# CityU-AIM-Group/HTD

Measured on AMD Instinct MI355X. Metric: images/sec (1333x800) HTD-R50 train step, higher is better.
Workload: dtype f32; 1 GPU; HTD ResNet-50 FPN fp32 train step fwd+bwd+SGD, batch 4/GPU @ 1333x800 (padded 1344x800), random-init weights, 2000 RPN proposals/img, 512 RoIs/img/stage; global_batch=4, parallelism=dp1, stage2_positives=169, proposals=random-init RPN (few positives: the regression branch is nearly idle)

## Files before the change

### htd_amd/csrc/common.h

```cpp
#pragma once
#include <hip/hip_runtime.h>
#include <stdint.h>
#include <stdio.h>
#include <string.h>

#include "../../include/htd_amd.h"

namespace htd {

void set_error(const char *fmt, ...);
int conv_math();

inline int check_launch(const char *what)
{
    hipError_t e = hipGetLastError();
    if (e != hipSuccess) {
        set_error("%s: launch failed: %s", what, hipGetErrorString(e));
        return HTD_ERR_LAUNCH;
    }
    return HTD_OK;
}

#define HTD_REQUIRE(cond, ...)               \
    do {                                     \
        if (!(cond)) {                       \
            htd::set_error(__VA_ARGS__);     \
            return HTD_ERR_ARG;              \
        }                                    \
    } while (0)

constexpr int kWave = 64;

__device__ __forceinline__ float wave_sum(float v)
{
#pragma unroll
    for (int o = 32; o > 0; o >>= 1) v += __shfl_xor(v, o, 64);
    return v;
}
__device__ __forceinline__ float wave_max(float v)
{
#pragma unroll
    for (int o = 32; o > 0; o >>= 1) v = fmaxf(v, __shfl_xor(v, o, 64));
    return v;
}

__device__ __forceinline__ unsigned mag_bits(float v) { return (v != v) ? 0x7fc00000u : (__float_as_uint(v) & 0x7fffffffu); }
__device__ __forceinline__ unsigned mag_bits4(unsigned mx, float4 v)
{
    return max(max(mx, max(mag_bits(v.x), mag_bits(v.y))), max(mag_bits(v.z), mag_bits(v.w)));
}
__device__ __forceinline__ void wave_mag_out(unsigned bits, float *out)
{
#pragma unroll
    for (int o = 32; o > 0; o >>= 1) bits = max(bits, (unsigned)__shfl_xor((int)bits, o, 64));
    if ((threadIdx.x & 63) == 0 && bits > *reinterpret_cast<volatile unsigned *>(out))
        __hip_atomic_fetch_max(reinterpret_cast<unsigned *>(out), bits, __ATOMIC_RELAXED, __HIP_MEMORY_SCOPE_AGENT);
}

inline int64_t ceil_div(int64_t a, int64_t b) { return (a + b - 1) / b; }

}
```

### htd_amd/csrc/conv_fwd.hip

```cpp
#include <algorithm>
#include <mutex>
#include <unordered_map>

#include <stdlib.h>

#include "common.h"

namespace {

using f32x16 = __attribute__((ext_vector_type(16))) float;
using bf16x8 = __attribute__((ext_vector_type(8))) __bf16;

using bf16x2 = __attribute__((ext_vector_type(2))) __bf16;
using f32x2 = __attribute__((ext_vector_type(2))) float;

__device__ __forceinline__ void split3x2(float a, float b, unsigned &h, unsigned &m, unsigned &l)
{
    union { bf16x2 v; unsigned u; } c;
    c.v = __builtin_convertvector(f32x2{a, b}, bf16x2);
    h = c.u;
    const float ra = a - __uint_as_float(h << 16), rb = b - __uint_as_float(h & 0xffff0000u);
    c.v = __builtin_convertvector(f32x2{ra, rb}, bf16x2);
    m = c.u;
    c.v = __builtin_convertvector(f32x2{ra - __uint_as_float(m << 16), rb - __uint_as_float(m & 0xffff0000u)}, bf16x2);
    l = c.u;
}

__device__ __forceinline__ float4 keep4(bool ok, float4 v)
{
    return make_float4(ok ? v.x : 0.f, ok ? v.y : 0.f, ok ? v.z : 0.f, ok ? v.w : 0.f);
}

__device__ __forceinline__ void mfma_x3(f32x16 &acc, const bf16x8 &a, const bf16x8 &b)
{
    asm("v_mfma_f32_32x32x16_bf16 %0, %1, %2, %0" : "+a"(acc) : "v"(a), "v"(b));
}

struct ConvParams {
    const float *x, *w, *bias, *residual, *mask_src;
    float *y;
    int B, H, W, Ci, Co, kh, kw, stride, pad, dil, Ho, Wo;
    int Hx, Wx;
    int ntaps;
    int tap_dy[16], tap_dx[16], tap_w[16];
    int o_h0, o_w0, o_step, oH, oW;
    int relu;
    int res_H, res_W;
    float res_sh, res_sw;
    int64_t w_bstride;
    const int64_t *group_count;
    int lim;
    int64_t M;
    int mt, nt;
    int splits;
    int slices_per_split;
    float *partial;
    int tail_first, tail_splits, tail_sps;
    int cmajor;
    float *amax_out;
};

template <int BK, int WGM, int WGN, int TM, int TN, bool X3 = false>
struct Tile {
    static constexpr int BM = WGM * TM * 32, BN = WGN * TN * 32;
    static constexpr int LDS_STRIDE = BK + 4;
    static constexpr int ROW_HALFS = 3 * BK + 8;
    static constexpr int VEC_PER_ROW = BK / 4;
    static constexpr int ROWS_PER_PASS = 256 / VEC_PER_ROW;
    static constexpr int PASSES_A = (BM + ROWS_PER_PASS - 1) / ROWS_PER_PASS;
    static constexpr int PASSES_B = (BN + ROWS_PER_PASS - 1) / ROWS_PER_PASS;
    static constexpr int MAIN_FLOATS = X3 ? (BM + BN) * ROW_HALFS / 2 : (BM + BN) * LDS_STRIDE;
    static constexpr int EPI_STRIDE = BN + 4;
    static constexpr int EPI_ROWS = WGM * 32;
    static constexpr int EPI_FLOATS = EPI_ROWS * EPI_STRIDE;
    static constexpr int LDS_FLOATS = MAIN_FLOATS > EPI_FLOATS ? MAIN_FLOATS : EPI_FLOATS;
};

template <int BK, int WGM, int WGN, int TM, int TN, bool TAPS, bool X3 = false>
__global__ __launch_bounds__(256, (TM * TN >= 4 ? 3 : 4)) void conv_igemm_kernel(ConvParams p)
{
    static_assert(!X3 || BK % 16 == 0, "the bf16 MFMA takes 16 k per instruction");
    using T = Tile<BK, WGM, WGN, TM, TN, X3>;
    __shared__ __attribute__((aligned(16))) float lds[T::LDS_FLOATS];

    const int nblk = p.mt * p.nt;
    int bid = blockIdx.x, tail_split = -1;
    if (p.tail_splits > 0) {
        const int xcd = bid % 8, idx = bid / 8, dp = p.tail_first / 8;
        if (idx < dp) {
            bid = xcd * dp + idx;
        } else {
            const int units = (nblk - p.tail_first) * p.tail_splits, q = units / 8, r = units % 8;
            const int w = (xcd < r ? xcd * (q + 1) : r * (q + 1) + (xcd - r) * q) + (idx - dp);
            bid = p.tail_first + w / p.tail_splits;
            tail_split = w % p.tail_splits;
        }
    } else {
        const int q = nblk / 8, r = nblk % 8, xcd = bid % 8, idx = bid / 8;
        bid = (xcd < r ? xcd * (q + 1) : r * (q + 1) + (xcd - r) * q) + idx;
    }
    const int tile_m = bid / p.nt, tile_n = bid % p.nt;
    const int64_t m0 = (int64_t)tile_m * T::BM;
    const int n0 = tile_n * T::BN;

    const int tid = threadIdx.x, lane = tid & 63, wave = tid >> 6;
    const int wm = wave / WGN, wn = wave % WGN;

    int k_limit = 0x7fffffff;
    if (p.group_count) {
        const int rows_per_group = p.Ho * p.Wo;
        const int g = (int)(m0 / rows_per_group);
        const int cnt = (int)p.group_count[g];
        const bool dead = ((p.lim & 1) && (int)(m0 - (int64_t)g * rows_per_group) >= cnt) || ((p.lim & 2) && n0 >= cnt);
        if (dead) {
            for (int e = tid; e < T::BM * (T::BN / 4); e += 256) {
                const int64_t m = m0 + e / (T::BN / 4);
                const int n = n0 + (e % (T::BN / 4)) * 4;
                if (m < p.M && n + 3 < p.Co) *reinterpret_cast<float4 *>(p.y + m * p.Co + n) = make_float4(0.f, 0.f, 0.f, 0.f);
                else if (m < p.M)
                    for (int q = 0; q < 4; ++q)
                        if (n + q < p.Co) p.y[m * p.Co + n + q] = 0.f;
            }
            return;
        }
        if (p.lim & 4) k_limit = cnt;
    }

    const int vcol = tid % T::VEC_PER_ROW;
    const int vrow = tid / T::VEC_PER_ROW;
    int a_hi0[T::PASSES_A], a_wi0[T::PASSES_A];
    unsigned a_img[T::PASSES_A];
    bool a_ok[T::PASSES_A];
#pragma unroll
    for (int i = 0; i < T::PASSES_A; ++i) {
        const int r = vrow + i * T::ROWS_PER_PASS;
        const int64_t m = m0 + r;
        a_ok[i] = r < T::BM && m < p.M;
        const unsigned mm = a_ok[i] ? (unsigned)m : 0u;
        const unsigned wo = mm % (unsigned)p.Wo;
        const unsigned t = mm / (unsigned)p.Wo;
        const unsigned ho = t % (unsigned)p.Ho;
        const unsigned b = t / (unsigned)p.Ho;
        a_hi0[i] = TAPS ? (int)ho : (int)ho * p.stride - p.pad;
        a_wi0[i] = TAPS ? (int)wo : (int)wo * p.stride - p.pad;
        a_img[i] = b * (unsigned)(p.Hx * p.Wx);
    }
    const unsigned wrow_stride = (unsigned)(p.kh * p.kw * p.Ci);
    const float *wbase = p.w + (p.w_bstride > 0 ? (m0 / ((int64_t)p.Ho * p.Wo)) * p.w_bstride : 0);
    bool b_ok[T::PASSES_B];
    unsigned b_off[T::PASSES_B];
#pragma unroll
    for (int i = 0; i < T::PASSES_B; ++i) {
        const int r = vrow + i * T::ROWS_PER_PASS;
        const int n = n0 + r;
        b_ok[i] = r < T::BN && n < p.Co;
        b_off[i] = (unsigned)(b_ok[i] ? n : 0) * wrow_stride + vcol * 4;
    }

    const int slices_per_tap = p.Ci / BK;
    const int total_slices = (TAPS ? p.ntaps : p.kh * p.kw) * slices_per_tap;
    const int s_begin = tail_split >= 0 ? tail_split * p.tail_sps : blockIdx.y * p.slices_per_split;
    int num_slices = min(total_slices, s_begin + (tail_split >= 0 ? p.tail_sps : p.slices_per_split));
    if (k_limit != 0x7fffffff) num_slices = min(num_slices, (k_limit + BK - 1) / BK);

    int ld_ci0, ld_ky, ld_kx;
    unsigned ld_woff;
    const bool cmajor = !TAPS && p.cmajor;
    if (cmajor) {
        const int ntap = p.kh * p.kw, cs = s_begin / ntap, tap = s_begin - cs * ntap;
        ld_ci0 = cs * BK;
        ld_ky = tap / p.kw;
        ld_kx = tap - ld_ky * p.kw;
        ld_woff = (unsigned)(tap * p.Ci + ld_ci0);
    } else {
        const int tap = s_begin / slices_per_tap;
        ld_ci0 = (s_begin - tap * slices_per_tap) * BK;
        ld_ky = TAPS ? tap : tap / p.kw;
        ld_kx = TAPS ? 0 : tap - ld_ky * p.kw;
        ld_woff = (unsigned)s_begin * BK;
    }

    float4 ra[T::PASSES_A], rb[T::PASSES_B];
    unsigned ra_ok = 0u;
    unsigned a_base[T::PASSES_A];
#pragma unroll
    for (int i = 0; i < T::PASSES_A; ++i)
        a_base[i] = (a_img[i] + (unsigned)(a_hi0[i] * p.Wx + a_wi0[i])) * (unsigned)p.Ci + vcol * 4;
    auto load_slice = [&]() {
        const int dy = TAPS ? p.tap_dy[ld_ky] : ld_ky * p.dil;
        const int dx = TAPS ? p.tap_dx[ld_ky] : ld_kx * p.dil;
        const unsigned koff = (unsigned)((dy * p.Wx + dx) * p.Ci + ld_ci0);
#pragma unroll
        for (int i = 0; i < T::PASSES_A; ++i) {
            const bool ok = a_ok[i] & ((unsigned)(a_hi0[i] + dy) < (unsigned)p.H) & ((unsigned)(a_wi0[i] + dx) < (unsigned)p.W);
            const unsigned off = (a_base[i] + koff) & (0u - (unsigned)ok);
            ra[i] = *reinterpret_cast<const float4 *>(p.x + off);
            ra_ok = ok ? (ra_ok | (1u << i)) : (ra_ok & ~(1u << i));
        }
        const unsigned woff = TAPS ? (unsigned)(p.tap_w[ld_ky] * p.Ci + ld_ci0) : ld_woff;
#pragma unroll
        for (int i = 0; i < T::PASSES_B; ++i) rb[i] = *reinterpret_cast<const float4 *>(wbase + b_off[i] + woff);
        if (cmajor) {
            ld_woff += (unsigned)p.Ci;
            if (++ld_kx == p.kw) {
                ld_kx = 0;
                if (++ld_ky == p.kh) {
                    ld_ky = 0;
                    ld_ci0 += BK;
                    ld_woff = (unsigned)ld_ci0;
                }
            }
        } else {
            ld_woff += BK;
            ld_ci0 += BK;
            if (ld_ci0 == p.Ci) {
                ld_ci0 = 0;
                if (TAPS) ++ld_ky;
                else if (++ld_kx == p.kw) { ld_kx = 0; ++ld_ky; }
            }
        }
    };
    auto store_slice = [&](int buf) {
        if constexpr (X3) {
            unsigned short *la = reinterpret_cast<unsigned short *>(lds);
            unsigned short *lb = la + T::BM * T::ROW_HALFS;
            auto put = [&](unsigned short *row, float4 v) {
                unsigned h0, m0_, l0, h1, m1, l1;
                split3x2(v.x, v.y, h0, m0_, l0);
                split3x2(v.z, v.w, h1, m1, l1);
                *reinterpret_cast<uint2 *>(row + vcol * 4) = make_uint2(h0, h1);
                *reinterpret_cast<uint2 *>(row + BK + vcol * 4) = make_uint2(m0_, m1);
                *reinterpret_cast<uint2 *>(row + 2 * BK + vcol * 4) = make_uint2(l0, l1);
            };
#pragma unroll
            for (int i = 0; i < T::PASSES_A; ++i) {
                const int r = vrow + i * T::ROWS_PER_PASS;
                if (T::BM % T::ROWS_PER_PASS == 0 || r < T::BM) put(la + r * T::ROW_HALFS, keep4((ra_ok >> i) & 1u, ra[i]));
            }
#pragma unroll
            for (int i = 0; i < T::PASSES_B; ++i) {
                const int r = vrow + i * T::ROWS_PER_PASS;
                if (T::BN % T::ROWS_PER_PASS == 0 || r < T::BN) put(lb + r * T::ROW_HALFS, keep4(b_ok[i], rb[i]));
            }
            return;
        }
        float *la = lds;
        float *lb = lds + T::BM * T::LDS_STRIDE;
#pragma unroll
        for (int i = 0; i < T::PASSES_A; ++i) {
            const int r = vrow + i * T::ROWS_PER_PASS;
            if (T::BM % T::ROWS_PER_PASS == 0 || r < T::BM)
                *reinterpret_cast<float4 *>(la + r * T::LDS_STRIDE + vcol * 4) = keep4((ra_ok >> i) & 1u, ra[i]);
        }
#pragma unroll
        for (int i = 0; i < T::PASSES_B; ++i) {
            const int r = vrow + i * T::ROWS_PER_PASS;
            if (T::BN % T::ROWS_PER_PASS == 0 || r < T::BN)
                *reinterpret_cast<float4 *>(lb + r * T::LDS_STRIDE + vcol * 4) = keep4(b_ok[i], rb[i]);
        }
// ... 78 lines not shown
            for (int j = 0; j < TN; ++j) asm volatile("s_nop 15" : "+a"(acc[i][j]));
    }

    const bool vec_ok = (p.Co & 3) == 0;
    unsigned omx = 0u;
    constexpr int V = T::BN / 4;
    constexpr int RPP = 256 / V;
#pragma unroll
    for (int i = 0; i < TM; ++i) {
#pragma unroll
        for (int j = 0; j < TN; ++j)
#pragma unroll
            for (int r = 0; r < 16; ++r) {
                const int row = wm * 32 + (r & 3) + 8 * (r >> 2) + 4 * fhalf;
                lds[row * T::EPI_STRIDE + (wn * TN + j) * 32 + frow] = acc[i][j][r];
            }
        __syncthreads();
        const int c4 = tid % V;
        const int n = n0 + c4 * 4;
        constexpr int NPASS = T::EPI_ROWS / RPP;
        if (vec_ok && tail_split < 0 && p.splits <= 1 && p.res_H == 0) {
            const bool col_ok = n < p.Co;
            float4 bv = make_float4(0.f, 0.f, 0.f, 0.f);
            if (p.bias != nullptr && col_ok) bv = *reinterpret_cast<const float4 *>(p.bias + n);
            constexpr int UB = NPASS < 4 ? NPASS : 4;
#pragma unroll
            for (int pass0 = 0; pass0 < NPASS; pass0 += UB) {
                float4 v[UB], rv[UB], mv[UB];
                int64_t o[UB];
                bool ok[UB];
#pragma unroll
                for (int u = 0; u < UB; ++u) {
                    const int row = tid / V + (pass0 + u) * RPP;
                    const int64_t m = m0 + ((row >> 5) * TM + i) * 32 + (row & 31);
                    ok[u] = m < p.M && col_ok;
                    int64_t oo;
                    if constexpr (TAPS) {
                        const unsigned mm = ok[u] ? (unsigned)m : 0u, wo = mm % (unsigned)p.Wo, t = mm / (unsigned)p.Wo;
                        const unsigned ho = t % (unsigned)p.Ho, b = t / (unsigned)p.Ho;
                        oo = (((int64_t)b * p.oH + p.o_h0 + p.o_step * (int)ho) * p.oW + p.o_w0 + p.o_step * (int)wo) * p.Co + n;
                    } else
                        oo = m * p.Co + n;
                    o[u] = oo & -(int64_t)ok[u];
                    v[u] = *reinterpret_cast<const float4 *>(lds + row * T::EPI_STRIDE + c4 * 4);
                }
                if (p.residual != nullptr) {
#pragma unroll
                    for (int u = 0; u < UB; ++u) rv[u] = *reinterpret_cast<const float4 *>(p.residual + o[u]);
                }
                if (p.mask_src != nullptr) {
#pragma unroll
                    for (int u = 0; u < UB; ++u) mv[u] = *reinterpret_cast<const float4 *>(p.mask_src + o[u]);
                }
#pragma unroll
                for (int u = 0; u < UB; ++u) { v[u].x += bv.x; v[u].y += bv.y; v[u].z += bv.z; v[u].w += bv.w; }
                if (p.residual != nullptr) {
#pragma unroll
                    for (int u = 0; u < UB; ++u) { v[u].x += rv[u].x; v[u].y += rv[u].y; v[u].z += rv[u].z; v[u].w += rv[u].w; }
                }
                if (p.relu) {
#pragma unroll
                    for (int u = 0; u < UB; ++u) {
                        v[u].x = fmaxf(v[u].x, 0.f); v[u].y = fmaxf(v[u].y, 0.f); v[u].z = fmaxf(v[u].z, 0.f); v[u].w = fmaxf(v[u].w, 0.f);
                    }
                }
                if (p.mask_src != nullptr) {
#pragma unroll
                    for (int u = 0; u < UB; ++u) {
                        v[u].x = mv[u].x > 0.f ? v[u].x : 0.f; v[u].y = mv[u].y > 0.f ? v[u].y : 0.f;
                        v[u].z = mv[u].z > 0.f ? v[u].z : 0.f; v[u].w = mv[u].w > 0.f ? v[u].w : 0.f;
                    }
                }
#pragma unroll
                for (int u = 0; u < UB; ++u)
                    if (ok[u]) {
                        *reinterpret_cast<float4 *>(p.y + o[u]) = v[u];
                        omx = htd::mag_bits4(omx, v[u]);
                    }
            }
            if (i + 1 < TM) __syncthreads();
            continue;
        }
#pragma unroll
        for (int pass = 0; pass < NPASS; ++pass) {
            const int row = tid / V + pass * RPP;
            const int64_t m = m0 + ((row >> 5) * TM + i) * 32 + (row & 31);
            if (m >= p.M || n >= p.Co) continue;
            float4 v = *reinterpret_cast<const float4 *>(lds + row * T::EPI_STRIDE + c4 * 4);
            int64_t o;
            if constexpr (TAPS) {
                const unsigned mm = (unsigned)m, wo = mm % (unsigned)p.Wo, t = mm / (unsigned)p.Wo;
                const unsigned ho = t % (unsigned)p.Ho, b = t / (unsigned)p.Ho;
                o = (((int64_t)b * p.oH + p.o_h0 + p.o_step * (int)ho) * p.oW + p.o_w0 + p.o_step * (int)wo) * p.Co + n;
            } else
                o = m * p.Co + n;
            if (tail_split >= 0) {
                const int lrow = ((row >> 5) * TM + i) * 32 + (row & 31);
                float *dst = p.partial + ((int64_t)(bid - p.tail_first) * p.tail_splits + tail_split) * (T::BM * T::BN) +
                             lrow * T::BN + c4 * 4;
                *reinterpret_cast<float4 *>(dst) = v;
                continue;
            }
            if (p.splits > 1) {
                float *dst = p.partial + (int64_t)blockIdx.y * p.M * p.Co + o;
                if (vec_ok) *reinterpret_cast<float4 *>(dst) = v;
                else {
                    dst[0] = v.x;
                    if (n + 1 < p.Co) dst[1] = v.y;
                    if (n + 2 < p.Co) dst[2] = v.z;
                    if (n + 3 < p.Co) dst[3] = v.w;
                }
                continue;
            }
            if (vec_ok) {
                if (p.bias) {
                    const float4 bv = *reinterpret_cast<const float4 *>(p.bias + n);
                    v.x += bv.x; v.y += bv.y; v.z += bv.z; v.w += bv.w;
                }
                if (p.residual) {
                    int64_t ro = o;
                    if (p.res_H > 0) {
                        const unsigned mm = (unsigned)m, wo = mm % (unsigned)p.Wo, t = mm / (unsigned)p.Wo;
                        const unsigned ho = t % (unsigned)p.Ho, b = t / (unsigned)p.Ho;
                        const int rh = min((int)floorf(ho * p.res_sh), p.res_H - 1);
                        const int rw = min((int)floorf(wo * p.res_sw), p.res_W - 1);
                        ro = (((int64_t)b * p.res_H + rh) * p.res_W + rw) * p.Co + n;
                    }
                    const float4 rv = *reinterpret_cast<const float4 *>(p.residual + ro);
                    v.x += rv.x; v.y += rv.y; v.z += rv.z; v.w += rv.w;
                }
                if (p.relu) { v.x = fmaxf(v.x, 0.f); v.y = fmaxf(v.y, 0.f); v.z = fmaxf(v.z, 0.f); v.w = fmaxf(v.w, 0.f); }
                if (p.mask_src) {
                    const float4 mv = *reinterpret_cast<const float4 *>(p.mask_src + o);
                    v.x = mv.x > 0.f ? v.x : 0.f; v.y = mv.y > 0.f ? v.y : 0.f;
                    v.z = mv.z > 0.f ? v.z : 0.f; v.w = mv.w > 0.f ? v.w : 0.f;
                }
                *reinterpret_cast<float4 *>(p.y + o) = v;
                omx = htd::mag_bits4(omx, v);
            } else {
                auto put = [&](int e, float t) {
                    if (n + e >= p.Co) return;
                    t += p.bias ? p.bias[n + e] : 0.f;
                    if (p.residual) t += p.residual[o + e];
                    if (p.relu) t = fmaxf(t, 0.f);
                    if (p.mask_src) t = p.mask_src[o + e] > 0.f ? t : 0.f;
                    p.y[o + e] = t;
                    omx = max(omx, htd::mag_bits(t));
                };
                put(0, v.x); put(1, v.y); put(2, v.z); put(3, v.w);
            }
        }
        if (i + 1 < TM) __syncthreads();
    }
    if (p.amax_out != nullptr && tail_split < 0 && p.splits <= 1) htd::wave_mag_out(omx, p.amax_out);
}

__global__ __launch_bounds__(256) void conv_splitk_epilogue_kernel(ConvParams p)
{
    const int64_t total = p.M * p.Co;
    unsigned omx = 0u;
    for (int64_t o = (int64_t)blockIdx.x * blockDim.x + threadIdx.x; o < total; o += (int64_t)gridDim.x * blockDim.x) {
        float v = 0.f;
        for (int k = 0; k < p.splits; ++k) v += p.partial[(int64_t)k * total + o];
        const int n = (int)(o % p.Co);
        if (p.bias) v += p.bias[n];
        if (p.residual) {
            int64_t ro = o;
            if (p.res_H > 0) {
                const int64_t m = o / p.Co;
                const unsigned mm = (unsigned)m, wo = mm % (unsigned)p.Wo, t = mm / (unsigned)p.Wo;
                const unsigned ho = t % (unsigned)p.Ho, b = t / (unsigned)p.Ho;
                const int rh = min((int)floorf(ho * p.res_sh), p.res_H - 1);
                const int rw = min((int)floorf(wo * p.res_sw), p.res_W - 1);
                ro = (((int64_t)b * p.res_H + rh) * p.res_W + rw) * p.Co + n;
            }
            v += p.residual[ro];
        }
        if (p.relu) v = fmaxf(v, 0.f);
        if (p.mask_src) v = p.mask_src[o] > 0.f ? v : 0.f;
        p.y[o] = v;
        omx = max(omx, htd::mag_bits(v));
    }
    if (p.amax_out != nullptr) htd::wave_mag_out(omx, p.amax_out);
}

__global__ __launch_bounds__(256) void conv_tail_epilogue_kernel(ConvParams p, int BM, int BN)
{
    const int64_t per_tile = (int64_t)BM * BN, total = (int64_t)(p.mt * p.nt - p.tail_first) * per_tile;
    unsigned omx = 0u;
    for (int64_t e = (int64_t)blockIdx.x * blockDim.x + threadIdx.x; e < total; e += (int64_t)gridDim.x * blockDim.x) {
        const int t = (int)(e / per_tile), within = (int)(e - (int64_t)t * per_tile);
        const int tile = p.tail_first + t, tile_m = tile / p.nt, tile_n = tile % p.nt;
        const int64_t m = (int64_t)tile_m * BM + within / BN;
        const int n = tile_n * BN + within % BN;
        if (m >= p.M || n >= p.Co) continue;
        const float *src = p.partial + (int64_t)t * p.tail_splits * per_tile + within;
        float v = 0.f;
        for (int k = 0; k < p.tail_splits; ++k) v += src[(int64_t)k * per_tile];
        const int64_t o = m * p.Co + n;
        if (p.bias) v += p.bias[n];
        if (p.residual) {
            int64_t ro = o;
            if (p.res_H > 0) {
                const unsigned mm = (unsigned)m, wo = mm % (unsigned)p.Wo, tt = mm / (unsigned)p.Wo;
                const unsigned ho = tt % (unsigned)p.Ho, b = tt / (unsigned)p.Ho;
                const int rh = min((int)floorf(ho * p.res_sh), p.res_H - 1);
                const int rw = min((int)floorf(wo * p.res_sw), p.res_W - 1);
                ro = (((int64_t)b * p.res_H + rh) * p.res_W + rw) * p.Co + n;
            }
            v += p.residual[ro];
        }
        if (p.relu) v = fmaxf(v, 0.f);
        if (p.mask_src) v = p.mask_src[o] > 0.f ? v : 0.f;
        p.y[o] = v;
        omx = max(omx, htd::mag_bits(v));
    }
    if (p.amax_out != nullptr) htd::wave_mag_out(omx, p.amax_out);
}

int g_conv_math = getenv("HTD_CONV_MATH") ? atoi(getenv("HTD_CONV_MATH")) : 1;

template <int WGM, int WGN, int TM, int TN>
void launch_cfg(const ConvParams &p, unsigned blocks, hipStream_t s)
{
    const dim3 grid(blocks, p.splits);
    const bool x3 = g_conv_math == 1;
    if (p.ntaps > 0) {
        if (p.Ci % 16 == 0) {
            if (x3) hipLaunchKernelGGL((conv_igemm_kernel<16, WGM, WGN, TM, TN, true, true>), grid, dim3(256), 0, s, p);
            else hipLaunchKernelGGL((conv_igemm_kernel<16, WGM, WGN, TM, TN, true>), grid, dim3(256), 0, s, p);
        } else
            hipLaunchKernelGGL((conv_igemm_kernel<8, WGM, WGN, TM, TN, true>), grid, dim3(256), 0, s, p);
    } else if (p.Ci % 32 == 0) {
        if (x3) hipLaunchKernelGGL((conv_igemm_kernel<32, WGM, WGN, TM, TN, false, true>), grid, dim3(256), 0, s, p);
        else hipLaunchKernelGGL((conv_igemm_kernel<32, WGM, WGN, TM, TN, false>), grid, dim3(256), 0, s, p);
    } else if (p.Ci % 16 == 0) {
        if (x3) hipLaunchKernelGGL((conv_igemm_kernel<16, WGM, WGN, TM, TN, false, true>), grid, dim3(256), 0, s, p);
        else hipLaunchKernelGGL((conv_igemm_kernel<16, WGM, WGN, TM, TN, false>), grid, dim3(256), 0, s, p);
    } else
        hipLaunchKernelGGL((conv_igemm_kernel<8, WGM, WGN, TM, TN, false>), grid, dim3(256), 0, s, p);
}

int plan_splits(int64_t M, int Co, int Ci, int taps)
{
    const int bk = Ci % 32 == 0 ? 32 : (Ci % 16 == 0 ? 16 : 8);
    const int total_slices = taps * (Ci / bk);
    const int64_t tiles = htd::ceil_div(M, 128) * htd::ceil_div(Co, 64);
    if (tiles <= 0 || tiles >= 384 || total_slices < 16) return 1;
    int64_t want = htd::ceil_div(768, tiles);
    want = std::min<int64_t>(want, total_slices / 8);
    return (int)std::max<int64_t>(1, std::min<int64_t>(want, 16));
}

struct TileCfg { int bm, bn; };
constexpr TileCfg kTileCfg[] = {{64, 64}, {128, 32}, {128, 64}, {128, 128}, {128, 64}, {64, 128}};
constexpr int kNumTileCfg = 6;

static const bool g_tune = getenv("HTD_CONV_TUNE") != nullptr;
int forced_tile()
{
    if (!g_tune) return -1;
    const char *e = getenv("HTD_CONV_FORCE_TILE");
    const int v = e ? atoi(e) : -1;
    return (v >= 0 && v < kNumTileCfg) ? v : -1;
}

static float tile_score(int cfg, int64_t M, int Co, int K, int splits)
{
    const int bm = kTileCfg[cfg].bm, bn = kTileCfg[cfg].bn;
    const int64_t tiles = htd::ceil_div(M, bm) * htd::ceil_div(Co, bn);
    const bool long_k = K >= 1024;
    float base;
    if (g_conv_math == 1) {
        switch (cfg) {
        case 3: base = 1.00f; break;
        case 4: base = long_k ? 0.86f : 0.90f; break;
        case 5: base = long_k ? 0.88f : 0.94f; break;
        default: base = long_k ? 0.72f : 0.82f; break;
        }
    } else {
        switch (cfg) {
        case 3: base = long_k ? 1.00f : 0.90f; break;
        case 4: base = long_k ? 0.98f : 0.97f; break;
        case 5: base = long_k ? 0.98f : 0.98f; break;
        default: base = long_k ? 0.86f : (K >= 512 ? 0.90f : 0.95f); break;
        }
    }
    const float w = (float)(tiles * splits) / 256.f;
    float quant;
    if (w >= 7.f) quant = w / ceilf(w);
    else if (w >= 3.f) quant = 0.97f;
    else quant = w / ceilf(w);
    const float useful = (float)((double)M * Co / ((double)tiles * bm * bn));
    return base * quant * useful;
}

struct TileKey {
    int64_t M;
    int Co, Ci, taps, epi;
    bool operator==(const TileKey &o) const { return M == o.M && Co == o.Co && Ci == o.Ci && taps == o.taps && epi == o.epi; }
};
struct TileKeyHash {
    size_t operator()(const TileKey &k) const
    {
        uint64_t h = (uint64_t)k.M * 0x9E3779B97F4A7C15ull;
        h ^= ((uint64_t)k.Co << 40) ^ ((uint64_t)k.Ci << 20) ^ ((uint64_t)k.taps << 4) ^ (uint64_t)k.epi;
        h *= 0xBF58476D1CE4E5B9ull;
        return (size_t)(h ^ (h >> 29));
    }
};
std::mutex g_tile_mutex;
std::unordered_map<TileKey, int, TileKeyHash> g_tile_table;

int table_tile(int64_t M, int Co, int Ci, int taps, int epi)
{
    std::lock_guard<std::mutex> lock(g_tile_mutex);
    if (g_tile_table.empty()) return -1;
    const auto it = g_tile_table.find(TileKey{M, Co, Ci, taps, epi});
    return it == g_tile_table.end() ? -1 : it->second;
}

int choose_tile(int64_t M, int Co, int Ci, int taps, int epi, int splits, int &bm, int &bn)
{
    const int K = taps * Ci;
    int cfg = forced_tile();
    if (cfg < 0 && epi >= 0) cfg = table_tile(M, Co, Ci, taps, epi);
    if (cfg >= 0 && Co <= 64 && kTileCfg[cfg].bn > 64) cfg = -1;
    if (cfg < 0) {
        if (Co <= 32) cfg = 1;
        else if (Co <= 64) cfg = (htd::ceil_div(M, 128) * htd::ceil_div(Co, 64) < 4400 && M >= 2048) ? 0 : 2;
        else {
            static const int cand[4] = {3, 4, 5, 0};
            float best = -1.f;
            for (int c : cand) {
                const float sc = tile_score(c, M, Co, K, splits);
                if (sc > best * 1.005f) { best = sc; cfg = c; }
            }
        }
    }
    bm = kTileCfg[cfg].bm;
    bn = kTileCfg[cfg].bn;
    return cfg;
}

static const bool g_no_tail = getenv("HTD_CONV_NO_TAIL") != nullptr;
int plan_tail(int64_t M, int Co, int Ci, int taps, int bm, int bn, int &tail_splits, int &tail_sps)
{
    tail_splits = tail_sps = 0;
    if (g_no_tail || (Co & 3)) return 0;
    const int bk = Ci % 32 == 0 ? 32 : (Ci % 16 == 0 ? 16 : 8);
    const int total_slices = taps * (Ci / bk);
    const int64_t tiles = htd::ceil_div(M, bm) * htd::ceil_div(Co, bn);
    const int64_t rem = tiles % 256, whole = tiles - rem;
    if (tiles < 256 * 3 || tiles >= 256 * 7 || rem == 0 || rem > 128 || total_slices < 8) return 0;
    int want = (int)std::min<int64_t>(16, std::max<int64_t>(2, (256 + rem / 2) / rem));
    want = std::min(want, total_slices / 4);
    if (want < 2) return 0;
    tail_sps = (int)htd::ceil_div(total_slices, want);
    tail_splits = (int)htd::ceil_div(total_slices, tail_sps);
    return (int)whole;
}

int launch_conv(ConvParams p, hipStream_t s, void *workspace)
{
    const int bk = (p.Ci % 32 == 0 && p.ntaps == 0) ? 32 : (p.Ci % 16 == 0 ? 16 : 8);
    const int total_slices = (p.ntaps > 0 ? p.ntaps : p.kh * p.kw) * (p.Ci / bk);
    p.splits = (workspace && p.ntaps == 0) ? plan_splits(p.M, p.Co, p.Ci, p.kh * p.kw) : 1;
    p.slices_per_split = (int)htd::ceil_div(total_slices, p.splits);
    p.splits = (int)htd::ceil_div(total_slices, p.slices_per_split);
    int bm, bn;
// ... 309 lines not shown
```

### htd_amd/csrc/conv_wgrad.hip

```cpp
#include <algorithm>

#include "common.h"

namespace {

using f32x16 = __attribute__((ext_vector_type(16))) float;

__device__ __forceinline__ float4 keep4(bool ok, float4 v)
{
    return make_float4(ok ? v.x : 0.f, ok ? v.y : 0.f, ok ? v.z : 0.f, ok ? v.w : 0.f);
}

struct WgradParams {
    const float *x, *gy;
    float *out;
    float *bias_out;
    int B, H, W, Ci, Co, kh, kw, stride, pad, dil, Ho, Wo;
    int64_t K;
    int Ntot;
    int mt, nt, splits;
    int64_t slices_per_split;
    const float *amax_x, *amax_g;
};

// ... 1104 lines not shown
            if ((c & 1) == 0) {
                if constexpr (H2) split2w(v.x * sc, v.y * sc, h[0], l[0]);
                else split3x2w(v.x, v.y, h[0], m[0], l[0]);
            } else {
                if constexpr (H2) split2w(v.z * sc, v.w * sc, h[1], l[1]);
                else split3x2w(v.z, v.w, h[1], m[1], l[1]);
                unsigned short *d = wr + (u >= PA ? b_lds0 : u == 0 ? a_lds0 : a_lds1);
                const int plane = u < PA ? XHD_PLANE_A : XHD_PLANE_B;
                *reinterpret_cast<uint2 *>(d) = make_uint2(h[0], h[1]);
                if constexpr (H2) {
                    *reinterpret_cast<uint2 *>(d + plane) = make_uint2(l[0], l[1]);
                } else {
                    *reinterpret_cast<uint2 *>(d + plane) = make_uint2(m[0], m[1]);
                    *reinterpret_cast<uint2 *>(d + 2 * plane) = make_uint2(l[0], l[1]);
                }
                if (u < PA) { bsum.x += v.x; bsum.y += v.y; bsum.z += v.z; bsum.w += v.w; }
            }
#pragma unroll
            for (int e = c * NM / NC; e < (c + 1) * NM / NC; ++e) {
                const int q = e / (3 * TM), t = (e % (3 * TM)) / TM, i = e % TM;
                acc[t][i] = mfma_x3w<H2>(fa[i][QA[q]], fb[t][QB[q]], acc[t][i]);
            }
            __builtin_amdgcn_sched_barrier(0);
        }
        if (__builtin_amdgcn_readfirstlane(wave) == 0) {
            if (ragged) put(wr + b_lds1, XHD_PLANE_B, qb[1], sx);
        }
        load_slice(qa, qb);
        __syncthreads();
    };
    auto store_slice = [&](unsigned short *wr, const float4 (&qa)[PA], const float4 (&qb)[2]) {
        put(wr + a_lds0, XHD_PLANE_A, qa[0], sg);
        if constexpr (PA > 1) put(wr + a_lds1, XHD_PLANE_A, qa[PA - 1], sg);
#pragma unroll
        for (int i = 0; i < PA; ++i) { bsum.x += qa[i].x; bsum.y += qa[i].y; bsum.z += qa[i].z; bsum.w += qa[i].w; }
        put(wr + b_lds0, XHD_PLANE_B, qb[0], sx);
        if (ragged) put(wr + b_lds1, XHD_PLANE_B, qb[1], sx);
    };

    unsigned short *buf0 = lds, *buf1 = lds + XHD_BUF;
    load_slice(ra[0], rb[0]);
    load_slice(ra[1], rb[1]);
    store_slice(buf0, ra[0], rb[0]);
    load_slice(ra[0], rb[0]);
    __syncthreads();
    for (int s = 0; s < n_slices; s += 2) {
        half(buf0, buf1, ra[1], rb[1]);
        half(buf1, buf0, ra[0], rb[0]);
    }

    if (do_bias) {
        float4 *red = reinterpret_cast<float4 *>(lds);
        __syncthreads();
        red[tid] = bsum;
        __syncthreads();
        if (tid < VA) {
            float4 t = red[tid];
            for (int r = 1; r < RA; ++r) {
                const float4 v = red[r * VA + tid];
                t.x += v.x; t.y += v.y; t.z += v.z; t.w += v.w;
            }
            float *dst = p.bias_out + (int64_t)split * p.Co;
            const int m = m0 + tid * 4;
            if (m < p.Co) dst[m] = t.x;
            if (m + 1 < p.Co) dst[m + 1] = t.y;
            if (m + 2 < p.Co) dst[m + 2] = t.z;
            if (m + 3 < p.Co) dst[m + 3] = t.w;
        }
    }
    float *out = p.out + (int64_t)split * p.Co * p.Ntot;
    const int fcol = lane & 31, fhalf = lane >> 5;
    const int ci = ci0 + wn * 32 + fcol;
    if (ci < p.Ci) {
#pragma unroll
        for (int t = 0; t < 3; ++t) {
            const int n = (ky * 3 + t) * p.Ci + ci;
#pragma unroll
            for (int i = 0; i < TM; ++i)
#pragma unroll
                for (int r = 0; r < 16; ++r) {
                    const int m = m0 + wm * TM * 32 + i * 32 + (r & 3) + 8 * (r >> 2) + 4 * fhalf;
                    if (m < p.Co) out[(int64_t)m * p.Ntot + n] = H2 ? acc[t][i][r] * sg_inv * sx_inv : acc[t][i][r];
                }
        }
    }
}

__global__ __launch_bounds__(256) void splitk_reduce_kernel(const float *__restrict__ ws, float *__restrict__ out,
                                                            int64_t n, int splits, const float *__restrict__ ws2 = nullptr,
                                                            float *__restrict__ out2 = nullptr, int n2 = 0, int acc = 0)
{
    const int extra = out2 ? (n2 + 255) / 256 : 0;
    if ((int)blockIdx.x >= (int)gridDim.x - extra) {
        const int i = ((int)blockIdx.x - ((int)gridDim.x - extra)) * 256 + threadIdx.x;
        if (i < n2) {
            float s = acc ? out2[i] : 0.f;
            int k = 0;
            for (; k + 3 < splits; k += 4) {
                const float a = ws2[(int64_t)k * n2 + i], b = ws2[(int64_t)(k + 1) * n2 + i];
                const float c = ws2[(int64_t)(k + 2) * n2 + i], d = ws2[(int64_t)(k + 3) * n2 + i];
                s += a; s += b; s += c; s += d;
            }
            for (; k < splits; ++k) s += ws2[(int64_t)k * n2 + i];
            out2[i] = s;
        }
        return;
    }
    const unsigned main_blocks = gridDim.x - extra;
    const int64_t n4 = (n & 3) == 0 ? (n >> 2) : 0;
    for (int64_t i = (int64_t)blockIdx.x * blockDim.x + threadIdx.x; i < n4; i += (int64_t)main_blocks * blockDim.x) {
        float4 s = acc ? *reinterpret_cast<const float4 *>(out + i * 4) : make_float4(0.f, 0.f, 0.f, 0.f);
        int k = 0;
        for (; k + 3 < splits; k += 4) {
            float4 v[4];
#pragma unroll
            for (int u = 0; u < 4; ++u) v[u] = *reinterpret_cast<const float4 *>(ws + (int64_t)(k + u) * n + i * 4);
#pragma unroll
            for (int u = 0; u < 4; ++u) { s.x += v[u].x; s.y += v[u].y; s.z += v[u].z; s.w += v[u].w; }
        }
        for (; k < splits; ++k) {
            const float4 v = *reinterpret_cast<const float4 *>(ws + (int64_t)k * n + i * 4);
            s.x += v.x; s.y += v.y; s.z += v.z; s.w += v.w;
        }
        *reinterpret_cast<float4 *>(out + i * 4) = s;
    }
    if (blockIdx.x == 0)
        for (int64_t i = n4 * 4 + threadIdx.x; i < n; i += blockDim.x) {
            float s = acc ? out[i] : 0.f;
            for (int k = 0; k < splits; ++k) s += ws[(int64_t)k * n + i];
            out[i] = s;
        }
}

__global__ __launch_bounds__(256) void reduce_rows_kernel(const float *__restrict__ ws, float *__restrict__ out, int n,
                                                          int rows)
{
    __shared__ float red[16][17];
    const int col = threadIdx.x & 15, grp = threadIdx.x >> 4;
    const int c = blockIdx.x * 16 + col;
    float s = 0.f;
    if (c < n)
        for (int k = grp; k < rows; k += 16) s += ws[(int64_t)k * n + c];
    red[grp][col] = s;
    __syncthreads();
    if (grp == 0 && c < n) {
        float t = red[0][col];
#pragma unroll
        for (int g = 1; g < 16; ++g) t += red[g][col];
        out[c] = t;
    }
}

using htd::mag_bits;
using htd::wave_mag_out;

__global__ __launch_bounds__(256) void colsum_mask_kernel(const float *__restrict__ g, const float *__restrict__ y,
                                                          float *__restrict__ gm, float *__restrict__ partial,
                                                          int64_t rows, int C, int64_t rows_per_block, float *__restrict__ amax_out)
{
    const int c = blockIdx.y * 256 + threadIdx.x;
    const int64_t r0 = (int64_t)blockIdx.x * rows_per_block, r1 = min(rows, r0 + rows_per_block);
    float s = 0.f;
    unsigned mx = 0u;
    if (c < C)
        for (int64_t r = r0; r < r1; ++r) {
            float v = g[r * C + c];
            if (y) {
                v = y[r * C + c] > 0.f ? v : 0.f;
                gm[r * C + c] = v;
            }
            mx = max(mx, mag_bits(v));
            s += v;
        }
    if (amax_out) wave_mag_out(mx, amax_out);
    if (partial && c < C) partial[(int64_t)blockIdx.x * C + c] = s;
}

__global__ __launch_bounds__(256) void colsum_mask_vec_kernel(const float *__restrict__ g, const float *__restrict__ y,
                                                              float *__restrict__ gm, float *__restrict__ partial,
                                                              int64_t rows, int C, int64_t rows_per_block,
                                                              float *__restrict__ amax_out)
{
    __shared__ float4 red[256];
    unsigned mx = 0u;
    const int C4 = C >> 2;
    const int cbase = blockIdx.y * 256;
    const int cw = min(256, C4 - cbase);
    const int R = 256 / cw;
    const int c4 = threadIdx.x % cw, rsub = threadIdx.x / cw;
    const int64_t r0 = (int64_t)blockIdx.x * rows_per_block, r1 = min(rows, r0 + rows_per_block);
    float4 s = make_float4(0.f, 0.f, 0.f, 0.f);
    if (rsub < R) {
        int64_t r = r0 + rsub;
        for (; r + 3 * (int64_t)R < r1; r += 4 * (int64_t)R) {
            float4 v[4], yv[4];
#pragma unroll
            for (int u = 0; u < 4; ++u) {
                const int64_t o = (r + u * (int64_t)R) * C + (int64_t)(cbase + c4) * 4;
                v[u] = *reinterpret_cast<const float4 *>(g + o);
                if (y) yv[u] = *reinterpret_cast<const float4 *>(y + o);
            }
#pragma unroll
            for (int u = 0; u < 4; ++u) {
                if (y) {
                    const int64_t o = (r + u * (int64_t)R) * C + (int64_t)(cbase + c4) * 4;
                    v[u].x = yv[u].x > 0.f ? v[u].x : 0.f; v[u].y = yv[u].y > 0.f ? v[u].y : 0.f;
                    v[u].z = yv[u].z > 0.f ? v[u].z : 0.f; v[u].w = yv[u].w > 0.f ? v[u].w : 0.f;
                    *reinterpret_cast<float4 *>(gm + o) = v[u];
                }
                mx = htd::mag_bits4(mx, v[u]);
                s.x += v[u].x; s.y += v[u].y; s.z += v[u].z; s.w += v[u].w;
            }
        }
        for (; r < r1; r += R) {
            const int64_t o = r * C + (int64_t)(cbase + c4) * 4;
            float4 v = *reinterpret_cast<const float4 *>(g + o);
            if (y) {
                const float4 yv = *reinterpret_cast<const float4 *>(y + o);
                v.x = yv.x > 0.f ? v.x : 0.f; v.y = yv.y > 0.f ? v.y : 0.f;
                v.z = yv.z > 0.f ? v.z : 0.f; v.w = yv.w > 0.f ? v.w : 0.f;
                *reinterpret_cast<float4 *>(gm + o) = v;
            }
            mx = htd::mag_bits4(mx, v);
            s.x += v.x; s.y += v.y; s.z += v.z; s.w += v.w;
        }
    }
    if (amax_out) wave_mag_out(mx, amax_out);
    if (!partial) return;
    red[threadIdx.x] = s;
    __syncthreads();
    if (rsub == 0) {
        for (int k = 1; k < R; ++k) {
            const float4 t = red[k * cw + c4];
            s.x += t.x; s.y += t.y; s.z += t.z; s.w += t.w;
        }
        *reinterpret_cast<float4 *>(partial + (int64_t)blockIdx.x * C + (int64_t)(cbase + c4) * 4) = s;
    }
}

struct Cfg { int splits; int mt, nt; int bm, bn; };

template <int WGM, int WGN, int TM, int TN>
void launch_wgrad(int pix, bool covec, dim3 grid, hipStream_t s, const WgradParams &p)
{
#define HTD_WGRAD_CASE(PIX, CV)                                                                                   \
    if (pix == PIX && covec == CV) {                                                                               \
        hipLaunchKernelGGL((conv_wgrad_kernel<WGM, WGN, TM, TN, PIX, CV>), grid, dim3(256), 0, s, p);             \
        return;                                                                                                    \
    }
    HTD_WGRAD_CASE(PIX_POINTWISE, true) HTD_WGRAD_CASE(PIX_WIDE, true) HTD_WGRAD_CASE(PIX_GENERAL, true)
    HTD_WGRAD_CASE(PIX_POINTWISE, false) HTD_WGRAD_CASE(PIX_WIDE, false) HTD_WGRAD_CASE(PIX_GENERAL, false)
#undef HTD_WGRAD_CASE
}

Cfg choose(int Co, int Ntot, int64_t K)
{
    Cfg c;
    c.bm = Co <= 32 ? 32 : 128;
    c.bn = 128;
    c.mt = (int)htd::ceil_div(Co, c.bm);
    c.nt = (int)htd::ceil_div(Ntot, c.bn);
    const int64_t slices = htd::ceil_div(K, BKW);
    static const int units = getenv("HTD_WGRAD_UNITS") ? atoi(getenv("HTD_WGRAD_UNITS")) : 1536;
    int64_t want = htd::ceil_div(units, (int64_t)c.mt * c.nt);
    const int64_t tiles = (int64_t)c.mt * c.nt;
    int64_t cap = std::max<int64_t>(1, slices / 20);
    if (tiles * cap < 256)
        cap = std::max(cap, std::min<int64_t>(htd::ceil_div(256, tiles), std::max<int64_t>(1, slices / 5)));
    want = std::min<int64_t>(want, cap);
    c.splits = (int)std::max<int64_t>(1, std::min<int64_t>(want, 192));
    if (c.splits >= 6) c.splits = (c.splits + 7) / 8 * 8;
    static const int forced = getenv("HTD_WGRAD_SPLITS") ? atoi(getenv("HTD_WGRAD_SPLITS")) : 0;
    if (forced > 0) c.splits = (int)std::min<int64_t>(forced, slices);
    return c;
}

static const bool g_wgrad_x3h_off = getenv("HTD_WGRAD_X3H") != nullptr && atoi(getenv("HTD_WGRAD_X3H")) == 0;
bool x3h_takes(int Ci, int Co, int kh, int kw, int stride, int pad, int dil)
{
    return !g_wgrad_x3h_off && kh == 3 && kw == 3 && stride == 1 && pad == 1 && dil == 1 && Co >= 64 && (Co & 3) == 0 &&
           Ci >= 32 && (Ci & 3) == 0;
}
int x3h_splits(int B, int H, int W, int Ci, int Co)
{
    const int64_t tiles = htd::ceil_div(Co, 128) * htd::ceil_div(Ci, 64) * 3;
    const int64_t slices = htd::ceil_div((int64_t)B * H * (W + 1), XH_KS);
    static const int target = getenv("HTD_WGRAD_X3H_UNITS") ? atoi(getenv("HTD_WGRAD_X3H_UNITS")) : 768;
    int64_t want = htd::ceil_div(target, tiles);
    int64_t cap = std::max<int64_t>(1, slices / 8);
    if (tiles * cap < 256) cap = std::max(cap, std::min<int64_t>(htd::ceil_div(256, tiles), std::max<int64_t>(1, slices / 4)));
    want = std::min<int64_t>(want, cap);
    int splits = (int)std::max<int64_t>(1, std::min<int64_t>(want, 128));
    if (splits >= 6) splits = (splits + 7) / 8 * 8;
    static const int forced = getenv("HTD_WGRAD_X3H_SPLITS") ? atoi(getenv("HTD_WGRAD_X3H_SPLITS")) : 0;
    if (forced > 0) splits = (int)std::min<int64_t>(forced, std::max<int64_t>(1, slices / 2));
    return splits;
}

}

int g_wgrad_math = -1;

extern "C" int64_t htd_conv2d_wgrad_workspace_bytes(int B, int H, int W, int Ci, int Co, int kh, int kw, int stride,
                                                    int pad, int dil)
{
    const int Ho = (H + 2 * pad - (dil * (kh - 1) + 1)) / stride + 1;
    const int Wo = (W + 2 * pad - (dil * (kw - 1) + 1)) / stride + 1;
    const Cfg c = choose(Co, kh * kw * Ci, (int64_t)B * Ho * Wo);
    int splits = c.splits;
    if (x3h_takes(Ci, Co, kh, kw, stride, pad, dil)) splits = std::max(splits, x3h_splits(B, H, W, Ci, Co));
    return (int64_t)splits * Co * (kh * kw * Ci + 1) * 4 + 256;
}

static int bwd_weight_impl(const float *x, const float *gy, float *gw, float *gbias, int B, int H, int W, int Ci, int Co, int kh,
                           int kw, int stride, int pad, int dil, void *workspace, void *stream, int accumulate,
                           const float *amax_x = nullptr, const float *amax_g = nullptr)
{
    HTD_REQUIRE(B > 0 && H > 0 && W > 0 && Ci > 0 && Co > 0 && kh > 0 && kw > 0 && stride > 0 && dil > 0 && pad >= 0,
                "conv2d_bwd_weight: bad sizes");
    HTD_REQUIRE(Ci % 4 == 0, "conv2d_bwd_weight: Ci=%d must be a multiple of 4", Ci);
    HTD_REQUIRE(x && gy && gw && workspace, "conv2d_bwd_weight: null pointer");
    WgradParams p{};
    p.x = x; p.gy = gy;
    p.amax_x = amax_x; p.amax_g = amax_g;
    const bool h2 = amax_x != nullptr && amax_g != nullptr;
    p.B = B; p.H = H; p.W = W; p.Ci = Ci; p.Co = Co; p.kh = kh; p.kw = kw; p.stride = stride; p.pad = pad; p.dil = dil;
    p.Ho = (H + 2 * pad - (dil * (kh - 1) + 1)) / stride + 1;
    p.Wo = (W + 2 * pad - (dil * (kw - 1) + 1)) / stride + 1;
    HTD_REQUIRE(p.Ho > 0 && p.Wo > 0, "conv2d_bwd_weight: empty output");
    p.K = (int64_t)B * p.Ho * p.Wo;
    HTD_REQUIRE((int64_t)B * H * W * Ci < (1ll << 31) && p.K * Co < (1ll << 31),
                "conv2d_bwd_weight: operand larger than 2^31 elements (32-bit element offsets)");
    p.Ntot = kh * kw * Ci;
    static const int math_env0 = getenv("HTD_CONV_MATH") ? atoi(getenv("HTD_CONV_MATH")) : 1;
    if ((g_wgrad_math < 0 ? math_env0 : g_wgrad_math) == 1 && x3h_takes(Ci, Co, kh, kw, stride, pad, dil)) {
        p.mt = (int)htd::ceil_div(Co, 128);
        p.nt = (int)htd::ceil_div(Ci, 64);
        p.splits = x3h_splits(B, H, W, Ci, Co);
        const int64_t slices = htd::ceil_div((int64_t)B * H * (W + 1), XH_KS);
        p.slices_per_split = htd::ceil_div(slices, p.splits);
        p.splits = (int)htd::ceil_div(slices, p.slices_per_split);
        const bool direct = p.splits == 1 && !accumulate;
        p.out = direct ? gw : (float *)workspace;
        float *bias_part = (float *)workspace + (int64_t)p.splits * Co * p.Ntot;
        p.bias_out = !gbias ? nullptr : (direct ? gbias : bias_part);
        hipStream_t s = (hipStream_t)stream;
        const dim3 grid((unsigned)(p.mt * p.nt * 3 * p.splits));
        static const bool x3hd_on = !(getenv("HTD_WGRAD_X3D") && atoi(getenv("HTD_WGRAD_X3D")) == 0);
        if (x3hd_on && XHD_KS / (W + 1) + 1 <= H && (int64_t)B * H * W * Ci * 4 < (1ll << 31) &&
            (int64_t)B * H * W * Co * 4 < (1ll << 31))
        {
            static const bool tile64 = !(getenv("HTD_WGRAD_TILE64") && atoi(getenv("HTD_WGRAD_TILE64")) == 0);
            if (tile64 && Co <= 64) {
                p.mt = (int)htd::ceil_div(Co, 64);
                const dim3 g64((unsigned)(p.mt * p.nt * 3 * p.splits));
                if (h2) hipLaunchKernelGGL((conv_wgrad_x3hd_kernel<1, true>), g64, dim3(256), 0, s, p);
                else hipLaunchKernelGGL((conv_wgrad_x3hd_kernel<1, false>), g64, dim3(256), 0, s, p);
            } else if (h2) {
                hipLaunchKernelGGL((conv_wgrad_x3hd_kernel<2, true>), grid, dim3(256), 0, s, p);
            } else {
                hipLaunchKernelGGL((conv_wgrad_x3hd_kernel<2, false>), grid, dim3(256), 0, s, p);
            }
        }
        else {
            HTD_REQUIRE(!h2, "conv2d_bwd_weight_h2: this 3x3 layer is not taken by the H2 kernels (htd_conv2d_bwd_weight_h2_supported)");
            if (W + 1 >= XH_KS) hipLaunchKernelGGL(conv_wgrad_x3h_kernel<true>, grid, dim3(256), 0, s, p);
            else hipLaunchKernelGGL(conv_wgrad_x3h_kernel<false>, grid, dim3(256), 0, s, p);
        }
        if (!direct) {
            const int64_t n = (int64_t)Co * p.Ntot;
            const unsigned blocks = (unsigned)std::min<int64_t>(htd::ceil_div(n, 256), 2048);
            const unsigned extra = gbias ? (unsigned)htd::ceil_div(Co, 256) : 0u;
            hipLaunchKernelGGL(splitk_reduce_kernel, dim3(blocks + extra), dim3(256), 0, s, (const float *)workspace, gw, n,
                               p.splits, (const float *)(gbias ? bias_part : nullptr), gbias, Co, accumulate);
        }
        return htd::check_launch("conv2d_bwd_weight");
    }
    const Cfg c = choose(Co, p.Ntot, p.K);
    p.mt = c.mt; p.nt = c.nt; p.splits = c.splits;
    p.slices_per_split = htd::ceil_div(htd::ceil_div(p.K, BKW), c.splits);
// ... 130 lines not shown
```

### htd_amd/csrc/roi_align.hip

```cpp
#include <algorithm>

#include "common.h"

namespace {

struct RoiGeom {
    float start_h, start_w, bin_h, bin_w;
    int grid_h, grid_w, batch;
    float inv_count;
};

__device__ __forceinline__ RoiGeom roi_geometry(const float *roi, float scale, int ph, int pw,
                                                int sampling_ratio, int aligned)
{
    RoiGeom g;
    const float off = aligned ? 0.5f : 0.f;
    g.batch = (int)roi[0];
    g.start_w = roi[1] * scale - off;
    g.start_h = roi[2] * scale - off;
    const float end_w = roi[3] * scale - off, end_h = roi[4] * scale - off;
    float rw = end_w - g.start_w, rh = end_h - g.start_h;
    if (!aligned) { rw = fmaxf(rw, 1.f); rh = fmaxf(rh, 1.f); }
    g.bin_h = rh / (float)ph;
    g.bin_w = rw / (float)pw;
    g.grid_h = sampling_ratio > 0 ? sampling_ratio : (int)ceilf(rh / (float)ph);
    g.grid_w = sampling_ratio > 0 ? sampling_ratio : (int)ceilf(rw / (float)pw);
    const int cnt = g.grid_h * g.grid_w;
    g.inv_count = 1.f / (float)(cnt > 1 ? cnt : 1);
    return g;
}

__device__ __forceinline__ float axis_weight(float start, float bin, int bin_idx, int grid, int p,
                                             int extent)
{
    float w = 0.f;
    const float step = bin / (float)grid;
    const float base = start + (float)bin_idx * bin;
    for (int s = 0; s < grid; ++s) {
        const float v = base + ((float)s + .5f) * step;
        if (v < -1.0f || v > (float)extent) continue;
        const float vc = fminf(fmaxf(v, 0.f), (float)(extent - 1));
        w += fmaxf(0.f, 1.f - fabsf(vc - (float)p));
    }
    return w;
}

__device__ __forceinline__ void axis_span(float start, float bin, int bin_idx, int grid, int extent,
                                          int &lo, int &hi)
{
    if (grid <= 0) { lo = 0; hi = -1; return; }
    const float step = bin / (float)grid;
    const float base = start + (float)bin_idx * bin;
    const float v0 = base + .5f * step, v1 = base + ((float)(grid - 1) + .5f) * step;
    const float c0 = fminf(fmaxf(fminf(v0, v1), 0.f), (float)(extent - 1));
    const float c1 = fminf(fmaxf(fmaxf(v0, v1), 0.f), (float)(extent - 1));
    lo = (int)c0;
    hi = min((int)c1 + 1, extent - 1);
}

__device__ __forceinline__ float lane_bcast(float v, int src)
{
    return __int_as_float(__builtin_amdgcn_readlane(__float_as_int(v), src));
}

template <bool BACKWARD>
__global__ __launch_bounds__(256) void roi_align_kernel(const float *__restrict__ feat_or_gout,
                                                        const float *__restrict__ rois,
                                                        const int64_t *__restrict__ roi_level, int level,
                                                        float *__restrict__ out_or_gfeat, int64_t n,
                                                        int B, int C, int H, int W, int ph, int pw,
                                                        float scale, int sampling_ratio, int aligned,
                                                        int chunks, int64_t tasks)
{
    const int lane = threadIdx.x & 63;
    const int64_t task = (int64_t)blockIdx.x * (blockDim.x >> 6) + (threadIdx.x >> 6);
    if (task >= tasks) return;
    const int chunk = (int)(task % chunks);
    const int64_t t2 = task / chunks;
    const int bin = (int)(t2 % (ph * pw));
    const int64_t ri = t2 / (ph * pw);
    const int64_t roi_row = ri;
    if (roi_level && roi_level[ri] != (int64_t)level) return;
    const int bi = bin / pw, bj = bin % pw;
    const RoiGeom g = roi_geometry(rois + 5 * roi_row, scale, ph, pw, sampling_ratio, aligned);

    int r0, r1, c0, c1;
    axis_span(g.start_h, g.bin_h, bi, g.grid_h, H, r0, r1);
    axis_span(g.start_w, g.bin_w, bj, g.grid_w, W, c0, c1);
    if (g.batch < 0 || g.batch >= B) { r0 = 0; r1 = -1; }

    const size_t img_base = (size_t)g.batch * H * W * C;
    const size_t bin_off = ((size_t)roi_row * ph * pw + bin) * C;

    if (!BACKWARD) {
        const int ch = chunk * 256 + lane * 4;
        const bool act = ch < C;
        float4 acc = make_float4(0.f, 0.f, 0.f, 0.f);
        for (int rb = r0; rb <= r1; rb += 64) {
            const float wy_l = (rb + lane <= r1) ? axis_weight(g.start_h, g.bin_h, bi, g.grid_h, rb + lane, H) : 0.f;
            for (int cb = c0; cb <= c1; cb += 64) {
                const float wx_l = (cb + lane <= c1) ? axis_weight(g.start_w, g.bin_w, bj, g.grid_w, cb + lane, W) : 0.f;
                const int rn = min(64, r1 - rb + 1), cn = min(64, c1 - cb + 1);
                for (int r = 0; r < rn; ++r) {
                    const float wy = lane_bcast(wy_l, r);
                    const float *row = feat_or_gout + img_base + ((size_t)(rb + r) * W + cb) * C + ch;
#pragma unroll 4
                    for (int c = 0; c < cn; ++c) {
                        const float w = wy * lane_bcast(wx_l, c);
                        if (act) {
                            const float4 v = *reinterpret_cast<const float4 *>(row + (size_t)c * C);
                            acc.x += w * v.x; acc.y += w * v.y; acc.z += w * v.z; acc.w += w * v.w;
                        }
                    }
                }
            }
        }
        if (act) {
            acc.x *= g.inv_count; acc.y *= g.inv_count; acc.z *= g.inv_count; acc.w *= g.inv_count;
            *reinterpret_cast<float4 *>(out_or_gfeat + bin_off + ch) = acc;
        }
    } else {
        float go[4];
#pragma unroll
        for (int k = 0; k < 4; ++k) {
            const int ch = chunk * 256 + lane + 64 * k;
            go[k] = ch < C ? feat_or_gout[bin_off + ch] * g.inv_count : 0.f;
        }
        for (int rb = r0; rb <= r1; rb += 64) {
            const float wy_l = (rb + lane <= r1) ? axis_weight(g.start_h, g.bin_h, bi, g.grid_h, rb + lane, H) : 0.f;
            for (int cb = c0; cb <= c1; cb += 64) {
                const float wx_l = (cb + lane <= c1) ? axis_weight(g.start_w, g.bin_w, bj, g.grid_w, cb + lane, W) : 0.f;
                const int rn = min(64, r1 - rb + 1), cn = min(64, c1 - cb + 1);
                for (int r = 0; r < rn; ++r) {
                    const float wy = lane_bcast(wy_l, r);
                    if (wy == 0.f) continue;
                    float *row = out_or_gfeat + img_base + ((size_t)(rb + r) * W + cb) * C + chunk * 256 + lane;
                    for (int c = 0; c < cn; ++c) {
                        const float w = wy * lane_bcast(wx_l, c);
                        if (w == 0.f) continue;
#pragma unroll
                        for (int k = 0; k < 4; ++k)
                            if (chunk * 256 + lane + 64 * k < C)
                                atomicAdd(row + (size_t)c * C + 64 * k, w * go[k]);
                    }
                }
            }
        }
    }
}

template <int WAVES>
__global__ __launch_bounds__(64 * WAVES) void roi_align_fwd_split_kernel(const float *__restrict__ feat, const float *__restrict__ rois,
                                                                  const int64_t *__restrict__ roi_level, int level,
                                                                  float *__restrict__ out, int B, int C, int H, int W, int ph,
                                                                  int pw, float scale, int sampling_ratio, int aligned,
                                                                  int chunks)
{
    __shared__ float4 part[WAVES][64];
    const int lane = threadIdx.x & 63, wave = threadIdx.x >> 6;
    const int64_t task = blockIdx.x;
    const int chunk = (int)(task % chunks);
    const int64_t t2 = task / chunks;
    const int bin = (int)(t2 % (ph * pw));
    const int64_t ri = t2 / (ph * pw);
    if (roi_level && roi_level[ri] != (int64_t)level) return;
    const int bi = bin / pw, bj = bin % pw;
    const RoiGeom g = roi_geometry(rois + 5 * ri, scale, ph, pw, sampling_ratio, aligned);
    int r0, r1, c0, c1;
    axis_span(g.start_h, g.bin_h, bi, g.grid_h, H, r0, r1);
    axis_span(g.start_w, g.bin_w, bj, g.grid_w, W, c0, c1);
    if (g.batch < 0 || g.batch >= B) { r0 = 0; r1 = -1; }
    const size_t img_base = (size_t)g.batch * H * W * C;
    const int ch = chunk * 256 + lane * 4;
    const bool act = ch < C;
    float4 acc = make_float4(0.f, 0.f, 0.f, 0.f);
    for (int rb = r0; rb <= r1; rb += 64) {
        const float wy_l = (rb + lane <= r1) ? axis_weight(g.start_h, g.bin_h, bi, g.grid_h, rb + lane, H) : 0.f;
        const int rn = min(64, r1 - rb + 1);
        for (int cb = c0; cb <= c1; cb += 64) {
            const float wx_l = (cb + lane <= c1) ? axis_weight(g.start_w, g.bin_w, bj, g.grid_w, cb + lane, W) : 0.f;
            const int cn = min(64, c1 - cb + 1);
            for (int r = wave; r < rn; r += WAVES) {
                const float wy = lane_bcast(wy_l, r);
                const float *row = feat + img_base + ((size_t)(rb + r) * W + cb) * C + ch;
#pragma unroll 4
                for (int c = 0; c < cn; ++c) {
                    const float w = wy * lane_bcast(wx_l, c);
                    if (act) {
                        const float4 v = *reinterpret_cast<const float4 *>(row + (size_t)c * C);
                        acc.x += w * v.x; acc.y += w * v.y; acc.z += w * v.z; acc.w += w * v.w;
                    }
                }
            }
        }
    }
    part[wave][lane] = acc;
    __syncthreads();
    if (wave == 0 && act) {
        float4 t = part[0][lane];
#pragma unroll
        for (int w = 1; w < WAVES; ++w) {
            const float4 v = part[w][lane];
            t.x += v.x; t.y += v.y; t.z += v.z; t.w += v.w;
        }
        t.x *= g.inv_count; t.y *= g.inv_count; t.z *= g.inv_count; t.w *= g.inv_count;
        *reinterpret_cast<float4 *>(out + ((size_t)ri * ph * pw + bin) * C + ch) = t;
    }
}

struct LevelTable {
    const float *feat[8];
    int H[8], W[8];
    float scale[8];
};

__global__ __launch_bounds__(256) void roi_align_levels_fwd_kernel(LevelTable tab, const float *__restrict__ rois,
                                                                   const int64_t *__restrict__ roi_level, float *__restrict__ out,
                                                                   int64_t n, int B, int C, int L, int ph, int pw,
                                                                   int sampling_ratio, int aligned, int chunks, int64_t tasks,
                                                                   float *__restrict__ amax_out)
{
    const int lane = threadIdx.x & 63;
    const int64_t task = (int64_t)blockIdx.x * (blockDim.x >> 6) + (threadIdx.x >> 6);
    if (task >= tasks) return;
    const unsigned seen = amax_out ? *reinterpret_cast<const volatile unsigned *>(amax_out) : 0u;
    const int chunk = (int)(task % chunks);
    const int64_t t2 = task / chunks;
    const int bin = (int)(t2 % (ph * pw));
    const int64_t ri = t2 / (ph * pw);
    const int lv = (int)roi_level[ri];
    const int ch = chunk * 256 + lane * 4;
    const bool act = ch < C;
    const size_t bin_off = ((size_t)ri * ph * pw + bin) * C;
    float4 acc = make_float4(0.f, 0.f, 0.f, 0.f);
    RoiGeom g{};
    g.inv_count = 0.f;
    if (lv >= 0 && lv < L) {
        const int H = tab.H[lv], W = tab.W[lv];
        const float *feat = tab.feat[lv];
        const int bi = bin / pw, bj = bin % pw;
        g = roi_geometry(rois + 5 * ri, tab.scale[lv], ph, pw, sampling_ratio, aligned);
        int r0, r1, c0, c1;
        axis_span(g.start_h, g.bin_h, bi, g.grid_h, H, r0, r1);
        axis_span(g.start_w, g.bin_w, bj, g.grid_w, W, c0, c1);
        if (g.batch < 0 || g.batch >= B) { r0 = 0; r1 = -1; }
        const size_t img_base = (size_t)g.batch * H * W * C;
        for (int rb = r0; rb <= r1; rb += 64) {
            const float wy_l = (rb + lane <= r1) ? axis_weight(g.start_h, g.bin_h, bi, g.grid_h, rb + lane, H) : 0.f;
            for (int cb = c0; cb <= c1; cb += 64) {
                const float wx_l = (cb + lane <= c1) ? axis_weight(g.start_w, g.bin_w, bj, g.grid_w, cb + lane, W) : 0.f;
                const int rn = min(64, r1 - rb + 1), cn = min(64, c1 - cb + 1);
                for (int r = 0; r < rn; ++r) {
                    const float wy = lane_bcast(wy_l, r);
                    const float *row = feat + img_base + ((size_t)(rb + r) * W + cb) * C + ch;
#pragma unroll 4
                    for (int c = 0; c < cn; ++c) {
                        const float w = wy * lane_bcast(wx_l, c);
                        if (act) {
                            const float4 v = *reinterpret_cast<const float4 *>(row + (size_t)c * C);
                            acc.x += w * v.x; acc.y += w * v.y; acc.z += w * v.z; acc.w += w * v.w;
                        }
                    }
                }
            }
        }
    }
    if (act) {
        acc.x *= g.inv_count; acc.y *= g.inv_count; acc.z *= g.inv_count; acc.w *= g.inv_count;
        *reinterpret_cast<float4 *>(out + bin_off + ch) = acc;
    }
    if (amax_out) {
        const bool nan = act && ((acc.x != acc.x) | (acc.y != acc.y) | (acc.z != acc.z) | (acc.w != acc.w));
        const float m = act ? fmaxf(fmaxf(fabsf(acc.x), fabsf(acc.y)), fmaxf(fabsf(acc.z), fabsf(acc.w))) : 0.f;
        unsigned bits = nan ? 0x7fc00000u : __float_as_uint(m);
        for (int o = 32; o > 0; o >>= 1) bits = max(bits, (unsigned)__shfl_xor((int)bits, o));
        if (lane == 0 && bits > seen)
            __hip_atomic_fetch_max(reinterpret_cast<unsigned *>(amax_out), bits, __ATOMIC_RELAXED, __HIP_MEMORY_SCOPE_AGENT);
    }
}

struct AllLevelsOut {
    float *out[8];
};

template <int WAVES>
__global__ __launch_bounds__(WAVES == 1 ? 256 : 64 * WAVES) void roi_align_all_levels_fwd_kernel(
    LevelTable tab, AllLevelsOut outs, const float *__restrict__ rois, int64_t n, int B, int C, int L, int ph, int pw,
    int sampling_ratio, int aligned, int chunks, int64_t tasks)
{
    __shared__ float4 part[WAVES == 1 ? 1 : WAVES][64];
    const int lane = threadIdx.x & 63, wave = threadIdx.x >> 6;
    const int64_t task = WAVES == 1 ? (int64_t)blockIdx.x * 4 + wave : (int64_t)blockIdx.x;
    if (WAVES == 1 && task >= tasks) return;
    const int chunk = (int)(task % chunks);
    int64_t t2 = task / chunks;
    const int bin = (int)(t2 % (ph * pw));
    t2 /= ph * pw;
    const int64_t ri = t2 % n;
    const int lv = (int)(t2 / n);
    const int H = tab.H[lv], W = tab.W[lv];
    const float *feat = tab.feat[lv];
    const int bi = bin / pw, bj = bin % pw;
    const RoiGeom g = roi_geometry(rois + 5 * ri, tab.scale[lv], ph, pw, sampling_ratio, aligned);
    int r0, r1, c0, c1;
    axis_span(g.start_h, g.bin_h, bi, g.grid_h, H, r0, r1);
    axis_span(g.start_w, g.bin_w, bj, g.grid_w, W, c0, c1);
    if (g.batch < 0 || g.batch >= B) { r0 = 0; r1 = -1; }
    const size_t img_base = (size_t)g.batch * H * W * C;
    const int ch = chunk * 256 + lane * 4;
    const bool act = ch < C;
    float4 acc = make_float4(0.f, 0.f, 0.f, 0.f);
    for (int rb = r0; rb <= r1; rb += 64) {
        const float wy_l = (rb + lane <= r1) ? axis_weight(g.start_h, g.bin_h, bi, g.grid_h, rb + lane, H) : 0.f;
        const int rn = min(64, r1 - rb + 1);
        for (int cb = c0; cb <= c1; cb += 64) {
            const float wx_l = (cb + lane <= c1) ? axis_weight(g.start_w, g.bin_w, bj, g.grid_w, cb + lane, W) : 0.f;
            const int cn = min(64, c1 - cb + 1);
            for (int r = (WAVES == 1 ? 0 : wave); r < rn; r += WAVES) {
                const float wy = lane_bcast(wy_l, r);
                const float *row = feat + img_base + ((size_t)(rb + r) * W + cb) * C + ch;
#pragma unroll 4
                for (int c = 0; c < cn; ++c) {
                    const float w = wy * lane_bcast(wx_l, c);
                    if (act) {
                        const float4 v = *reinterpret_cast<const float4 *>(row + (size_t)c * C);
                        acc.x += w * v.x; acc.y += w * v.y; acc.z += w * v.z; acc.w += w * v.w;
                    }
                }
            }
        }
    }
    float *dst = outs.out[lv] + ((size_t)ri * ph * pw + bin) * C + ch;
    if constexpr (WAVES == 1) {
        if (act) {
            acc.x *= g.inv_count; acc.y *= g.inv_count; acc.z *= g.inv_count; acc.w *= g.inv_count;
            *reinterpret_cast<float4 *>(dst) = acc;
        }
    } else {
        part[wave][lane] = acc;
        __syncthreads();
        if (wave == 0 && act) {
            float4 t = part[0][lane];
#pragma unroll
            for (int w = 1; w < WAVES; ++w) {
                const float4 v = part[w][lane];
                t.x += v.x; t.y += v.y; t.z += v.z; t.w += v.w;
            }
            t.x *= g.inv_count; t.y *= g.inv_count; t.z *= g.inv_count; t.w *= g.inv_count;
            *reinterpret_cast<float4 *>(dst) = t;
        }
    }
}

constexpr int MAXP = 8;

__global__ __launch_bounds__(256) void roi_align_bwd_rows_kernel(const float *__restrict__ gout,
                                                                 const float *__restrict__ rois,
                                                                 const int64_t *__restrict__ roi_level, int level,
                                                                 float *__restrict__ gfeat, int64_t n, int B, int C,
                                                                 int H, int W, int ph, int pw, float scale,
                                                                 int sampling_ratio, int aligned, int chunks,
                                                                 int row_slots, int64_t tasks)
{
    const int lane = threadIdx.x & 63;
    const int64_t task = (int64_t)blockIdx.x * (blockDim.x >> 6) + (threadIdx.x >> 6);
    if (task >= tasks) return;
    const int chunk = (int)(task % chunks);
    const int64_t t2 = task / chunks;
    const int slot = (int)(t2 % row_slots);
    const int64_t ri = t2 / row_slots;
    if (roi_level && roi_level[ri] != (int64_t)level) return;
    const RoiGeom g = roi_geometry(rois + 5 * ri, scale, ph, pw, sampling_ratio, aligned);
    if (g.batch < 0 || g.batch >= B) return;
    int r_lo, r_hi, c_lo, c_hi, t0, t1;
    axis_span(g.start_h, g.bin_h, 0, g.grid_h, H, r_lo, t0);
    axis_span(g.start_h, g.bin_h, ph - 1, g.grid_h, H, t1, r_hi);
    if (t0 < r_lo || r_hi < t1) return;
    axis_span(g.start_w, g.bin_w, 0, g.grid_w, W, c_lo, t0);
    axis_span(g.start_w, g.bin_w, pw - 1, g.grid_w, W, t1, c_hi);
    if (t0 < c_lo || c_hi < t1) return;
    const size_t img_base = (size_t)g.batch * H * W * C;
    const float *go = gout + (size_t)ri * ph * pw * C + chunk * 256 + lane;
    bool chk[4];
#pragma unroll
    for (int k = 0; k < 4; ++k) chk[k] = chunk * 256 + lane + 64 * k < C;

    for (int r = r_lo + slot; r <= r_hi; r += row_slots) {
        const float wy_l = lane < ph ? axis_weight(g.start_h, g.bin_h, lane, g.grid_h, r, H) : 0.f;
        float T[MAXP][4];
#pragma unroll
        for (int q = 0; q < MAXP; ++q)
#pragma unroll
            for (int k = 0; k < 4; ++k) T[q][k] = 0.f;
        bool any_row = false;
        for (int p = 0; p < ph; ++p) {
            const float wy = lane_bcast(wy_l, p) * g.inv_count;
            if (wy == 0.f) continue;
            any_row = true;
#pragma unroll
            for (int q = 0; q < MAXP; ++q)
                if (q < pw) {
#pragma unroll
                    for (int k = 0; k < 4; ++k)
                        if (chk[k]) T[q][k] += wy * go[((size_t)p * pw + q) * C + 64 * k];
                }
        }
        if (!any_row) continue;
        for (int cb = c_lo; cb <= c_hi; cb += 64) {
            float wx_l[MAXP];
#pragma unroll
            for (int q = 0; q < MAXP; ++q)
                wx_l[q] = (q < pw && cb + lane <= c_hi) ? axis_weight(g.start_w, g.bin_w, q, g.grid_w, cb + lane, W) : 0.f;
            const int cn = min(64, c_hi - cb + 1);
            float *row = gfeat + img_base + ((size_t)r * W + cb) * C + chunk * 256 + lane;
            for (int c = 0; c < cn; ++c) {
                float v[4] = {0.f, 0.f, 0.f, 0.f};
                bool any = false;
#pragma unroll
                for (int q = 0; q < MAXP; ++q) {
                    const float w = lane_bcast(wx_l[q], c);
                    if (w != 0.f) {
                        any = true;
#pragma unroll
                        for (int k = 0; k < 4; ++k) v[k] += w * T[q][k];
                    }
                }
                if (!any) continue;
#pragma unroll
                for (int k = 0; k < 4; ++k)
                    if (chk[k]) atomicAdd(row + (size_t)c * C + 64 * k, v[k]);
            }
        }
    }
}

constexpr int GW_TILE = 8;

struct RoiBox { short b, r_lo, r_hi, c_lo, c_hi, pad0, pad1, pad2; };

__global__ __launch_bounds__(256) void roi_bbox_kernel(const float *__restrict__ rois, const int64_t *__restrict__ roi_level,
                                                       int level, RoiBox *__restrict__ box, int64_t n, int B, int H, int W,
                                                       int ph, int pw, float scale, int sampling_ratio, int aligned)
{
    const int64_t ri = (int64_t)blockIdx.x * 256 + threadIdx.x;
    if (ri >= n) return;
    RoiBox o{};
    o.b = -1;
    if (!roi_level || roi_level[ri] == (int64_t)level) {
        const RoiGeom g = roi_geometry(rois + 5 * ri, scale, ph, pw, sampling_ratio, aligned);
        int r_lo, r_hi, c_lo, c_hi, t0, t1;
        axis_span(g.start_h, g.bin_h, 0, g.grid_h, H, r_lo, t0);
        axis_span(g.start_h, g.bin_h, ph - 1, g.grid_h, H, t1, r_hi);
        bool ok = g.batch >= 0 && g.batch < B && !(t0 < r_lo || r_hi < t1);
        axis_span(g.start_w, g.bin_w, 0, g.grid_w, W, c_lo, t0);
        axis_span(g.start_w, g.bin_w, pw - 1, g.grid_w, W, t1, c_hi);
        ok = ok && !(t0 < c_lo || c_hi < t1);
        if (ok) { o.b = (short)g.batch; o.r_lo = (short)r_lo; o.r_hi = (short)r_hi; o.c_lo = (short)c_lo; o.c_hi = (short)c_hi; }
    }
    box[ri] = o;
}

template <int CPL, int ROWS, int RS, bool FOLD>
__device__ __forceinline__ void gather_tile(const float *__restrict__ gout, const float *__restrict__ rois,
                                            const RoiBox *__restrict__ box, float *__restrict__ gfeat, int64_t n, int B, int C,
                                            int H, int W, int ph, int pw, float scale, int sampling_ratio, int aligned,
                                            int accumulate, int chunks, int segs, int hts, int64_t task, bool active,
                                            const float *__restrict__ tbuf)
{
    static_assert(!FOLD || ROWS == 1, "folded rows: one-row tiles");
    static_assert(ROWS * MAXP <= 64, "one lane per (row, bin) weight");
    static_assert(RS == 1 || ROWS == 1, "the RoI split keeps one-row tiles");
    const int lane = threadIdx.x & 63;
    const int wave = threadIdx.x >> 6, part = wave % RS;
    constexpr unsigned long long kEvery = RS == 4 ? 0x1111111111111111ull : (RS == 2 ? 0x5555555555555555ull : ~0ull);
    const unsigned long long mine = kEvery << part;
    const int chunk = (int)(task % chunks);
    int64_t t2 = task / chunks;
    const int seg = (int)(t2 % segs);
    t2 /= segs;
    const int ht = (int)(t2 % hts), b = (int)(t2 / hts);
    const int y0 = ht * ROWS, y1 = min(H, y0 + ROWS) - 1;
    const int x0 = seg * GW_TILE, x1 = min(W, x0 + GW_TILE) - 1;
    const int ch = chunk * 64 * CPL + lane * CPL;
    const bool act = ch < C;

    float acc[ROWS][GW_TILE][CPL];
#pragma unroll
    for (int r = 0; r < ROWS; ++r)
#pragma unroll
        for (int i = 0; i < GW_TILE; ++i)
#pragma unroll
            for (int k = 0; k < CPL; ++k) acc[r][i][k] = 0.f;
    bool touched = false;

    for (int64_t base = 0; base < (active ? n : 0); base += 64) {
        bool hit = false;
        if (base + lane < n) {
            const RoiBox o = box[base + lane];
            hit = o.b == b && o.r_lo <= y1 && y0 <= o.r_hi && o.c_lo <= x1 && o.c_hi >= x0;
        }
        unsigned long long mask = __ballot(hit) & mine;
        while (mask) {
            const int src = __builtin_ctzll(mask);
            mask &= mask - 1;
            const int64_t ri = base + src;
            touched = true;
            const RoiGeom g = roi_geometry(rois + 5 * ri, scale, ph, pw, sampling_ratio, aligned);
            if constexpr (FOLD) {
                static_assert(GW_TILE * MAXP == 64, "one lane per (bin, pixel) weight");
                const int xi_f = lane % GW_TILE, q_f = lane / GW_TILE;
                const float wx_f = (x0 + xi_f <= x1 && q_f < pw) ? axis_weight(g.start_w, g.bin_w, q_f, g.grid_w, x0 + xi_f, W) : 0.f;
                const float *tp = tbuf + (((size_t)ri * H + y0) * pw) * C + ch;
#pragma unroll
                for (int q = 0; q < MAXP; ++q) {
                    if (q >= pw) continue;
                    if (__ballot(q_f == q && wx_f != 0.f) == 0ull) continue;
                    float v[CPL];
#pragma unroll
                    for (int k = 0; k < CPL; ++k) v[k] = 0.f;
                    if (act) {
                        if constexpr (CPL == 4) {
                            const float4 t4 = *reinterpret_cast<const float4 *>(tp + (size_t)q * C);
                            v[0] = t4.x; v[1] = t4.y; v[2] = t4.z; v[3] = t4.w;
                        } else {
#pragma unroll
                            for (int k = 0; k < CPL; ++k) v[k] = tp[(size_t)q * C + k];
                        }
                    }
#pragma unroll
                    for (int xi = 0; xi < GW_TILE; ++xi) {
                        const float w = lane_bcast(wx_f, q * GW_TILE + xi);
                        if (w != 0.f) {
#pragma unroll
                            for (int k = 0; k < CPL; ++k) acc[0][xi][k] += w * v[k];
                        }
                    }
                }
                continue;
            }
            const int r_l = lane / MAXP, p_l = lane % MAXP;
            const float wy_l = (r_l < ROWS && p_l < ph && y0 + r_l <= y1)
                                   ? axis_weight(g.start_h, g.bin_h, p_l, g.grid_h, y0 + r_l, H) * g.inv_count : 0.f;
            float T[ROWS][MAXP][CPL];
#pragma unroll
            for (int r = 0; r < ROWS; ++r)
#pragma unroll
                for (int q = 0; q < MAXP; ++q)
#pragma unroll
                    for (int k = 0; k < CPL; ++k) T[r][q][k] = 0.f;
            const float *go = gout + (size_t)ri * ph * pw * C + ch;
            for (int p = 0; p < ph; ++p) {
                float wy[ROWS];
                bool any = false;
#pragma unroll
                for (int r = 0; r < ROWS; ++r) {
                    wy[r] = lane_bcast(wy_l, r * MAXP + p);
                    any = any || wy[r] != 0.f;
                }
                if (!any) continue;
#pragma unroll
                for (int q = 0; q < MAXP; ++q)
                    if (q < pw && act) {
                        float v[CPL];
                        if constexpr (CPL == 4) {
                            const float4 t = *reinterpret_cast<const float4 *>(go + ((size_t)p * pw + q) * C);
                            v[0] = t.x; v[1] = t.y; v[2] = t.z; v[3] = t.w;
                        } else if constexpr (CPL == 2) {
                            const float2 t = *reinterpret_cast<const float2 *>(go + ((size_t)p * pw + q) * C);
                            v[0] = t.x; v[1] = t.y;
                        } else {
                            v[0] = go[((size_t)p * pw + q) * C];
                        }
#pragma unroll
                        for (int r = 0; r < ROWS; ++r)
#pragma unroll
                            for (int k = 0; k < CPL; ++k) T[r][q][k] += wy[r] * v[k];
                    }
            }
            static_assert(GW_TILE * MAXP == 64, "one lane per (bin, pixel) weight");
            const int xi_l = lane % GW_TILE, q_l = lane / GW_TILE;
            const float wx_l = (x0 + xi_l <= x1 && q_l < pw) ? axis_weight(g.start_w, g.bin_w, q_l, g.grid_w, x0 + xi_l, W) : 0.f;
#pragma unroll
            for (int xi = 0; xi < GW_TILE; ++xi) {
#pragma unroll
                for (int q = 0; q < MAXP; ++q) {
                    if (q >= pw) continue;
                    const float w = lane_bcast(wx_l, q * GW_TILE + xi);
                    if (w != 0.f) {
#pragma unroll
                        for (int r = 0; r < ROWS; ++r)
#pragma unroll
                            for (int k = 0; k < CPL; ++k) acc[r][xi][k] += w * T[r][q][k];
                    }
                }
            }
        }
    }
    if constexpr (RS > 1) {
        __shared__ float lsum[4][GW_TILE * CPL][64];
        __shared__ int ltouched[4];
        if (part > 0) {
#pragma unroll
            for (int i = 0; i < GW_TILE; ++i)
#pragma unroll
                for (int k = 0; k < CPL; ++k) lsum[wave][i * CPL + k][lane] = acc[0][i][k];
            if (lane == 0) ltouched[wave] = touched ? 1 : 0;
        }
        __syncthreads();
        if (part > 0) return;
#pragma unroll
        for (int w = 1; w < RS; ++w) {
#pragma unroll
            for (int i = 0; i < GW_TILE; ++i)
#pragma unroll
                for (int k = 0; k < CPL; ++k) acc[0][i][k] += lsum[wave + w][i * CPL + k][lane];
            touched = touched || ltouched[wave + w] != 0;
        }
    }
    if (!active || !act || (accumulate && !touched)) return;
#pragma unroll
    for (int r = 0; r < ROWS; ++r) {
        if (y0 + r > y1) continue;
        float *row = gfeat + (((size_t)b * H + y0 + r) * W + x0) * C + ch;
#pragma unroll
        for (int xi = 0; xi < GW_TILE; ++xi) {
            if (x0 + xi > x1) continue;
            float *dst = row + (size_t)xi * C;
#pragma unroll
            for (int k = 0; k < CPL; ++k) dst[k] = accumulate ? dst[k] + acc[r][xi][k] : acc[r][xi][k];
        }
    }
}

template <int CPL, int ROWS, int RS>
__global__ __launch_bounds__(256, (RS > 1 ? 4 : 1)) void roi_align_bwd_gather_kernel(const float *__restrict__ gout, const float *__restrict__ rois,
                                                                   const RoiBox *__restrict__ box, float *__restrict__ gfeat,
                                                                   int64_t n, int B, int C, int H, int W, int ph, int pw,
                                                                   float scale, int sampling_ratio, int aligned, int accumulate,
                                                                   int chunks, int segs, int hts, int64_t tasks)
{
    const int64_t task = (int64_t)blockIdx.x * (4 / RS) + (threadIdx.x >> 6) / RS;
    if (RS == 1 && task >= tasks) return;
    gather_tile<CPL, ROWS, RS, false>(gout, rois, box, gfeat, n, B, C, H, W, ph, pw, scale, sampling_ratio, aligned, accumulate,
                                      chunks, segs, hts, task < tasks ? task : 0, task < tasks, nullptr);
}

constexpr int GL_MAX = 6;
struct GatherLevels {
    float *gfeat[GL_MAX];
    const float *gout[GL_MAX];
    float *tbuf[GL_MAX];
    int64_t ftask0[GL_MAX + 1];
    const RoiBox *box[GL_MAX];
    int H[GL_MAX], W[GL_MAX], segs[GL_MAX], hts[GL_MAX], accumulate[GL_MAX], level[GL_MAX];
    float scale[GL_MAX];
    int64_t task0[GL_MAX + 1];
    int slots;
};

__global__ __launch_bounds__(256) void roi_fold_kernel(const float *__restrict__ gout, const float *__restrict__ rois, GatherLevels t,
                                                       int64_t n, int C, int ph, int pw, int sampling_ratio, int aligned, int chunks)
{
    const int lane = threadIdx.x & 63;
    const int64_t task = (int64_t)blockIdx.x * 4 + (threadIdx.x >> 6);
    if (task >= t.ftask0[t.slots]) return;
    int k = 0;
#pragma unroll
    for (int i = 1; i < GL_MAX; ++i)
        if (i < t.slots && task >= t.ftask0[i]) k = i;
    int64_t r = task - t.ftask0[k];
    const int chunk = (int)(r % chunks);
    r /= chunks;
    const int H = t.H[k];
    const int y = (int)(r % H);
    const int64_t ri = r / H;
    const RoiBox o = t.box[k][ri];
    if (o.b < 0 || y < o.r_lo || y > o.r_hi) return;
    const RoiGeom g = roi_geometry(rois + 5 * ri, t.scale[k], ph, pw, sampling_ratio, aligned);
    const float wy_l = lane < ph ? axis_weight(g.start_h, g.bin_h, lane, g.grid_h, y, H) * g.inv_count : 0.f;
    const int ch = chunk * 256 + lane * 4;
    if (ch >= C) return;
    float T[MAXP][4];
#pragma unroll
    for (int q = 0; q < MAXP; ++q)
#pragma unroll
        for (int c = 0; c < 4; ++c) T[q][c] = 0.f;
    const float *go = (t.gout[k] ? t.gout[k] : gout) + (size_t)ri * ph * pw * C + ch;
    for (int p = 0; p < ph; ++p) {
        const float wy = lane_bcast(wy_l, p);
        if (wy == 0.f) continue;
#pragma unroll
        for (int q = 0; q < MAXP; ++q)
            if (q < pw) {
                const float4 v = *reinterpret_cast<const float4 *>(go + ((size_t)p * pw + q) * C);
                T[q][0] += wy * v.x; T[q][1] += wy * v.y; T[q][2] += wy * v.z; T[q][3] += wy * v.w;
            }
    }
    float *dst = t.tbuf[k] + (((size_t)ri * H + y) * pw) * C + ch;
#pragma unroll
    for (int q = 0; q < MAXP; ++q)
        if (q < pw) *reinterpret_cast<float4 *>(dst + (size_t)q * C) = make_float4(T[q][0], T[q][1], T[q][2], T[q][3]);
}

template <int CPL, int ROWS, int RS, bool FOLD>
__global__ __launch_bounds__(256, (RS > 1 ? 4 : 1)) void roi_align_bwd_gather_levels_kernel(const float *__restrict__ gout,
                                                                          const float *__restrict__ rois, GatherLevels t, int64_t n,
                                                                          int B, int C, int ph, int pw, int sampling_ratio,
                                                                          int aligned, int chunks)
{
    int64_t task = (int64_t)blockIdx.x * (4 / RS) + (threadIdx.x >> 6) / RS;
    const bool active = task < t.task0[t.slots];
    if (RS == 1 && !active) return;
    if (!active) task = 0;
    int k = 0;
#pragma unroll
    for (int i = 1; i < GL_MAX; ++i)
        if (i < t.slots && task >= t.task0[i]) k = i;
    gather_tile<CPL, ROWS, RS, FOLD>(t.gout[k] ? t.gout[k] : gout, rois, t.box[k], t.gfeat[k], n, B, C, t.H[k], t.W[k], ph, pw,
                                     t.scale[k], sampling_ratio, aligned, t.accumulate[k], chunks, t.segs[k], t.hts[k],
                                     task - t.task0[k], active, t.tbuf[k]);
}

__global__ __launch_bounds__(256) void roi_bbox_levels_kernel(const float *__restrict__ rois, const int64_t *__restrict__ roi_level,
                                                              GatherLevels t, int64_t n, int B, int ph, int pw, int sampling_ratio,
                                                              int aligned)
{
    const int64_t ri = (int64_t)blockIdx.x * 256 + threadIdx.x;
    if (ri >= n) return;
    const int k = blockIdx.y;
    const int H = t.H[k], W = t.W[k];
    RoiBox o{};
    o.b = -1;
    if (!roi_level || roi_level[ri] == (int64_t)t.level[k]) {
        const RoiGeom g = roi_geometry(rois + 5 * ri, t.scale[k], ph, pw, sampling_ratio, aligned);
        int r_lo, r_hi, c_lo, c_hi, t0, t1;
        axis_span(g.start_h, g.bin_h, 0, g.grid_h, H, r_lo, t0);
        axis_span(g.start_h, g.bin_h, ph - 1, g.grid_h, H, t1, r_hi);
        bool ok = g.batch >= 0 && g.batch < B && !(t0 < r_lo || r_hi < t1);
        axis_span(g.start_w, g.bin_w, 0, g.grid_w, W, c_lo, t0);
        axis_span(g.start_w, g.bin_w, pw - 1, g.grid_w, W, t1, c_hi);
        ok = ok && !(t0 < c_lo || c_hi < t1);
        if (ok) { o.b = (short)g.batch; o.r_lo = (short)r_lo; o.r_hi = (short)r_hi; o.c_lo = (short)c_lo; o.c_hi = (short)c_hi; }
    }
    const_cast<RoiBox *>(t.box[k])[ri] = o;
}

int gather_split(int64_t n, int64_t tiles_min, bool every_level)
{
    static const int forced = getenv("HTD_ROI_BWD_SPLIT") ? atoi(getenv("HTD_ROI_BWD_SPLIT")) : 0;
    if (forced == 1 || forced == 2 || forced == 4) return forced;
    (void)n; (void)tiles_min;
    return every_level ? 2 : 1;
}

int launch(bool backward, const float *in, const float *rois, const int64_t *roi_level, int level, float *out,
           int64_t n, int B, int C, int H, int W, int ph, int pw, float scale, int sr, int aligned,
           void *stream)
{
    HTD_REQUIRE(n >= 0 && B > 0 && C > 0 && H > 0 && W > 0 && ph > 0 && pw > 0,
                "roi_align: bad sizes n=%lld B=%d C=%d H=%d W=%d", (long long)n, B, C, H, W);
    HTD_REQUIRE(C % 4 == 0, "roi_align: C=%d must be a multiple of 4 (float4 channel vectors)", C);
    if (n == 0) return HTD_OK;
    HTD_REQUIRE(in && rois && out, "roi_align: null pointer");
    const int chunks = (C + 255) / 256;
    const int waves_per_block = 4;
    hipStream_t s = (hipStream_t)stream;
    if (backward && ph <= MAXP && pw <= MAXP && n * chunks >= 256) {
        const int row_slots = (int)std::min<int64_t>(H, std::max<int64_t>(8, htd::ceil_div(16384, n * chunks)));
        const int64_t tasks = n * row_slots * chunks;
        const int64_t blocks = htd::ceil_div(tasks, waves_per_block);
        HTD_REQUIRE(blocks < (1ll << 31), "roi_align: too many tasks");
        hipLaunchKernelGGL(roi_align_bwd_rows_kernel, dim3((unsigned)blocks), dim3(256), 0, s, in, rois, roi_level,
                           level, out, n, B, C, H, W, ph, pw, scale, sr, aligned, chunks, row_slots, tasks);
        return htd::check_launch("roi_align");
    }
    const int64_t tasks = n * ph * pw * chunks;
    if (!backward && tasks < 8192) {
        hipLaunchKernelGGL(roi_align_fwd_split_kernel<8>, dim3((unsigned)tasks), dim3(512), 0, s, in, rois, roi_level, level, out, B,
                           C, H, W, ph, pw, scale, sr, aligned, chunks);
        return htd::check_launch("roi_align");
    }
    const int64_t blocks = htd::ceil_div(tasks, waves_per_block);
    HTD_REQUIRE(blocks < (1ll << 31), "roi_align: too many tasks");
    if (backward)
        hipLaunchKernelGGL(roi_align_kernel<true>, dim3((unsigned)blocks), dim3(256), 0, s, in, rois, roi_level, level,
                           out, n, B, C, H, W, ph, pw, scale, sr, aligned, chunks, tasks);
    else
        hipLaunchKernelGGL(roi_align_kernel<false>, dim3((unsigned)blocks), dim3(256), 0, s, in, rois, roi_level, level,
                           out, n, B, C, H, W, ph, pw, scale, sr, aligned, chunks, tasks);
    return htd::check_launch("roi_align");
}

}

extern "C" int htd_roi_align_fwd(const float *feat, const float *rois, const int64_t *roi_level, int level,
                                 float *out, int64_t n, int B, int C, int H, int W, int ph, int pw, float spatial_scale,
                                 int sampling_ratio, int aligned, void *stream)
{
    return launch(false, feat, rois, roi_level, level, out, n, B, C, H, W, ph, pw, spatial_scale, sampling_ratio,
                  aligned, stream);
}

static int roi_align_levels_fwd_impl(const float *const *feats, const int *H, const int *W, const float *scales, int L,
                                     const float *rois, const int64_t *roi_level, float *out, int64_t n, int B, int C, int ph,
                                     int pw, int sampling_ratio, int aligned, float *amax_out, void *stream)
{
    HTD_REQUIRE(L > 0 && L <= 8 && n >= 0 && B > 0 && C > 0 && ph > 0 && pw > 0, "roi_align_levels: bad sizes");
    HTD_REQUIRE(C % 4 == 0, "roi_align_levels: C=%d must be a multiple of 4", C);
    if (n == 0) return HTD_OK;
    HTD_REQUIRE(feats && H && W && scales && rois && roi_level && out, "roi_align_levels: null pointer");
    LevelTable tab{};
    for (int l = 0; l < L; ++l) {
        HTD_REQUIRE(feats[l] && H[l] > 0 && W[l] > 0, "roi_align_levels: bad level %d", l);
        tab.feat[l] = feats[l]; tab.H[l] = H[l]; tab.W[l] = W[l]; tab.scale[l] = scales[l];
    }
    const int chunks = (C + 255) / 256;
    const int64_t tasks = n * ph * pw * chunks;
    const int64_t blocks = htd::ceil_div(tasks, 4);
    HTD_REQUIRE(blocks < (1ll << 31), "roi_align_levels: too many tasks");
    hipLaunchKernelGGL(roi_align_levels_fwd_kernel, dim3((unsigned)blocks), dim3(256), 0, (hipStream_t)stream, tab, rois, roi_level, out,
                       n, B, C, L, ph, pw, sampling_ratio, aligned, chunks, tasks, amax_out);
    return htd::check_launch("roi_align_levels");
}

extern "C" int htd_roi_align_levels_fwd(const float *const *feats, const int *H, const int *W, const float *scales, int L,
                                        const float *rois, const int64_t *roi_level, float *out, int64_t n, int B, int C, int ph,
                                        int pw, int sampling_ratio, int aligned, void *stream)
{
    return roi_align_levels_fwd_impl(feats, H, W, scales, L, rois, roi_level, out, n, B, C, ph, pw, sampling_ratio, aligned, nullptr,
                                     stream);
}

extern "C" int htd_roi_align_levels_fwd_amax(const float *const *feats, const int *H, const int *W, const float *scales, int L,
                                             const float *rois, const int64_t *roi_level, float *out, int64_t n, int B, int C,
                                             int ph, int pw, int sampling_ratio, int aligned, float *amax_out, void *stream)
{
    HTD_REQUIRE(amax_out, "roi_align_levels: null maximum");
    return roi_align_levels_fwd_impl(feats, H, W, scales, L, rois, roi_level, out, n, B, C, ph, pw, sampling_ratio, aligned, amax_out,
                                     stream);
}

extern "C" int htd_roi_align_all_levels_fwd(const float *const *feats, const int *H, const int *W, const float *scales, int L,
                                            const float *rois, float *const *outs, int64_t n, int B, int C, int ph, int pw,
                                            int sampling_ratio, int aligned, void *stream)
{
    HTD_REQUIRE(L > 0 && L <= 8 && n >= 0 && B > 0 && C > 0 && ph > 0 && pw > 0, "roi_align_all_levels: bad sizes");
    HTD_REQUIRE(C % 4 == 0, "roi_align_all_levels: C=%d must be a multiple of 4", C);
    if (n == 0) return HTD_OK;
    HTD_REQUIRE(feats && H && W && scales && rois && outs, "roi_align_all_levels: null pointer");
    LevelTable tab{};
    AllLevelsOut o{};
    for (int l = 0; l < L; ++l) {
        HTD_REQUIRE(feats[l] && outs[l] && H[l] > 0 && W[l] > 0, "roi_align_all_levels: bad level %d", l);
        tab.feat[l] = feats[l]; tab.H[l] = H[l]; tab.W[l] = W[l]; tab.scale[l] = scales[l];
        o.out[l] = outs[l];
    }
    const int chunks = (C + 255) / 256;
    const int64_t tasks = (int64_t)L * n * ph * pw * chunks;
    HTD_REQUIRE(tasks < (1ll << 31), "roi_align_all_levels: too many tasks");
    hipStream_t s = (hipStream_t)stream;
    if (tasks < 4 * 8192)
        hipLaunchKernelGGL(roi_align_all_levels_fwd_kernel<8>, dim3((unsigned)tasks), dim3(512), 0, s, tab, o, rois, n, B, C, L, ph, pw,
                           sampling_ratio, aligned, chunks, tasks);
    else
        hipLaunchKernelGGL(roi_align_all_levels_fwd_kernel<1>, dim3((unsigned)htd::ceil_div(tasks, 4)), dim3(256), 0, s, tab, o, rois, n,
                           B, C, L, ph, pw, sampling_ratio, aligned, chunks, tasks);
    return htd::check_launch("roi_align_all_levels");
}

extern "C" int64_t htd_roi_align_bwd_gather_workspace_bytes(int64_t n) { return (n > 0 ? n : 1) * (int64_t)sizeof(RoiBox); }

extern "C" int htd_roi_align_bwd_gather(const float *grad_out, const float *rois, const int64_t *roi_level, int level,
                                        float *grad_feat, int64_t n, int B, int C, int H, int W, int ph, int pw,
                                        float spatial_scale, int sampling_ratio, int aligned, int accumulate, void *workspace,
                                        void *stream)
{
    HTD_REQUIRE(n >= 0 && B > 0 && C > 0 && H > 0 && W > 0 && ph > 0 && pw > 0 && ph <= MAXP && pw <= MAXP,
                "roi_align_bwd_gather: bad sizes n=%lld B=%d C=%d H=%d W=%d out=%dx%d", (long long)n, B, C, H, W, ph, pw);
    HTD_REQUIRE(C % 4 == 0 && H < 32768 && W < 32768 && B < 32768, "roi_align_bwd_gather: C=%d must be a multiple of 4", C);
    HTD_REQUIRE(grad_feat && (n == 0 || (grad_out && rois && workspace)), "roi_align_bwd_gather: null pointer");
    hipStream_t s = (hipStream_t)stream;
    if (n == 0) {
        if (!accumulate && hipMemsetAsync(grad_feat, 0, (size_t)B * H * W * C * 4, s) != hipSuccess) {
            htd::set_error("roi_align_bwd_gather: memset failed");
            return HTD_ERR_LAUNCH;
        }
        return HTD_OK;
    }
    RoiBox *box = (RoiBox *)workspace;
    hipLaunchKernelGGL(roi_bbox_kernel, dim3((unsigned)htd::ceil_div(n, 256)), dim3(256), 0, s, rois, roi_level, level, box, n, B,
                       H, W, ph, pw, spatial_scale, sampling_ratio, aligned);
    const int segs = (W + GW_TILE - 1) / GW_TILE;
    constexpr int rows = 1;
    const int chunks = (C + 255) / 256;
    const int hts = (H + rows - 1) / rows;
    const int64_t tasks = (int64_t)B * hts * segs * chunks;
    const int64_t blocks = htd::ceil_div(tasks, 4);
    HTD_REQUIRE(blocks < (1ll << 31), "roi_align_bwd_gather: too many tiles");
    const int rs = gather_split(n, tasks, roi_level == nullptr);
    if (rs == 4)
        hipLaunchKernelGGL((roi_align_bwd_gather_kernel<4, rows, 4>), dim3((unsigned)tasks), dim3(256), 0, s, grad_out, rois, box,
                           grad_feat, n, B, C, H, W, ph, pw, spatial_scale, sampling_ratio, aligned, accumulate, chunks, segs, hts, tasks);
    else if (rs == 2)
        hipLaunchKernelGGL((roi_align_bwd_gather_kernel<4, rows, 2>), dim3((unsigned)htd::ceil_div(tasks, 2)), dim3(256), 0, s, grad_out,
                           rois, box, grad_feat, n, B, C, H, W, ph, pw, spatial_scale, sampling_ratio, aligned, accumulate, chunks, segs,
                           hts, tasks);
    else
        hipLaunchKernelGGL((roi_align_bwd_gather_kernel<4, rows, 1>), dim3((unsigned)blocks), dim3(256), 0, s, grad_out, rois, box,
                           grad_feat, n, B, C, H, W, ph, pw, spatial_scale, sampling_ratio, aligned, accumulate, chunks, segs, hts, tasks);
    return htd::check_launch("roi_align_bwd_gather");
}

namespace {
int levels_bwd_gather(const float *grad_out, const float *const *grad_outs, const float *rois, const int64_t *roi_level,
                      float *const *grad_feats, const int *H, const int *W, const float *scales, const int *accumulate, int L,
                      int64_t n, int B, int C, int ph, int pw, int sampling_ratio, int aligned, void *workspace, void *stream,
                      const char *what, void *fold_ws = nullptr)
{
    HTD_REQUIRE(L > 0 && L <= GL_MAX && n >= 0 && B > 0 && C > 0 && ph > 0 && pw > 0 && ph <= MAXP && pw <= MAXP,
                "%s: bad sizes L=%d n=%lld B=%d C=%d out=%dx%d", what, L, (long long)n, B, C, ph, pw);
    HTD_REQUIRE(C % 4 == 0 && B < 32768 && grad_feats && H && W && scales && accumulate,
                "%s: C=%d must be a multiple of 4, tables non-null", what, C);
    HTD_REQUIRE(n == 0 || ((grad_out || grad_outs) && rois && workspace), "%s: null pointer", what);
    hipStream_t s = (hipStream_t)stream;
    GatherLevels t{};
    const int chunks = (C + 255) / 256;
    int64_t tasks = 0, tiles_min = 1ll << 62;
    for (int l = L - 1; l >= 0; --l) {
        if (!grad_feats[l]) continue;
        HTD_REQUIRE(H[l] > 0 && W[l] > 0 && H[l] < 32768 && W[l] < 32768, "%s: bad map size", what);
        if (n == 0) {
            if (!accumulate[l] && hipMemsetAsync(grad_feats[l], 0, (size_t)B * H[l] * W[l] * C * 4, s) != hipSuccess) {
                htd::set_error("%s: memset failed", what);
                return HTD_ERR_LAUNCH;
            }
            continue;
        }
        const int k = t.slots++;
        t.gfeat[k] = grad_feats[l];
        t.gout[k] = grad_outs ? grad_outs[l] : nullptr;
        HTD_REQUIRE(!grad_outs || grad_outs[l], "%s: level %d has a gradient map but no grad_out", what, l);
        t.box[k] = (const RoiBox *)workspace + (int64_t)l * n;
        t.H[k] = H[l]; t.W[k] = W[l]; t.scale[k] = scales[l]; t.accumulate[k] = accumulate[l]; t.level[k] = l;
        t.segs[k] = (W[l] + GW_TILE - 1) / GW_TILE;
        t.hts[k] = H[l];
        t.task0[k] = tasks;
        const int64_t tiles = (int64_t)B * t.hts[k] * t.segs[k] * chunks;
        tiles_min = std::min(tiles_min, tiles);
        tasks += tiles;
    }
    if (t.slots == 0) return HTD_OK;
    t.task0[t.slots] = tasks;
    int64_t ftasks = 0, foff = 0;
    for (int k = 0; k < t.slots; ++k) {
        t.tbuf[k] = fold_ws ? (float *)fold_ws + foff : nullptr;
        foff += n * (int64_t)t.H[k] * pw * C;
        t.ftask0[k] = ftasks;
        ftasks += n * (int64_t)t.H[k] * chunks;
    }
    t.ftask0[t.slots] = ftasks;
    hipLaunchKernelGGL(roi_bbox_levels_kernel, dim3((unsigned)htd::ceil_div(n, 256), (unsigned)t.slots), dim3(256), 0, s, rois,
                       roi_level, t, n, B, ph, pw, sampling_ratio, aligned);
    HTD_REQUIRE(tasks < (1ll << 31), "%s: too many tiles", what);
    const int rs = gather_split(n, tiles_min, roi_level == nullptr);
    if (fold_ws) {
        HTD_REQUIRE(ftasks < (1ll << 33), "%s: too many fold tasks", what);
        hipLaunchKernelGGL(roi_fold_kernel, dim3((unsigned)htd::ceil_div(ftasks, 4)), dim3(256), 0, s, grad_out, rois, t, n, C, ph, pw,
                           sampling_ratio, aligned, chunks);
        if (rs == 4)
            hipLaunchKernelGGL((roi_align_bwd_gather_levels_kernel<4, 1, 4, true>), dim3((unsigned)tasks), dim3(256), 0, s, grad_out, rois,
                               t, n, B, C, ph, pw, sampling_ratio, aligned, chunks);
        else if (rs == 2)
            hipLaunchKernelGGL((roi_align_bwd_gather_levels_kernel<4, 1, 2, true>), dim3((unsigned)htd::ceil_div(tasks, 2)), dim3(256), 0,
                               s, grad_out, rois, t, n, B, C, ph, pw, sampling_ratio, aligned, chunks);
        else
            hipLaunchKernelGGL((roi_align_bwd_gather_levels_kernel<4, 1, 1, true>), dim3((unsigned)htd::ceil_div(tasks, 4)), dim3(256), 0,
                               s, grad_out, rois, t, n, B, C, ph, pw, sampling_ratio, aligned, chunks);
        return htd::check_launch(what);
    }
    if (rs == 4)
        hipLaunchKernelGGL((roi_align_bwd_gather_levels_kernel<4, 1, 4, false>), dim3((unsigned)tasks), dim3(256), 0, s, grad_out, rois, t,
                           n, B, C, ph, pw, sampling_ratio, aligned, chunks);
    else if (rs == 2)
        hipLaunchKernelGGL((roi_align_bwd_gather_levels_kernel<4, 1, 2, false>), dim3((unsigned)htd::ceil_div(tasks, 2)), dim3(256), 0, s,
                           grad_out, rois, t, n, B, C, ph, pw, sampling_ratio, aligned, chunks);
    else
        hipLaunchKernelGGL((roi_align_bwd_gather_levels_kernel<4, 1, 1, false>), dim3((unsigned)htd::ceil_div(tasks, 4)), dim3(256), 0, s,
                           grad_out, rois, t, n, B, C, ph, pw, sampling_ratio, aligned, chunks);
    return htd::check_launch(what);
}
}

extern "C" int htd_roi_align_levels_bwd_gather(const float *grad_out, const float *rois, const int64_t *roi_level,
                                               float *const *grad_feats, const int *H, const int *W, const float *scales,
                                               const int *accumulate, int L, int64_t n, int B, int C, int ph, int pw,
                                               int sampling_ratio, int aligned, void *workspace, void *stream)
{
    HTD_REQUIRE(n == 0 || (grad_out && roi_level), "roi_align_levels_bwd_gather: null pointer");
    return levels_bwd_gather(grad_out, nullptr, rois, roi_level, grad_feats, H, W, scales, accumulate, L, n, B, C, ph, pw,
                             sampling_ratio, aligned, workspace, stream, "roi_align_levels_bwd_gather");
}

extern "C" int htd_roi_align_all_levels_bwd_gather(const float *const *grad_outs, const float *rois, float *const *grad_feats,
                                                   const int *H, const int *W, const float *scales, const int *accumulate, int L,
                                                   int64_t n, int B, int C, int ph, int pw, int sampling_ratio, int aligned,
                                                   void *workspace, void *stream)
{
    HTD_REQUIRE(n == 0 || grad_outs, "roi_align_all_levels_bwd_gather: null pointer");
    return levels_bwd_gather(nullptr, grad_outs, rois, nullptr, grad_feats, H, W, scales, accumulate, L, n, B, C, ph, pw,
                             sampling_ratio, aligned, workspace, stream, "roi_align_all_levels_bwd_gather");
}

extern "C" int64_t htd_roi_align_fold_workspace_bytes(int64_t n, const int *H, int L, int pw, int C)
{
    int64_t rows = 0;
    for (int l = 0; l < L; ++l) rows += H[l];
    return (n > 0 ? n : 1) * rows * pw * C * 4;
}

extern "C" int htd_roi_align_levels_bwd_gather_folded(const float *grad_out, const float *rois, const int64_t *roi_level,
                                                      float *const *grad_feats, const int *H, const int *W, const float *scales,
                                                      const int *accumulate, int L, int64_t n, int B, int C, int ph, int pw,
                                                      int sampling_ratio, int aligned, void *workspace, void *fold_ws, void *stream)
{
    HTD_REQUIRE(n == 0 || (grad_out && roi_level && fold_ws), "roi_align_levels_bwd_gather_folded: null pointer");
    return levels_bwd_gather(grad_out, nullptr, rois, roi_level, grad_feats, H, W, scales, accumulate, L, n, B, C, ph, pw,
                             sampling_ratio, aligned, workspace, stream, "roi_align_levels_bwd_gather_folded", fold_ws);
}

extern "C" int htd_roi_align_all_levels_bwd_gather_folded(const float *const *grad_outs, const float *rois, float *const *grad_feats,
                                                          const int *H, const int *W, const float *scales, const int *accumulate,
                                                          int L, int64_t n, int B, int C, int ph, int pw, int sampling_ratio,
                                                          int aligned, void *workspace, void *fold_ws, void *stream)
{
    HTD_REQUIRE(n == 0 || (grad_outs && fold_ws), "roi_align_all_levels_bwd_gather_folded: null pointer");
    return levels_bwd_gather(nullptr, grad_outs, rois, nullptr, grad_feats, H, W, scales, accumulate, L, n, B, C, ph, pw,
                             sampling_ratio, aligned, workspace, stream, "roi_align_all_levels_bwd_gather_folded", fold_ws);
}

extern "C" int htd_roi_align_bwd(const float *grad_out, const float *rois, const int64_t *roi_level, int level,
                                 float *grad_feat, int64_t n, int B, int C, int H, int W, int ph, int pw,
                                 float spatial_scale, int sampling_ratio, int aligned, void *stream)
{
    return launch(true, grad_out, rois, roi_level, level, grad_feat, n, B, C, H, W, ph, pw, spatial_scale,
                  sampling_ratio, aligned, stream);
}
```

### htd_amd/csrc/roi_ops.hip

```cpp
#include <algorithm>

#include "common.h"

namespace {

__device__ __forceinline__ float4 ld4(const float *p) { return *reinterpret_cast<const float4 *>(p); }
__device__ __forceinline__ void st4(float *p, float4 v) { *reinterpret_cast<float4 *>(p) = v; }

__global__ __launch_bounds__(256) void fuse_global_fwd_kernel(const float *__restrict__ x,
                                                              const float *__restrict__ rois,
                                                              const float *__restrict__ g,
                                                              const float *__restrict__ extra, float alpha,
                                                              float *__restrict__ out, int64_t total4, int P,
                                                              int C4, int B, float *__restrict__ amax_out)
{
    unsigned mx = 0u;
    for (int64_t idx = (int64_t)blockIdx.x * blockDim.x + threadIdx.x; idx < total4;
         idx += (int64_t)gridDim.x * blockDim.x) {
        const int c4 = (int)(idx % C4);
        const int64_t i = idx / ((int64_t)P * C4);
        int b = (int)rois[5 * i];
        b = b < 0 ? 0 : (b >= B ? B - 1 : b);
        float4 v = ld4(x + idx * 4);
        const float4 gv = ld4(g + ((int64_t)b * C4 + c4) * 4);
        v.x += gv.x; v.y += gv.y; v.z += gv.z; v.w += gv.w;
        if (extra) {
            const float4 e = ld4(extra + idx * 4);
            v.x += alpha * e.x; v.y += alpha * e.y; v.z += alpha * e.z; v.w += alpha * e.w;
        }
        st4(out + idx * 4, v);
        mx = htd::mag_bits4(mx, v);
    }
    if (amax_out) htd::wave_mag_out(mx, amax_out);
}

__global__ __launch_bounds__(256) void plain_and_fused_kernel(const float *__restrict__ x, const float *__restrict__ rois,
                                                              const float *__restrict__ g, float *__restrict__ both,
                                                              int64_t total4, int P, int C4, int B, float *__restrict__ amax_out)
{
    unsigned mx = 0u;
    for (int64_t idx = (int64_t)blockIdx.x * blockDim.x + threadIdx.x; idx < total4; idx += (int64_t)gridDim.x * blockDim.x) {
        const int c4 = (int)(idx % C4);
        const int64_t i = idx / ((int64_t)P * C4);
        int b = (int)rois[5 * i];
        b = b < 0 ? 0 : (b >= B ? B - 1 : b);
        float4 v = ld4(x + idx * 4);
        st4(both + idx * 4, v);
        mx = htd::mag_bits4(mx, v);
        const float4 gv = ld4(g + ((int64_t)b * C4 + c4) * 4);
        v.x += gv.x; v.y += gv.y; v.z += gv.z; v.w += gv.w;
        st4(both + (total4 + idx) * 4, v);
        mx = htd::mag_bits4(mx, v);
    }
    if (amax_out) htd::wave_mag_out(mx, amax_out);
}

constexpr int ROIS_PER_BLOCK = 16;
__global__ __launch_bounds__(256) void fuse_global_bwd_kernel(const float *__restrict__ grad,
                                                              const float *__restrict__ rois,
                                                              float *__restrict__ gg, int64_t n, int P, int C,
                                                              int B)
{
    const int c = blockIdx.y * 256 + threadIdx.x;
    if (c >= C) return;
    const int64_t i0 = (int64_t)blockIdx.x * ROIS_PER_BLOCK;
    const int64_t i1 = min(n, i0 + ROIS_PER_BLOCK);
    float acc = 0.f;
    int cur = -1;
    for (int64_t i = i0; i < i1; ++i) {
        int b = (int)rois[5 * i];
        b = b < 0 ? 0 : (b >= B ? B - 1 : b);
        if (b != cur) {
            if (cur >= 0) atomicAdd(gg + (int64_t)cur * C + c, acc);
            acc = 0.f;
            cur = b;
        }
        const float *p = grad + (i * P) * C + c;
        for (int q = 0; q < P; ++q) acc += p[(int64_t)q * C];
    }
    if (cur >= 0) atomicAdd(gg + (int64_t)cur * C + c, acc);
}

constexpr int VROIS = 4;
__global__ __launch_bounds__(256) void fuse_global_bwd_vec_kernel(const float *__restrict__ grad,
                                                                  const float *__restrict__ rois,
                                                                  float *__restrict__ gg, int64_t n, int P, int C4,
                                                                  int B)
{
    __shared__ float4 red[4][64];
    const int lane = threadIdx.x & 63, wave = threadIdx.x >> 6;
    const int64_t i0 = (int64_t)blockIdx.x * VROIS, i1 = min(n, i0 + VROIS);
    for (int c4 = blockIdx.y * 64 + lane; c4 - lane < C4; c4 += gridDim.y * 64) {
        const bool live = c4 < C4;
        float4 acc = make_float4(0.f, 0.f, 0.f, 0.f);
        int cur = -1;
        for (int64_t i = i0; i <= i1; ++i) {
            int b = -1;
            if (i < i1) {
                b = (int)rois[5 * i];
                b = b < 0 ? 0 : (b >= B ? B - 1 : b);
            }
            if (b != cur) {
                if (cur >= 0) {
                    red[wave][lane] = acc;
                    __syncthreads();
                    if (wave == 0 && live) {
                        float4 t = red[0][lane];
                        for (int w = 1; w < 4; ++w) { t.x += red[w][lane].x; t.y += red[w][lane].y; t.z += red[w][lane].z; t.w += red[w][lane].w; }
                        float *dst = gg + ((int64_t)cur * C4 + c4) * 4;
                        atomicAdd(dst, t.x); atomicAdd(dst + 1, t.y); atomicAdd(dst + 2, t.z); atomicAdd(dst + 3, t.w);
                    }
                    __syncthreads();
                }
                acc = make_float4(0.f, 0.f, 0.f, 0.f);
                cur = b;
            }
            if (i < i1 && live) {
                const float4 *p = reinterpret_cast<const float4 *>(grad) + (i * P) * C4 + c4;
                for (int q = wave; q < P; q += 4) {
                    const float4 v = p[(int64_t)q * C4];
                    acc.x += v.x; acc.y += v.y; acc.z += v.z; acc.w += v.w;
                }
            }
        }
    }
}

struct Ptr4 { const float *p[4]; };
struct MPtr4 { float *p[4]; };

__device__ __forceinline__ void softmax4(const float *att, int L, int64_t n, int64_t i, float *w)
{
    float m = -INFINITY;
    for (int l = 0; l < L; ++l) m = fmaxf(m, att[l * n + i]);
    float s = 0.f;
    for (int l = 0; l < L; ++l) { w[l] = __expf(att[l * n + i] - m); s += w[l]; }
    const float inv = 1.f / s;
    for (int l = 0; l < L; ++l) w[l] *= inv;
}

__device__ __forceinline__ bool on_ring(int p, int ph, int pw, int edge)
{
    const int y = p / pw, x = p % pw;
    return edge == 0 || y < edge || y >= ph - edge || x < edge || x >= pw - edge;
}

__global__ __launch_bounds__(256) void ba_fuse_fwd_kernel(Ptr4 lvl, int L, const float *__restrict__ border,
                                                          const float *__restrict__ att, float *__restrict__ out,
                                                          int64_t n, int ph, int pw, int C4, int edge)
{
    const int64_t i = blockIdx.x;
    float w[4];
    softmax4(att, L, n, i, w);
    const int P = ph * pw;
    const int64_t base = i * P * C4;
    for (int e = threadIdx.x; e < P * C4; e += blockDim.x) {
        const int p = e / C4;
        float4 acc = make_float4(0.f, 0.f, 0.f, 0.f);
        for (int l = 0; l < L; ++l) {
            const float4 v = ld4(lvl.p[l] + (base + e) * 4);
            acc.x += w[l] * v.x; acc.y += w[l] * v.y; acc.z += w[l] * v.z; acc.w += w[l] * v.w;
        }
        if (on_ring(p, ph, pw, edge)) {
            const float4 v = ld4(border + (base + e) * 4);
            acc.x += v.x; acc.y += v.y; acc.z += v.z; acc.w += v.w;
        }
        st4(out + (base + e) * 4, acc);
    }
}

__global__ __launch_bounds__(256) void ba_fuse_bwd_kernel(Ptr4 lvl, int L, const float *__restrict__ att,
                                                          const float *__restrict__ go, MPtr4 glvl,
                                                          float *__restrict__ gborder, float *__restrict__ gatt,
                                                          int64_t n, int ph, int pw, int C4, int edge)
{
    const int64_t i = blockIdx.x;
    float w[4];
    softmax4(att, L, n, i, w);
    const int P = ph * pw;
    const int64_t base = i * P * C4;
    float d[4] = {0.f, 0.f, 0.f, 0.f};
    for (int e = threadIdx.x; e < P * C4; e += blockDim.x) {
        const int p = e / C4;
        const float4 g = ld4(go + (base + e) * 4);
        const bool ring = on_ring(p, ph, pw, edge);
        for (int l = 0; l < L; ++l) {
            const float4 v = ld4(lvl.p[l] + (base + e) * 4);
            d[l] += g.x * v.x + g.y * v.y + g.z * v.z + g.w * v.w;
            float4 o = make_float4(w[l] * g.x, w[l] * g.y, w[l] * g.z, w[l] * g.w);
            if (l == 0 && gborder == nullptr && ring) {
                o.x += g.x; o.y += g.y; o.z += g.z; o.w += g.w;
            }
            st4(glvl.p[l] + (base + e) * 4, o);
        }
        if (gborder != nullptr) st4(gborder + (base + e) * 4, ring ? g : make_float4(0.f, 0.f, 0.f, 0.f));
    }
    __shared__ float red[4][4];
    const int lane = threadIdx.x & 63, wv = threadIdx.x >> 6;
    for (int l = 0; l < 4; ++l) {
        const float s = htd::wave_sum(d[l]);
        if (lane == 0) red[wv][l] = s;
    }
    __syncthreads();
    if (threadIdx.x == 0) {
        float dl[4], dot = 0.f;
        for (int l = 0; l < L; ++l) {
            dl[l] = red[0][l] + red[1][l] + red[2][l] + red[3][l];
// ... 404 lines not shown
}

__global__ __launch_bounds__(256) void bn_fold_fwd_kernel(const float *__restrict__ w, const float *__restrict__ gamma,
                                                          const float *__restrict__ beta, const float *__restrict__ mean,
                                                          const float *__restrict__ var, float eps,
                                                          float *__restrict__ wf, float *__restrict__ bf, int K)
{
    const int co = blockIdx.x;
    const float s = gamma[co] * rsqrtf(var[co] + eps);
    if (threadIdx.x == 0) bf[co] = beta[co] - mean[co] * s;
    const float *wr = w + (int64_t)co * K;
    float *wo = wf + (int64_t)co * K;
    for (int k = threadIdx.x * 4; k < K; k += 1024) {
        const float4 v = ld4(wr + k);
        st4(wo + k, make_float4(v.x * s, v.y * s, v.z * s, v.w * s));
    }
}

__global__ __launch_bounds__(256) void bn_fold_bwd_kernel(const float *__restrict__ w, const float *__restrict__ gamma,
                                                          const float *__restrict__ mean, const float *__restrict__ var,
                                                          float eps, const float *__restrict__ gwf,
                                                          const float *__restrict__ gbf, float *__restrict__ gw,
                                                          float *__restrict__ ggamma, float *__restrict__ gbeta, int K)
{
    const int co = blockIdx.x;
    const float rs = rsqrtf(var[co] + eps);
    const float s = gamma[co] * rs;
    const float *wr = w + (int64_t)co * K, *gr = gwf + (int64_t)co * K;
    float *go = gw + (int64_t)co * K;
    float dot = 0.f;
    for (int k = threadIdx.x * 4; k < K; k += 1024) {
        const float4 v = ld4(wr + k), g = ld4(gr + k);
        dot += v.x * g.x + v.y * g.y + v.z * g.z + v.w * g.w;
        st4(go + k, make_float4(g.x * s, g.y * s, g.z * s, g.w * s));
    }
    __shared__ float red[4];
    dot = htd::wave_sum(dot);
    if ((threadIdx.x & 63) == 0) red[threadIdx.x >> 6] = dot;
    __syncthreads();
    if (threadIdx.x == 0) {
        const float tot = red[0] + red[1] + red[2] + red[3];
        const float gb = gbf[co];
        gbeta[co] = gb;
        ggamma[co] = (tot - mean[co] * gb) * rs;
    }
}

struct FoldDesc {
    const float *w, *gamma, *beta, *mean, *var;
    float *wf, *bf, *wT;
    int Co, Ci, taps, tile0;
};
struct FoldBwdDesc {
    const float *w, *gamma, *mean, *var, *gwf, *gbf;
    float *gw, *ggamma, *gbeta;
    int Co, K, row0, pad;
};

template <typename D, typename F>
__device__ __forceinline__ int find_layer(const D *d, int n, int idx, F first)
{
    int lo = 0, hi = n - 1;
    while (lo < hi) {
        const int mid = (lo + hi + 1) >> 1;
        if (first(d[mid]) <= idx) lo = mid; else hi = mid - 1;
    }
    return lo;
}

__global__ __launch_bounds__(256) void bn_fold_many_fwd_kernel(const FoldDesc *__restrict__ descs, int n, float eps)
{
    __shared__ float tile[32][33];
    const int l = find_layer(descs, n, (int)blockIdx.x, [](const FoldDesc &x) { return x.tile0; });
    const FoldDesc d = descs[l];
    const int nco = (d.Co + 31) / 32, nci = (d.Ci + 31) / 32;
    int idx = (int)blockIdx.x - d.tile0;
    const int ci_t = idx % nci;
    idx /= nci;
    const int co_t = idx % nco, t = idx / nco;
    const int co0 = co_t * 32, ci0 = ci_t * 32;
    const int tx = threadIdx.x & 31, ty = threadIdx.x >> 5;
    for (int r = ty; r < 32; r += 8) {
        const int co = co0 + r, ci = ci0 + tx;
        float v = 0.f;
        if (co < d.Co && ci < d.Ci) {
            const int64_t i = ((int64_t)co * d.taps + t) * d.Ci + ci;
            if (d.gamma) {
                v = d.w[i] * (d.gamma[co] * rsqrtf(d.var[co] + eps));
                d.wf[i] = v;
            } else
                v = d.w[i];
        }
        tile[r][tx] = v;
    }
    if (d.gamma && t == 0 && ci_t == 0 && ty == 0 && co0 + tx < d.Co) {
        const int co = co0 + tx;
        const float s = d.gamma[co] * rsqrtf(d.var[co] + eps);
        d.bf[co] = d.beta[co] - d.mean[co] * s;
    }
    if (!d.wT) return;
    __syncthreads();
    for (int r = ty; r < 32; r += 8) {
        const int ci = ci0 + r, co = co0 + tx;
        if (ci < d.Ci && co < d.Co) d.wT[((int64_t)ci * d.taps + (d.taps - 1 - t)) * d.Co + co] = tile[tx][r];
    }
}

__global__ __launch_bounds__(256) void bn_fold_many_bwd_kernel(const FoldBwdDesc *__restrict__ descs, int n, float eps)
{
    const int l = find_layer(descs, n, (int)blockIdx.x, [](const FoldBwdDesc &x) { return x.row0; });
    const FoldBwdDesc d = descs[l];
    const int co = (int)blockIdx.x - d.row0, K = d.K;
    const float rs = rsqrtf(d.var[co] + eps);
    const float s = d.gamma[co] * rs;
    const float *wr = d.w + (int64_t)co * K, *gr = d.gwf + (int64_t)co * K;
    float *go = d.gw + (int64_t)co * K;
    float dot = 0.f;
    for (int k = threadIdx.x * 4; k < K; k += 1024) {
        const float4 v = ld4(wr + k), g = ld4(gr + k);
        dot += v.x * g.x + v.y * g.y + v.z * g.z + v.w * g.w;
        st4(go + k, make_float4(g.x * s, g.y * s, g.z * s, g.w * s));
    }
    __shared__ float red[4];
    dot = htd::wave_sum(dot);
    if ((threadIdx.x & 63) == 0) red[threadIdx.x >> 6] = dot;
    __syncthreads();
    if (threadIdx.x == 0) {
        const float tot = red[0] + red[1] + red[2] + red[3];
        const float gb = d.gbf[co];
        d.gbeta[co] = gb;
        d.ggamma[co] = (tot - d.mean[co] * gb) * rs;
    }
}

__global__ __launch_bounds__(256) void rows_gather_kernel(const float4 *__restrict__ x, const int64_t *__restrict__ rows,
                                                          float4 *__restrict__ out, int64_t total, int F4)
{
    for (int64_t t = (int64_t)blockIdx.x * 256 + threadIdx.x; t < total; t += (int64_t)gridDim.x * 256) {
        const int64_t i = t / F4;
        out[t] = x[rows[i] * F4 + (t - i * F4)];
    }
}
__global__ __launch_bounds__(256) void rows_add_kernel(const float4 *__restrict__ g, const int64_t *__restrict__ rows,
                                                       float4 *__restrict__ gx, int64_t total, int F4)
{
    for (int64_t t = (int64_t)blockIdx.x * 256 + threadIdx.x; t < total; t += (int64_t)gridDim.x * 256) {
        const int64_t i = t / F4;
        const int64_t o = rows[i] * F4 + (t - i * F4);
        const float4 a = gx[o], b = g[t];
        gx[o] = make_float4(a.x + b.x, a.y + b.y, a.z + b.z, a.w + b.w);
    }
}

inline unsigned grid_for(int64_t work, int block = 256, int cap = 4096)
{
    int64_t b = htd::ceil_div(work, block);
    return (unsigned)(b < 1 ? 1 : (b > cap ? cap : b));
}

}

static int fuse_global_fwd_impl(const float *roi_feats, const float *rois, const float *global_feat, const float *extra, float alpha,
                                float *out, int64_t n, int P, int C, int B, float *amax_out, void *stream)
{
    HTD_REQUIRE(C % 4 == 0 && P > 0 && B > 0 && n >= 0, "fuse_global: bad sizes n=%lld P=%d C=%d B=%d",
                (long long)n, P, C, B);
    if (n == 0) return HTD_OK;
    HTD_REQUIRE(roi_feats && rois && global_feat && out, "fuse_global: null pointer");
    const int64_t total4 = n * P * (C / 4);
    hipLaunchKernelGGL(fuse_global_fwd_kernel, dim3(grid_for(total4)), dim3(256), 0, (hipStream_t)stream, roi_feats,
                       rois, global_feat, extra, alpha, out, total4, P, C / 4, B, amax_out);
    return htd::check_launch("fuse_global_fwd");
}

extern "C" int htd_fuse_global_fwd(const float *roi_feats, const float *rois, const float *global_feat,
                                   const float *extra, float alpha, float *out, int64_t n, int P, int C, int B,
                                   void *stream)
{
    return fuse_global_fwd_impl(roi_feats, rois, global_feat, extra, alpha, out, n, P, C, B, nullptr, stream);
}

extern "C" int htd_fuse_global_fwd_amax(const float *roi_feats, const float *rois, const float *global_feat, const float *extra,
                                        float alpha, float *out, int64_t n, int P, int C, int B, float *amax_out, void *stream)
{
    HTD_REQUIRE(amax_out, "fuse_global: null maximum");
    return fuse_global_fwd_impl(roi_feats, rois, global_feat, extra, alpha, out, n, P, C, B, amax_out, stream);
}

static int plain_and_fused_impl(const float *roi_feats, const float *rois, const float *global_feat, float *both, int64_t n, int P,
                                int C, int B, float *amax_out, void *stream)
{
    HTD_REQUIRE(C % 4 == 0 && P > 0 && B > 0 && n >= 0, "plain_and_fused: bad sizes n=%lld P=%d C=%d B=%d", (long long)n, P, C, B);
    if (n == 0) return HTD_OK;
    HTD_REQUIRE(roi_feats && rois && global_feat && both, "plain_and_fused: null pointer");
    const int64_t total4 = n * P * (C / 4);
    hipLaunchKernelGGL(plain_and_fused_kernel, dim3(grid_for(total4)), dim3(256), 0, (hipStream_t)stream, roi_feats, rois,
                       global_feat, both, total4, P, C / 4, B, amax_out);
    return htd::check_launch("plain_and_fused_fwd");
}

extern "C" int htd_plain_and_fused_fwd(const float *roi_feats, const float *rois, const float *global_feat, float *both,
                                       int64_t n, int P, int C, int B, void *stream)
{
    return plain_and_fused_impl(roi_feats, rois, global_feat, both, n, P, C, B, nullptr, stream);
}

extern "C" int htd_plain_and_fused_fwd_amax(const float *roi_feats, const float *rois, const float *global_feat, float *both,
                                            int64_t n, int P, int C, int B, float *amax_out, void *stream)
{
    HTD_REQUIRE(amax_out, "plain_and_fused: null maximum");
    return plain_and_fused_impl(roi_feats, rois, global_feat, both, n, P, C, B, amax_out, stream);
}

extern "C" int htd_fuse_global_bwd_global(const float *grad, const float *rois, float *grad_global, int64_t n, int P,
                                          int C, int B, void *stream)
{
    HTD_REQUIRE(P > 0 && C > 0 && B > 0 && n >= 0, "fuse_global_bwd: bad sizes");
    if (n == 0) return HTD_OK;
    HTD_REQUIRE(grad && rois && grad_global, "fuse_global_bwd: null pointer");
    if ((C & 3) == 0 && (((uintptr_t)grad | (uintptr_t)grad_global) & 15) == 0) {
        dim3 grid((unsigned)htd::ceil_div(n, VROIS), (unsigned)htd::ceil_div(C / 4, 64));
        hipLaunchKernelGGL(fuse_global_bwd_vec_kernel, grid, dim3(256), 0, (hipStream_t)stream, grad, rois,
                           grad_global, n, P, C / 4, B);
        return htd::check_launch("fuse_global_bwd");
    }
    dim3 grid((unsigned)htd::ceil_div(n, ROIS_PER_BLOCK), (unsigned)htd::ceil_div(C, 256));
    hipLaunchKernelGGL(fuse_global_bwd_kernel, grid, dim3(256), 0, (hipStream_t)stream, grad, rois, grad_global, n, P,
                       C, B);
    return htd::check_launch("fuse_global_bwd");
}

extern "C" int htd_fuse_global_bwd_global_ws(const float *grad, const float *rois, float *grad_global, int64_t n, int P,
                                             int C, int B, void *workspace, void *stream)
{
    HTD_REQUIRE(P > 0 && C > 0 && B > 0 && n >= 0 && (C & 3) == 0, "fuse_global_bwd_ws: bad sizes");
    HTD_REQUIRE(grad_global, "fuse_global_bwd_ws: null pointer");
    hipStream_t s = (hipStream_t)stream;
    if (n == 0) {
        hipMemsetAsync(grad_global, 0, (size_t)B * C * 4, s);
        return HTD_OK;
    }
    HTD_REQUIRE(grad && rois && workspace, "fuse_global_bwd_ws: null pointer");
    float *tile = (float *)workspace, *partial = tile + n * C;
    const int chunks = (int)htd::ceil_div(n, IMG_CHUNK);
    hipLaunchKernelGGL(roi_tile_sums_kernel, dim3((unsigned)n), dim3(256), 0, s, grad, tile, P, C / 4);
    hipLaunchKernelGGL(image_sums_kernel, dim3((unsigned)B, (unsigned)htd::ceil_div(C / 4, 64), (unsigned)chunks), dim3(64), 0, s,
                       (const float *)tile, rois, partial, n, C / 4, B);
    hipLaunchKernelGGL(chunk_sums_kernel, dim3((unsigned)htd::ceil_div((int64_t)B * C, 256)), dim3(256), 0, s,
                       (const float *)partial, grad_global, (int64_t)B * C, chunks);
    return htd::check_launch("fuse_global_bwd_ws");
}

extern "C" int htd_ba_fuse_fwd(const float *const *lvl, int L, const float *border, const float *att, float *out,
                               int64_t n, int ph, int pw, int C, int edge, void *stream)
{
    HTD_REQUIRE(L >= 1 && L <= 4, "ba_fuse: L=%d not in [1,4]", L);
    HTD_REQUIRE(C % 4 == 0 && ph > 0 && pw > 0 && edge >= 0, "ba_fuse: bad sizes");
    if (n == 0) return HTD_OK;
    HTD_REQUIRE(lvl && border && att && out, "ba_fuse: null pointer");
    Ptr4 p{};
    for (int l = 0; l < L; ++l) p.p[l] = lvl[l];
    hipLaunchKernelGGL(ba_fuse_fwd_kernel, dim3((unsigned)n), dim3(256), 0, (hipStream_t)stream, p, L, border, att,
                       out, n, ph, pw, C / 4, edge);
    return htd::check_launch("ba_fuse_fwd");
}

extern "C" int htd_ba_fuse_bwd(const float *const *lvl, int L, const float *att, const float *grad_out,
                               float *const *grad_lvl, float *grad_border, float *grad_att, int64_t n, int ph, int pw,
                               int C, int edge, void *stream)
{
    HTD_REQUIRE(L >= 1 && L <= 4, "ba_fuse: L=%d not in [1,4]", L);
    HTD_REQUIRE(C % 4 == 0 && ph > 0 && pw > 0 && edge >= 0, "ba_fuse: bad sizes");
    if (n == 0) return HTD_OK;
    HTD_REQUIRE(lvl && att && grad_out && grad_lvl && grad_att, "ba_fuse_bwd: null pointer");
    Ptr4 p{};
    MPtr4 g{};
    for (int l = 0; l < L; ++l) { p.p[l] = lvl[l]; g.p[l] = grad_lvl[l]; }
    hipLaunchKernelGGL(ba_fuse_bwd_kernel, dim3((unsigned)n), dim3(256), 0, (hipStream_t)stream, p, L, att, grad_out,
                       g, grad_border, grad_att, n, ph, pw, C / 4, edge);
    return htd::check_launch("ba_fuse_bwd");
}

extern "C" int htd_global_avg_pool_fwd(const float *x, float *out, int64_t B, int P, int C, void *stream)
{
    HTD_REQUIRE(P > 0 && C > 0 && B >= 0, "global_avg_pool: bad sizes");
    if (B == 0) return HTD_OK;
    HTD_REQUIRE(x && out, "global_avg_pool: null pointer");
    hipLaunchKernelGGL(gap_fwd_kernel, dim3((unsigned)B, (unsigned)htd::ceil_div(C, 256)), dim3(256), 0,
                       (hipStream_t)stream, x, out, P, C);
    return htd::check_launch("global_avg_pool_fwd");
}

extern "C" int htd_global_avg_pool_bwd(const float *g, float *gx, int64_t B, int P, int C, void *stream)
{
    HTD_REQUIRE(P > 0 && C > 0 && C % 4 == 0 && B >= 0, "global_avg_pool_bwd: bad sizes");
    if (B == 0) return HTD_OK;
    HTD_REQUIRE(g && gx, "global_avg_pool_bwd: null pointer");
    const int64_t total4 = B * P * (C / 4);
    hipLaunchKernelGGL(gap_bwd_kernel, dim3(grid_for(total4)), dim3(256), 0, (hipStream_t)stream, g, gx, total4, P,
                       C / 4, 0);
    return htd::check_launch("global_avg_pool_bwd");
}

extern "C" int htd_global_avg_pool_bwd_acc(const float *g, float *gx, int64_t B, int P, int C, void *stream)
{
    HTD_REQUIRE(B >= 0 && P > 0 && C > 0 && C % 4 == 0, "global_avg_pool_bwd_acc: bad sizes");
    if (B == 0) return HTD_OK;
    HTD_REQUIRE(g && gx, "global_avg_pool_bwd_acc: null pointer");
    const int64_t total4 = B * P * (C / 4);
    hipLaunchKernelGGL(gap_bwd_kernel, dim3(grid_for(total4)), dim3(256), 0, (hipStream_t)stream, g, gx, total4, P, C / 4, 1);
    return htd::check_launch("global_avg_pool_bwd_acc");
}

static int gn_fwd_impl(const float *x, const float *gamma, const float *beta, float *y, float *mean, float *rstd, int64_t n, int P,
                       int C, int G, float eps, int relu, float *amax_out, void *stream)
{
    HTD_REQUIRE(G > 0 && C % G == 0, "group_norm: C=%d not divisible by G=%d", C, G);
    const int cpg = C / G;
    HTD_REQUIRE(cpg <= 64 && (cpg & (cpg - 1)) == 0, "group_norm: channels/group=%d must be a power of two <= 64", cpg);
    HTD_REQUIRE(C <= 1024, "group_norm: C=%d > 1024", C);
    if (n == 0) return HTD_OK;
    HTD_REQUIRE(x && gamma && beta && y && mean && rstd, "group_norm: null pointer");
    const int threads = (int)htd::ceil_div(C, 64) * 64;
    if (P <= 49)
        hipLaunchKernelGGL(gn_fwd_kernel<49>, dim3((unsigned)n), dim3(threads), 0, (hipStream_t)stream, x, gamma, beta, y,
                           mean, rstd, P, C, G, eps, relu, amax_out);
    else
        hipLaunchKernelGGL(gn_fwd_kernel<0>, dim3((unsigned)n), dim3(threads), 0, (hipStream_t)stream, x, gamma, beta, y,
                           mean, rstd, P, C, G, eps, relu, amax_out);
    return htd::check_launch("group_norm_fwd");
}

extern "C" int htd_group_norm_relu_fwd(const float *x, const float *gamma, const float *beta, float *y, float *mean,
                                       float *rstd, int64_t n, int P, int C, int G, float eps, int relu, void *stream)
{
    return gn_fwd_impl(x, gamma, beta, y, mean, rstd, n, P, C, G, eps, relu, nullptr, stream);
}

extern "C" int htd_group_norm_relu_fwd_amax(const float *x, const float *gamma, const float *beta, float *y, float *mean,
                                            float *rstd, int64_t n, int P, int C, int G, float eps, int relu, float *amax_out,
                                            void *stream)
{
    return gn_fwd_impl(x, gamma, beta, y, mean, rstd, n, P, C, G, eps, relu, amax_out, stream);
}

extern "C" int htd_group_norm_relu_bwd(const float *x, const float *y, const float *gamma, const float *mean,
                                       const float *rstd, const float *gy, float *gx, float *ggamma, float *gbeta,
                                       int64_t n, int P, int C, int G, int relu, void *stream)
{
    HTD_REQUIRE(G > 0 && C % G == 0, "group_norm: C=%d not divisible by G=%d", C, G);
    const int cpg = C / G;
    HTD_REQUIRE(cpg <= 64 && (cpg & (cpg - 1)) == 0, "group_norm: channels/group=%d must be a power of two <= 64", cpg);
    HTD_REQUIRE(C <= 1024, "group_norm: C=%d > 1024", C);
    if (n == 0) return HTD_OK;
    HTD_REQUIRE(x && y && gamma && mean && rstd && gy && gx && ggamma && gbeta, "group_norm_bwd: null pointer");
    const int threads = (int)htd::ceil_div(C, 64) * 64;
    if (launch_gn_bwd_tile(x, y, gamma, mean, rstd, gy, gx, ggamma, gbeta, n, P, C, G, relu, nullptr, nullptr, (hipStream_t)stream))
        return htd::check_launch("group_norm_bwd");
    hipLaunchKernelGGL((P <= 49 ? gn_bwd_kernel<49> : gn_bwd_kernel<0>), dim3((unsigned)n), dim3(threads), 0, (hipStream_t)stream, x, y, gamma, mean,
                       rstd, gy, gx, ggamma, gbeta, P, C, G, relu, (float *)nullptr);
    return htd::check_launch("group_norm_bwd");
}

static int gn_bwd_ws_impl(const float *x, const float *y, const float *gamma, const float *mean, const float *rstd, const float *gy,
                          float *gx, float *ggamma, float *gbeta, int64_t n, int P, int C, int G, int relu, void *workspace,
                          float *amax_out, void *stream)
{
    HTD_REQUIRE(G > 0 && C % G == 0, "group_norm: C=%d not divisible by G=%d", C, G);
    const int cpg = C / G;
    HTD_REQUIRE(cpg <= 64 && (cpg & (cpg - 1)) == 0, "group_norm: channels/group=%d must be a power of two <= 64", cpg);
    HTD_REQUIRE(C <= 1024, "group_norm: C=%d > 1024", C);
    HTD_REQUIRE(ggamma && gbeta, "group_norm_bwd: null pointer");
    hipStream_t s = (hipStream_t)stream;
    if (n == 0) {
        hipMemsetAsync(ggamma, 0, (size_t)C * 4, s);
        hipMemsetAsync(gbeta, 0, (size_t)C * 4, s);
        return HTD_OK;
    }
    HTD_REQUIRE(x && y && gamma && mean && rstd && gy && gx && workspace, "group_norm_bwd: null pointer");
    const int threads = (int)htd::ceil_div(C, 64) * 64;
    float *ws = (float *)workspace;
    if (!launch_gn_bwd_tile(x, y, gamma, mean, rstd, gy, gx, ggamma, gbeta, n, P, C, G, relu, ws, amax_out, s)) {
        HTD_REQUIRE(amax_out == nullptr, "group_norm_bwd: this shape (C=%d, P=%d) runs on the kernel that leaves no maximum", C, P);
        hipLaunchKernelGGL((P <= 49 ? gn_bwd_kernel<49> : gn_bwd_kernel<0>), dim3((unsigned)n), dim3(threads), 0, s, x, y, gamma, mean, rstd, gy, gx,
                           ggamma, gbeta, P, C, G, relu, ws);
    }
    hipLaunchKernelGGL(colsum_rows_kernel, dim3((unsigned)htd::ceil_div(C, 16), 2), dim3(256), 0, s, (const float *)ws, ggamma,
                       gbeta, C, (int)n);
    return htd::check_launch("group_norm_bwd_ws");
}

extern "C" int htd_group_norm_relu_bwd_ws(const float *x, const float *y, const float *gamma, const float *mean,
                                          const float *rstd, const float *gy, float *gx, float *ggamma, float *gbeta,
                                          int64_t n, int P, int C, int G, int relu, void *workspace, void *stream)
{
    return gn_bwd_ws_impl(x, y, gamma, mean, rstd, gy, gx, ggamma, gbeta, n, P, C, G, relu, workspace, nullptr, stream);
}

extern "C" int htd_group_norm_bwd_amax_supported(int P, int C, int G)
{
    if (gn_tile_off() || G <= 0 || C % G != 0 || (C & 3) || ((C / G) & 3) || C / 4 > 256 || P < 1) return 0;
    const int V = C / 4, R = std::min(1024 / V, P);
    return htd::ceil_div(P, R) <= 8 ? 1 : 0;
}

extern "C" int htd_group_norm_relu_bwd_amax(const float *x, const float *y, const float *gamma, const float *mean,
                                            const float *rstd, const float *gy, float *gx, float *ggamma, float *gbeta,
                                            int64_t n, int P, int C, int G, int relu, void *workspace, float *amax_out, void *stream)
{
    return gn_bwd_ws_impl(x, y, gamma, mean, rstd, gy, gx, ggamma, gbeta, n, P, C, G, relu, workspace, amax_out, stream);
}

extern "C" int htd_sgd_momentum_step(float *param, const float *grad, float *momentum_buf, int64_t n,
                                     const float *lr_dev, float momentum, float weight_decay, float grad_scale,
                                     void *stream)
{
    if (n == 0) return HTD_OK;
    HTD_REQUIRE(param && grad && momentum_buf && lr_dev, "sgd: null pointer");
    HTD_REQUIRE((((uintptr_t)param | (uintptr_t)grad | (uintptr_t)momentum_buf) & 15) == 0,
                "sgd: buffers must be 16-byte aligned");
    hipLaunchKernelGGL(sgd_kernel, dim3(grid_for(n / 4 + 1)), dim3(256), 0, (hipStream_t)stream, param, grad,
                       momentum_buf, n, lr_dev, momentum, weight_decay, grad_scale);
    return htd::check_launch("sgd");
}

__global__ __launch_bounds__(64) void log_accumulate_kernel(const float *__restrict__ packed, int n, int loss_index,
                                                            float weight, int64_t iter, double *__restrict__ acc)
{
    const double w = (double)weight;
    for (int i = threadIdx.x; i < n; i += 64)
        acc[i] = __dadd_rn(acc[i], __dmul_rn(w, (double)packed[i]));
    if (threadIdx.x == 0) {
        acc[n] = __dadd_rn(acc[n], w);
        if (!isfinite(packed[loss_index]) && acc[n + 1] < 0.0) acc[n + 1] = (double)iter;
    }
}

extern "C" int htd_log_accumulate(const float *packed, int n, int loss_index, float weight, int64_t iter, double *acc,
                                  void *stream)
{
    HTD_REQUIRE(n > 0 && loss_index >= 0 && loss_index < n, "log_accumulate: n=%d loss_index=%d", n, loss_index);
    HTD_REQUIRE(iter >= 0, "log_accumulate: iter=%lld", (long long)iter);
    HTD_REQUIRE(packed && acc, "log_accumulate: null pointer");
    hipLaunchKernelGGL(log_accumulate_kernel, dim3(1), dim3(64), 0, (hipStream_t)stream, packed, n, loss_index, weight,
                       iter, acc);
    return htd::check_launch("log_accumulate");
}

extern "C" int htd_bn_fold_fwd(const float *w, const float *gamma, const float *beta, const float *mean,
                               const float *var, float eps, float *w_folded, float *b_folded, int Co, int K,
                               void *stream)
{
    HTD_REQUIRE(Co > 0 && K > 0 && K % 4 == 0, "bn_fold: bad sizes Co=%d K=%d", Co, K);
    HTD_REQUIRE(w && gamma && beta && mean && var && w_folded && b_folded, "bn_fold: null pointer");
    hipLaunchKernelGGL(bn_fold_fwd_kernel, dim3((unsigned)Co), dim3(256), 0, (hipStream_t)stream, w, gamma, beta, mean,
                       var, eps, w_folded, b_folded, K);
    return htd::check_launch("bn_fold_fwd");
}

extern "C" int htd_bn_fold_many_fwd(const void *desc, int n_layers, int total_tiles, float eps, void *stream)
{
    static_assert(sizeof(FoldDesc) == 80, "FoldDesc layout is part of the ABI");
    HTD_REQUIRE(desc && n_layers > 0 && total_tiles > 0, "bn_fold_many_fwd: bad arguments");
    hipLaunchKernelGGL(bn_fold_many_fwd_kernel, dim3((unsigned)total_tiles), dim3(256), 0, (hipStream_t)stream,
                       (const FoldDesc *)desc, n_layers, eps);
    return htd::check_launch("bn_fold_many_fwd");
}

extern "C" int htd_bn_fold_many_bwd(const void *desc, int n_layers, int total_rows, float eps, void *stream)
{
    static_assert(sizeof(FoldBwdDesc) == 88, "FoldBwdDesc layout is part of the ABI");
    HTD_REQUIRE(desc && n_layers > 0 && total_rows > 0, "bn_fold_many_bwd: bad arguments");
    hipLaunchKernelGGL(bn_fold_many_bwd_kernel, dim3((unsigned)total_rows), dim3(256), 0, (hipStream_t)stream,
                       (const FoldBwdDesc *)desc, n_layers, eps);
    return htd::check_launch("bn_fold_many_bwd");
}

extern "C" int htd_bn_fold_bwd(const float *w, const float *gamma, const float *mean, const float *var, float eps,
                               const float *gw_folded, const float *gb_folded, float *gw, float *ggamma, float *gbeta,
                               int Co, int K, void *stream)
{
    HTD_REQUIRE(Co > 0 && K > 0 && K % 4 == 0, "bn_fold: bad sizes Co=%d K=%d", Co, K);
    HTD_REQUIRE(w && gamma && mean && var && gw_folded && gb_folded && gw && ggamma && gbeta, "bn_fold_bwd: null pointer");
    hipLaunchKernelGGL(bn_fold_bwd_kernel, dim3((unsigned)Co), dim3(256), 0, (hipStream_t)stream, w, gamma, mean, var,
                       eps, gw_folded, gb_folded, gw, ggamma, gbeta, K);
    return htd::check_launch("bn_fold_bwd");
}

namespace {

__global__ __launch_bounds__(256) void max_pool_fwd_kernel(const float *__restrict__ x, float *__restrict__ y,
                                                           int *__restrict__ idx, int B, int H, int W, int C4, int Ho,
                                                           int Wo, int k, int s, int p, float *__restrict__ amax_out)
{
    const int64_t total = (int64_t)B * Ho * Wo * C4;
    unsigned mx = 0u;
    for (int64_t t = (int64_t)blockIdx.x * 256 + threadIdx.x; t < total; t += (int64_t)gridDim.x * 256) {
        const int c4 = (int)(t % C4);
        int64_t r = t / C4;
        const int wo = (int)(r % Wo);
        r /= Wo;
        const int ho = (int)(r % Ho), b = (int)(r / Ho);
        float4 m = make_float4(-INFINITY, -INFINITY, -INFINITY, -INFINITY);
        int4 am = make_int4(-1, -1, -1, -1);
        for (int i = 0; i < k; ++i) {
            const int hi = ho * s - p + i;
            if ((unsigned)hi >= (unsigned)H) continue;
            for (int j = 0; j < k; ++j) {
                const int wi = wo * s - p + j;
                if ((unsigned)wi >= (unsigned)W) continue;
                const float4 v = reinterpret_cast<const float4 *>(x)[(((int64_t)b * H + hi) * W + wi) * C4 + c4];
                const int pix = hi * W + wi;
                if (v.x > m.x || v.x != v.x) { m.x = v.x; am.x = pix; }
                if (v.y > m.y || v.y != v.y) { m.y = v.y; am.y = pix; }
                if (v.z > m.z || v.z != v.z) { m.z = v.z; am.z = pix; }
                if (v.w > m.w || v.w != v.w) { m.w = v.w; am.w = pix; }
            }
        }
        reinterpret_cast<float4 *>(y)[t] = m;
        if (idx) reinterpret_cast<int4 *>(idx)[t] = am;
        mx = htd::mag_bits4(mx, m);
    }
    if (amax_out) htd::wave_mag_out(mx, amax_out);
}

__global__ __launch_bounds__(256) void max_pool_bwd_kernel(const float *__restrict__ g, const int *__restrict__ idx,
                                                           float *__restrict__ gx, int B, int H, int W, int C4, int Ho,
                                                           int Wo, int k, int s, int p)
{
    const int64_t total = (int64_t)B * H * W * C4;
    for (int64_t t = (int64_t)blockIdx.x * 256 + threadIdx.x; t < total; t += (int64_t)gridDim.x * 256) {
        const int c4 = (int)(t % C4);
        int64_t r = t / C4;
        const int wi = (int)(r % W);
        r /= W;
        const int hi = (int)(r % H), b = (int)(r / H);
        const int pix = hi * W + wi;
        float4 acc = make_float4(0.f, 0.f, 0.f, 0.f);
        const int ho_lo = max(0, (hi + p - k + s) / s), ho_hi = min(Ho - 1, (hi + p) / s);
        const int wo_lo = max(0, (wi + p - k + s) / s), wo_hi = min(Wo - 1, (wi + p) / s);
        for (int ho = ho_lo; ho <= ho_hi; ++ho)
            for (int wo = wo_lo; wo <= wo_hi; ++wo) {
                const int64_t o = (((int64_t)b * Ho + ho) * Wo + wo) * C4 + c4;
                const int4 am = reinterpret_cast<const int4 *>(idx)[o];
                const float4 gv = reinterpret_cast<const float4 *>(g)[o];
                if (am.x == pix) acc.x += gv.x;
                if (am.y == pix) acc.y += gv.y;
                if (am.z == pix) acc.z += gv.z;
                if (am.w == pix) acc.w += gv.w;
            }
        reinterpret_cast<float4 *>(gx)[t] = acc;
    }
}

}

namespace {
__global__ __launch_bounds__(256) void upsample_nearest_bwd_kernel(const float4 *__restrict__ g, float4 *__restrict__ out, int B,
                                                                   int H, int W, int h, int w, int C4, float sh, float sw)
{
    const int64_t total = (int64_t)B * h * w * C4;
    for (int64_t e = (int64_t)blockIdx.x * 256 + threadIdx.x; e < total; e += (int64_t)gridDim.x * 256) {
        const int c = (int)(e % C4);
        int64_t t = e / C4;
        const int rw = (int)(t % w);
        t /= w;
        const int rh = (int)(t % h), b = (int)(t / h);
        const int ho0 = max(0, (int)floorf(rh / sh) - 1), ho1 = min(H - 1, (int)ceilf((rh + 1) / sh) + 1);
        const int wo0 = max(0, (int)floorf(rw / sw) - 1), wo1 = min(W - 1, (int)ceilf((rw + 1) / sw) + 1);
        float4 acc = make_float4(0.f, 0.f, 0.f, 0.f);
        for (int ho = ho0; ho <= ho1; ++ho) {
            if (min((int)floorf(ho * sh), h - 1) != rh) continue;
            for (int wo = wo0; wo <= wo1; ++wo) {
                if (min((int)floorf(wo * sw), w - 1) != rw) continue;
                const float4 v = g[(((int64_t)b * H + ho) * W + wo) * C4 + c];
                acc.x += v.x; acc.y += v.y; acc.z += v.z; acc.w += v.w;
            }
        }
        out[e] = acc;
    }
}
}

namespace {
__global__ __launch_bounds__(256) void upsample_nearest_bwd_bf16_kernel(const uint2 *__restrict__ g, uint2 *__restrict__ out, int B,
                                                                        int H, int W, int h, int w, int C4, float sh, float sw)
{
    const int64_t total = (int64_t)B * h * w * C4;
    for (int64_t e = (int64_t)blockIdx.x * 256 + threadIdx.x; e < total; e += (int64_t)gridDim.x * 256) {
        const int c = (int)(e % C4);
        int64_t t = e / C4;
        const int rw = (int)(t % w);
        t /= w;
        const int rh = (int)(t % h), b = (int)(t / h);
        const int ho0 = max(0, (int)floorf(rh / sh) - 1), ho1 = min(H - 1, (int)ceilf((rh + 1) / sh) + 1);
        const int wo0 = max(0, (int)floorf(rw / sw) - 1), wo1 = min(W - 1, (int)ceilf((rw + 1) / sw) + 1);
        float acc[4] = {0.f, 0.f, 0.f, 0.f};
        for (int ho = ho0; ho <= ho1; ++ho) {
            if (min((int)floorf(ho * sh), h - 1) != rh) continue;
            for (int wo = wo0; wo <= wo1; ++wo) {
                if (min((int)floorf(wo * sw), w - 1) != rw) continue;
                const uint2 v = g[(((int64_t)b * H + ho) * W + wo) * C4 + c];
                acc[0] += __uint_as_float(v.x << 16); acc[1] += __uint_as_float(v.x & 0xffff0000u);
                acc[2] += __uint_as_float(v.y << 16); acc[3] += __uint_as_float(v.y & 0xffff0000u);
            }
        }
        unsigned r[4];
#pragma unroll
        for (int k = 0; k < 4; ++k) {
            const unsigned u = __float_as_uint(acc[k]);
            r[k] = (u & 0x7fffffffu) > 0x7f800000u ? ((u >> 16) | 0x40u) : ((u + 0x7fffu + ((u >> 16) & 1u)) >> 16);
        }
        out[e] = make_uint2(r[0] | (r[1] << 16), r[2] | (r[3] << 16));
    }
}
}

extern "C" int htd_upsample_nearest_bwd_bf16(const void *g, void *out, int B, int H, int W, int h, int w, int C, void *stream)
{
    HTD_REQUIRE(g && out && B > 0 && H > 0 && W > 0 && h > 0 && w > 0 && C > 0 && C % 4 == 0,
                "upsample_nearest_bwd_bf16: bad arguments");
    const int64_t total = (int64_t)B * h * w * (C / 4);
    const unsigned blocks = (unsigned)std::min<int64_t>(htd::ceil_div(total, 256), 65536);
    hipLaunchKernelGGL(upsample_nearest_bwd_bf16_kernel, dim3(blocks), dim3(256), 0, (hipStream_t)stream, (const uint2 *)g,
                       (uint2 *)out, B, H, W, h, w, C / 4, (float)h / (float)H, (float)w / (float)W);
    return htd::check_launch("upsample_nearest_bwd_bf16");
}

extern "C" int htd_upsample_nearest_bwd(const float *g, float *out, int B, int H, int W, int h, int w, int C, void *stream)
{
    HTD_REQUIRE(g && out && B > 0 && H > 0 && W > 0 && h > 0 && w > 0 && C > 0 && C % 4 == 0, "upsample_nearest_bwd: bad arguments");
    const int64_t total = (int64_t)B * h * w * (C / 4);
    const unsigned blocks = (unsigned)std::min<int64_t>(htd::ceil_div(total, 256), 65536);
    hipLaunchKernelGGL(upsample_nearest_bwd_kernel, dim3(blocks), dim3(256), 0, (hipStream_t)stream, (const float4 *)g,
                       (float4 *)out, B, H, W, h, w, C / 4, (float)h / (float)H, (float)w / (float)W);
    return htd::check_launch("upsample_nearest_bwd");
}

static int max_pool2d_fwd_impl(const float *x, float *y, int *idx, int B, int H, int W, int C, int k, int stride, int pad,
                               float *amax_out, void *stream)
{
    HTD_REQUIRE(B > 0 && H > 0 && W > 0 && C > 0 && k > 0 && stride > 0 && pad >= 0 && 2 * pad <= k,
                "max_pool2d: bad sizes");
    HTD_REQUIRE(C % 4 == 0, "max_pool2d: C=%d must be a multiple of 4", C);
    HTD_REQUIRE((int64_t)H * W < (1ll << 31), "max_pool2d: map too large");
    HTD_REQUIRE(x && y, "max_pool2d: null pointer");
    const int Ho = (H + 2 * pad - k) / stride + 1, Wo = (W + 2 * pad - k) / stride + 1;
    HTD_REQUIRE(Ho > 0 && Wo > 0, "max_pool2d: empty output");
    const int64_t total = (int64_t)B * Ho * Wo * (C / 4);
    const unsigned blocks = (unsigned)std::min<int64_t>(htd::ceil_div(total, 256), 65536);
    hipLaunchKernelGGL(max_pool_fwd_kernel, dim3(blocks), dim3(256), 0, (hipStream_t)stream, x, y, idx, B, H, W, C / 4,
                       Ho, Wo, k, stride, pad, amax_out);
    return htd::check_launch("max_pool2d_fwd");
}

extern "C" int htd_max_pool2d_fwd(const float *x, float *y, int *idx, int B, int H, int W, int C, int k, int stride,
                                  int pad, void *stream)
{
    return max_pool2d_fwd_impl(x, y, idx, B, H, W, C, k, stride, pad, nullptr, stream);
}

extern "C" int htd_max_pool2d_fwd_amax(const float *x, float *y, int *idx, int B, int H, int W, int C, int k, int stride, int pad,
                                       float *amax_out, void *stream)
{
    HTD_REQUIRE(amax_out, "max_pool2d: null maximum");
    return max_pool2d_fwd_impl(x, y, idx, B, H, W, C, k, stride, pad, amax_out, stream);
}

extern "C" int htd_max_pool2d_bwd(const float *g, const int *idx, float *gx, int B, int H, int W, int C, int k,
                                  int stride, int pad, void *stream)
{
    HTD_REQUIRE(B > 0 && H > 0 && W > 0 && C > 0 && k > 0 && stride > 0 && pad >= 0 && C % 4 == 0,
                "max_pool2d_bwd: bad sizes");
    HTD_REQUIRE(g && idx && gx, "max_pool2d_bwd: null pointer");
    const int Ho = (H + 2 * pad - k) / stride + 1, Wo = (W + 2 * pad - k) / stride + 1;
    const int64_t total = (int64_t)B * H * W * (C / 4);
    const unsigned blocks = (unsigned)std::min<int64_t>(htd::ceil_div(total, 256), 65536);
    hipLaunchKernelGGL(max_pool_bwd_kernel, dim3(blocks), dim3(256), 0, (hipStream_t)stream, g, idx, gx, B, H, W, C / 4,
                       Ho, Wo, k, stride, pad);
    return htd::check_launch("max_pool2d_bwd");
}

extern "C" int htd_rows_gather(const float *x, const int64_t *rows, float *out, int64_t n, int64_t N, int F, void *stream)
{
    HTD_REQUIRE(n >= 0 && N >= 0 && F > 0 && F % 4 == 0, "rows_gather: bad sizes n=%lld N=%lld F=%d", (long long)n, (long long)N, F);
    if (n == 0) return HTD_OK;
    HTD_REQUIRE(x && rows && out, "rows_gather: null pointer");
    const int64_t total = n * (F / 4);
    hipLaunchKernelGGL(rows_gather_kernel, dim3(grid_for(total, 256, 8192)), dim3(256), 0, (hipStream_t)stream, (const float4 *)x, rows,
                       (float4 *)out, total, F / 4);
    return htd::check_launch("rows_gather");
}

extern "C" int htd_rows_add(const float *g, const int64_t *rows, float *gx, int64_t n, int64_t N, int F, void *stream)
{
    HTD_REQUIRE(n >= 0 && N >= 0 && F > 0 && F % 4 == 0, "rows_add: bad sizes n=%lld N=%lld F=%d", (long long)n, (long long)N, F);
    if (n == 0) return HTD_OK;
    HTD_REQUIRE(g && rows && gx, "rows_add: null pointer");
    const int64_t total = n * (F / 4);
    hipLaunchKernelGGL(rows_add_kernel, dim3(grid_for(total, 256, 8192)), dim3(256), 0, (hipStream_t)stream, (const float4 *)g, rows,
                       (float4 *)gx, total, F / 4);
    return htd::check_launch("rows_add");
}
```

### include/htd_amd.h

```cpp
#ifndef HTD_AMD_H
#define HTD_AMD_H

#include <stdint.h>

#ifdef __cplusplus
extern "C" {
#endif

#define HTD_OK 0
#define HTD_ERR_ARG 1
#define HTD_ERR_LAUNCH 2

const char *htd_last_error(void);
#define HTD_ABI_VERSION 5
int htd_abi_version(void);

int htd_roi_align_fwd(const float *feat, const float *rois, const int64_t *roi_level, int level,
                      float *out, int64_t n, int B, int C, int H, int W, int ph, int pw, float spatial_scale,
                      int sampling_ratio, int aligned, void *stream);
int htd_roi_align_bwd(const float *grad_out, const float *rois, const int64_t *roi_level, int level,
                      float *grad_feat, int64_t n, int B, int C, int H, int W, int ph, int pw,
                      float spatial_scale, int sampling_ratio, int aligned, void *stream);
int htd_roi_align_levels_fwd(const float *const *feats, const int *H, const int *W, const float *scales, int L,
                             const float *rois, const int64_t *roi_level, float *out, int64_t n, int B, int C, int ph, int pw,
                             int sampling_ratio, int aligned, void *stream);
int htd_roi_align_levels_fwd_amax(const float *const *feats, const int *H, const int *W, const float *scales, int L,
                                  const float *rois, const int64_t *roi_level, float *out, int64_t n, int B, int C, int ph,
                                  int pw, int sampling_ratio, int aligned, float *amax_out, void *stream);
int htd_roi_align_levels_bwd_gather(const float *grad_out, const float *rois, const int64_t *roi_level,
                                    float *const *grad_feats, const int *H, const int *W, const float *scales,
                                    const int *accumulate, int L, int64_t n, int B, int C, int ph, int pw,
                                    int sampling_ratio, int aligned, void *workspace, void *stream);
int htd_roi_align_all_levels_fwd(const float *const *feats, const int *H, const int *W, const float *scales, int L,
                                 const float *rois, float *const *outs, int64_t n, int B, int C, int ph, int pw,
                                 int sampling_ratio, int aligned, void *stream);
int htd_roi_align_all_levels_bwd_gather(const float *const *grad_outs, const float *rois, float *const *grad_feats,
                                        const int *H, const int *W, const float *scales, const int *accumulate, int L,
                                        int64_t n, int B, int C, int ph, int pw, int sampling_ratio, int aligned,
                                        void *workspace, void *stream);
int64_t htd_roi_align_fold_workspace_bytes(int64_t n, const int *H, int L, int pw, int C);
int htd_roi_align_levels_bwd_gather_folded(const float *grad_out, const float *rois, const int64_t *roi_level,
                                           float *const *grad_feats, const int *H, const int *W, const float *scales,
                                           const int *accumulate, int L, int64_t n, int B, int C, int ph, int pw,
                                           int sampling_ratio, int aligned, void *workspace, void *fold_ws, void *stream);
int htd_roi_align_all_levels_bwd_gather_folded(const float *const *grad_outs, const float *rois, float *const *grad_feats,
                                               const int *H, const int *W, const float *scales, const int *accumulate,
                                               int L, int64_t n, int B, int C, int ph, int pw, int sampling_ratio,
                                               int aligned, void *workspace, void *fold_ws, void *stream);
int64_t htd_roi_align_bwd_gather_workspace_bytes(int64_t n);
int htd_roi_align_bwd_gather(const float *grad_out, const float *rois, const int64_t *roi_level, int level,
                             float *grad_feat, int64_t n, int B, int C, int H, int W, int ph, int pw,
                             float spatial_scale, int sampling_ratio, int aligned, int accumulate, void *workspace,
                             void *stream);

int64_t htd_nms_workspace_bytes(int64_t n_total);
int htd_nms_sorted(const float *boxes, uint8_t *keep_mask, int64_t n, float iou_thr, int offset,
                   void *workspace, void *stream);
int htd_nms_sorted_batched(const float *boxes, const int64_t *seg_offsets, int segments,
                           int64_t n_total, int64_t max_seg, uint8_t *keep_mask, float iou_thr,
                           int offset, void *workspace, void *stream);

int htd_soft_nms_segments(const float *boxes, float *scores, const int64_t *seg_offsets, int segments,
                          int64_t n_total, int *rank, float iou_thr, float sigma, float min_score,
                          int method, int offset, void *stream);

int64_t htd_segmented_topk_workspace_bytes(int S, int64_t nchunks);
int htd_segmented_topk(const float *keys, const int64_t *segs, const int32_t *chunk_tab, int S, int64_t nchunks,
                       int64_t *out_idx, float *out_val, void *workspace, void *stream);
int64_t htd_random_sample_workspace_bytes(int B, int64_t A, int64_t nchunks);
int htd_random_sample(const int64_t *assigned, const float *keys, int B, int64_t A, int num, int max_pos, float neg_pos_ub,
                      const int64_t *segs, const int32_t *chunk_tab, int64_t nchunks, unsigned char *pos_mask,
                      unsigned char *neg_mask, int64_t *counts, int64_t *order, int slots, void *workspace, void *stream);

int htd_fuse_global_fwd(const float *roi_feats, const float *rois, const float *global_feat,
                        const float *extra, float alpha, float *out, int64_t n, int P, int C,
                        int B, void *stream);
int htd_plain_and_fused_fwd(const float *roi_feats, const float *rois, const float *global_feat, float *both,
                            int64_t n, int P, int C, int B, void *stream);
int htd_fuse_global_fwd_amax(const float *roi_feats, const float *rois, const float *global_feat, const float *extra,
                             float alpha, float *out, int64_t n, int P, int C, int B, float *amax_out, void *stream);
int htd_plain_and_fused_fwd_amax(const float *roi_feats, const float *rois, const float *global_feat, float *both,
                                 int64_t n, int P, int C, int B, float *amax_out, void *stream);
int htd_fuse_global_bwd_global(const float *grad, const float *rois, float *grad_global,
                               int64_t n, int P, int C, int B, void *stream);

int htd_ba_fuse_fwd(const float *const *lvl, int L, const float *border, const float *att,
                    float *out, int64_t n, int ph, int pw, int C, int edge, void *stream);
int htd_ba_fuse_bwd(const float *const *lvl, int L, const float *att, const float *grad_out,
                    float *const *grad_lvl, float *grad_border, float *grad_att, int64_t n, int ph,
                    int pw, int C, int edge, void *stream);

int64_t htd_conv2d_workspace_bytes(int64_t M, int Co, int Ci, int kh, int kw);
int htd_conv2d_set_math(int mode);
int htd_conv2d_tile_table_set(int64_t M, int Co, int Ci, int taps, int epi, int cfg);
int htd_conv2d_tile_table_clear(void);
int htd_conv2d_tile_query(int64_t M, int Co, int Ci, int taps, int epi);
int htd_conv2d_fwd(const float *x, const float *w, const float *bias, const float *residual, int res_h,
                   int res_w, float *y, int B, int H, int W, int Ci, int Co, int kh, int kw, int stride,
                   int pad, int dil, int relu, void *workspace, void *stream);
int htd_bgemm_nt(const float *a, const float *b, float *c, int G, int M, int N, int K, void *stream);
int htd_bgemm_nt_counts(const float *a, const float *b, float *c, int G, int M, int N, int K, const int64_t *counts, int limit,
                        void *stream);
int htd_conv2d_flip_weights(const float *w, float *wT, int Co, int kh, int kw, int Ci, void *stream);
int htd_conv2d_flip_weights_padded(const float *w, float *wT, int Co, int Co_padded, int kh, int kw, int Ci, void *stream);
int htd_pad_channels(const float *x, float *y, int64_t rows, int C, int C_padded, void *stream);
int htd_conv2d_bwd_data(const float *gy, const float *wT, const float *mask_src, const float *accum, float *gx,
                        int B, int H, int W, int Ci, int Co, int kh, int kw, int stride, int pad, int dil,
                        void *workspace, void *stream);
int htd_conv2d_fwd_amax(const float *x, const float *w, const float *bias, const float *residual, int res_h, int res_w,
                        float *y, float *amax_out, int B, int H, int W, int Ci, int Co, int kh, int kw, int stride, int pad,
                        int dil, int relu, void *workspace, void *stream);
int htd_conv2d_bwd_data_amax(const float *gy, const float *wT, const float *mask_src, const float *accum, float *gx,
                             float *amax_out, int B, int H, int W, int Ci, int Co, int kh, int kw, int stride, int pad,
                             int dil, void *workspace, void *stream);
int64_t htd_conv2d_wgrad_workspace_bytes(int B, int H, int W, int Ci, int Co, int kh, int kw,
                                         int stride, int pad, int dil);
int htd_conv2d_bwd_weight(const float *x, const float *gy, float *gw, float *gbias, int B, int H, int W,
                          int Ci, int Co, int kh, int kw, int stride, int pad, int dil, void *workspace,
                          void *stream);
int htd_conv2d_bwd_weight_acc(const float *x, const float *gy, float *gw, float *gbias, int B, int H, int W, int Ci,
                              int Co, int kh, int kw, int stride, int pad, int dil, void *workspace, void *stream);
int htd_bias_grad_relu_mask(const float *g, const float *y, float *gm, float *gbias, int64_t rows,
                            int C, void *workspace, void *stream);
int htd_bias_grad_relu_mask_amax(const float *g, const float *y, float *gm, float *gbias, int64_t rows, int C,
                                 void *workspace, float *amax_out, void *stream);
int64_t htd_conv2d_stem7_workspace_bytes(void);
int htd_conv2d_stem7_fwd(const float *x, const float *w, const float *bias, float *y, int B, int H, int W, int relu,
                         void *workspace, void *stream);
int htd_conv2d_x3p_supported(int Ci, int Co, int kh, int kw, int stride, int pad, int dil);
int htd_conv2d_x3p_tile_table_set(int64_t M, int Co, int Ci, int taps, int epi, int cfg);
int htd_conv2d_x3p_tile_table_clear(void);
int htd_conv2d_x3p_tile_query(int64_t M, int Co, int Ci, int taps, int epi);
int htd_conv2d_x3p_plan_query(int cfg, int64_t M, int Co, int Ci, int kh, int kw, int64_t *out);
int64_t htd_conv2d_x3_planes_bytes(int Co, int kh, int kw, int Ci, int transposed);
int htd_conv2d_x3_planes(const float *w, void *planes, int Co, int kh, int kw, int Ci, int transposed, void *stream);
int htd_conv2d_x3_planes_many(const void *desc, int n, int64_t total_blocks, void *stream);
int64_t htd_conv2d_x3p_workspace_bytes(int64_t M, int Co, int Ci, int kh, int kw);
int htd_conv2d_fwd_x3p(const float *x, const void *wplanes, const float *bias, const float *residual, int res_h,
                       int res_w, float *y, int B, int H, int W, int Ci, int Co, int kh, int kw, int stride, int pad,
                       int relu, void *workspace, void *stream);
int htd_conv2d_bwd_data_x3p(const float *gy, const void *wplanesT, const float *mask_src, const float *accum,
                            float *gx, int B, int H, int W, int Ci, int Co, int kh, int kw, int pad, void *workspace,
                            void *stream);
int64_t htd_act_planes_rows(int64_t M);
int64_t htd_act_planes_bytes(int64_t M, int C);
int htd_act_planes(const float *x, void *planes, int64_t M, int C, void *stream);
int htd_conv2d_fwd_x3q(const float *x, const void *xplanes, const void *wplanes, const float *bias, const float *residual,
                       int res_h, int res_w, float *y, void *yplanes, float *amax_out, int B, int H, int W, int Ci, int Co, int kh, int kw,
                       int stride, int pad, int relu, void *workspace, void *stream);
int htd_conv2d_bwd_data_x3q(const float *gy, const void *gyplanes, const void *wplanesT, const float *mask_src,
                            const float *accum, float *gx, void *gxplanes, float *amax_out, int B, int H, int W, int Ci, int Co, int kh, int kw,
                            int pad, void *workspace, void *stream);

int htd_conv2d_set_h2(int on);
int htd_conv2d_bwd_weight_h2_supported(int B, int H, int W, int Ci, int Co, int kh, int kw, int stride, int pad, int dil);
int htd_conv2d_bwd_weight_h2(const float *x, const float *gy, const float *amax_x, const float *amax_g, float *gw,
                             float *gbias, int B, int H, int W, int Ci, int Co, int kh, int kw, int stride, int pad,
                             int dil, int accumulate, void *workspace, void *stream);
int htd_conv2d_x3h_supported(int Ci, int Co, int kh, int kw, int stride, int pad, int dil);
int htd_conv2d_x3h_strided_supported(int Ci, int Co, int kh, int kw, int stride, int pad, int dil);
int htd_conv2d_bwd_data_x3h_strided_supported(int Ci, int Co, int kh, int kw, int stride, int pad, int dil);
int64_t htd_conv2d_bwd_data_x3h_strided_workspace_bytes(int B, int H, int W, int Ci, int Co, int kh, int kw, int stride, int pad);
int htd_conv2d_bwd_data_x3h_strided(const float *gy, const float *amax, const void *wplanesT, const float *mask_src, float *gx,
                                    float *amax_out, int B, int H, int W, int Ci, int Co, int kh, int kw, int stride, int pad,
                                    void *workspace, void *stream);
int htd_absmax(const float *x, int64_t n, float *amax, void *stream);
int htd_conv2d_x3h_planes(const float *w, void *planes, int Co, int kh, int kw, int Ci, int transposed, void *stream);
int htd_conv2d_x3h_planes_many(const void *desc, int n, int64_t total_blocks, int64_t total_rows, void *stream);
int htd_conv2d_fwd_x3h(const float *x, const float *amax, const void *wplanes, const float *bias, const float *residual,
                       int res_h, int res_w, float *y, void *yplanes, float *amax_out, int B, int H, int W, int Ci,
                       int Co, int kh, int kw, int stride, int pad, int relu, void *workspace, void *stream);
int htd_conv2d_bwd_data_x3h(const float *gy, const float *amax, const void *wplanesT, const float *mask_src,
                            const float *accum, float *gx, void *gxplanes, float *amax_out, int B, int H, int W,
                            int Ci, int Co, int kh, int kw, int pad, void *workspace, void *stream);

int64_t htd_deform_columns_bytes(int B, int H, int W, int C, int kh, int kw, int stride, int pad, int dil);
int htd_deform_im2col(const float *x, const float *offset, const float *mask, float *columns, int B,
                      int H, int W, int C, int kh, int kw, int stride, int pad, int dil,
                      int deform_groups, void *stream);
int htd_deform_col2im(const float *x, const float *offset, const float *mask, const float *gcolumns,
                      float *gx, float *goffset, float *gmask, int B, int H, int W, int C, int kh,
                      int kw, int stride, int pad, int dil, int deform_groups, void *stream);
int htd_deform_im2col_bf16(const void *x, const float *offset, const float *mask, void *columns, int B, int H, int W,
                           int C, int kh, int kw, int stride, int pad, int dil, int deform_groups, void *stream);
int htd_deform_col2im_bf16(const void *x, const float *offset, const float *mask, const void *gcolumns, float *gx,
                           float *goffset, float *gmask, int B, int H, int W, int C, int kh, int kw, int stride, int pad,
                           int dil, int deform_groups, void *stream);

int htd_global_avg_pool_fwd(const float *x, float *out, int64_t B, int P, int C, void *stream);
int htd_global_avg_pool_bwd(const float *g, float *gx, int64_t B, int P, int C, void *stream);
int htd_global_avg_pool_bwd_acc(const float *g, float *gx, int64_t B, int P, int C, void *stream);

int htd_group_norm_relu_fwd(const float *x, const float *gamma, const float *beta, float *y,
                            float *mean, float *rstd, int64_t n, int P, int C, int G, float eps,
                            int relu, void *stream);
int htd_group_norm_relu_bwd(const float *x, const float *y, const float *gamma, const float *mean,
                            const float *rstd, const float *gy, float *gx, float *ggamma,
                            float *gbeta, int64_t n, int P, int C, int G, int relu, void *stream);
int htd_group_norm_relu_bwd_ws(const float *x, const float *y, const float *gamma, const float *mean, const float *rstd,
                               const float *gy, float *gx, float *ggamma, float *gbeta, int64_t n, int P, int C, int G,
                               int relu, void *workspace, void *stream);
int htd_group_norm_relu_fwd_amax(const float *x, const float *gamma, const float *beta, float *y, float *mean, float *rstd,
// ... 140 lines not shown
```

Baseline: 124.2 images/sec.

## Use block-level amax reduction and per-image RoI lists in RoI-align backward gather

Replaces the per-wave atomic max used to track activation magnitude with a block-level shared-memory reduction. Each block does a single atomic, skipped when the value already seen is larger. Grids are capped when amax is requested, and the RoI-align forward becomes a grid-stride loop. The RoI-align backward gather builds a compacted list of RoIs per image, so each tile scans only its own image's RoIs instead of all n. This adds a list-building kernel, larger workspace and an ABI bump.

```diff
diff --git a/htd_amd/csrc/common.h b/htd_amd/csrc/common.h
--- a/htd_amd/csrc/common.h
+++ b/htd_amd/csrc/common.h
@@ -49,12 +49,29 @@
 {
     return max(max(mx, max(mag_bits(v.x), mag_bits(v.y))), max(mag_bits(v.z), mag_bits(v.w)));
 }
-__device__ __forceinline__ void wave_mag_out(unsigned bits, float *out)
+__device__ __forceinline__ unsigned mag_seen(const float *out)
+{
+    return (out && threadIdx.x == 0) ? __hip_atomic_load(reinterpret_cast<const unsigned *>(out), __ATOMIC_RELAXED, __HIP_MEMORY_SCOPE_AGENT)
+                                     : 0u;
+}
+__device__ __forceinline__ unsigned wave_mag_max(unsigned bits)
 {
 #pragma unroll
     for (int o = 32; o > 0; o >>= 1) bits = max(bits, (unsigned)__shfl_xor((int)bits, o, 64));
-    if ((threadIdx.x & 63) == 0 && bits > *reinterpret_cast<volatile unsigned *>(out))
-        __hip_atomic_fetch_max(reinterpret_cast<unsigned *>(out), bits, __ATOMIC_RELAXED, __HIP_MEMORY_SCOPE_AGENT);
+    return bits;
+}
+__device__ __forceinline__ void block_mag_out(unsigned bits, float *out, unsigned seen)
+{
+    __shared__ unsigned mag_red[16];
+    bits = wave_mag_max(bits);
+    const int tid = threadIdx.x;
+    if ((tid & 63) == 0) mag_red[tid >> 6] = bits;
+    __syncthreads();
+    if (tid == 0) {
+        const int waves = (int)((blockDim.x + 63) >> 6);
+        for (int w = 1; w < waves; ++w) bits = max(bits, mag_red[w]);
+        if (bits > seen) __hip_atomic_fetch_max(reinterpret_cast<unsigned *>(out), bits, __ATOMIC_RELAXED, __HIP_MEMORY_SCOPE_AGENT);
+    }
 }
 
 inline int64_t ceil_div(int64_t a, int64_t b) { return (a + b - 1) / b; }
diff --git a/htd_amd/csrc/conv_fwd.hip b/htd_amd/csrc/conv_fwd.hip
--- a/htd_amd/csrc/conv_fwd.hip
+++ b/htd_amd/csrc/conv_fwd.hip
@@ -105,6 +105,7 @@
 
     const int tid = threadIdx.x, lane = tid & 63, wave = tid >> 6;
     const int wm = wave / WGN, wn = wave % WGN;
+    const unsigned oseen = htd::mag_seen(p.amax_out);
 
     int k_limit = 0x7fffffff;
     if (p.group_count) {
@@ -489,13 +490,14 @@
         }
         if (i + 1 < TM) __syncthreads();
     }
-    if (p.amax_out != nullptr && tail_split < 0 && p.splits <= 1) htd::wave_mag_out(omx, p.amax_out);
+    if (p.amax_out != nullptr && tail_split < 0 && p.splits <= 1) htd::block_mag_out(omx, p.amax_out, oseen);
 }
 
 __global__ __launch_bounds__(256) void conv_splitk_epilogue_kernel(ConvParams p)
 {
     const int64_t total = p.M * p.Co;
     unsigned omx = 0u;
+    const unsigned oseen = htd::mag_seen(p.amax_out);
     for (int64_t o = (int64_t)blockIdx.x * blockDim.x + threadIdx.x; o < total; o += (int64_t)gridDim.x * blockDim.x) {
         float v = 0.f;
         for (int k = 0; k < p.splits; ++k) v += p.partial[(int64_t)k * total + o];
@@ -518,13 +520,14 @@
         p.y[o] = v;
         omx = max(omx, htd::mag_bits(v));
     }
-    if (p.amax_out != nullptr) htd::wave_mag_out(omx, p.amax_out);
+    if (p.amax_out != nullptr) htd::block_mag_out(omx, p.amax_out, oseen);
 }
 
 __global__ __launch_bounds__(256) void conv_tail_epilogue_kernel(ConvParams p, int BM, int BN)
 {
     const int64_t per_tile = (int64_t)BM * BN, total = (int64_t)(p.mt * p.nt - p.tail_first) * per_tile;
     unsigned omx = 0u;
+    const unsigned oseen = htd::mag_seen(p.amax_out);
     for (int64_t e = (int64_t)blockIdx.x * blockDim.x + threadIdx.x; e < total; e += (int64_t)gridDim.x * blockDim.x) {
         const int t = (int)(e / per_tile), within = (int)(e - (int64_t)t * per_tile);
         const int tile = p.tail_first + t, tile_m = tile / p.nt, tile_n = tile % p.nt;
@@ -552,7 +555,7 @@
         p.y[o] = v;
         omx = max(omx, htd::mag_bits(v));
     }
-    if (p.amax_out != nullptr) htd::wave_mag_out(omx, p.amax_out);
+    if (p.amax_out != nullptr) htd::block_mag_out(omx, p.amax_out, oseen);
 }
 
 int g_conv_math = getenv("HTD_CONV_MATH") ? atoi(getenv("HTD_CONV_MATH")) : 1;
diff --git a/htd_amd/csrc/conv_wgrad.hip b/htd_amd/csrc/conv_wgrad.hip
--- a/htd_amd/csrc/conv_wgrad.hip
+++ b/htd_amd/csrc/conv_wgrad.hip
@@ -1280,7 +1280,7 @@
 }
 
 using htd::mag_bits;
-using htd::wave_mag_out;
+using htd::block_mag_out;
 
 __global__ __launch_bounds__(256) void colsum_mask_kernel(const float *__restrict__ g, const float *__restrict__ y,
                                                           float *__restrict__ gm, float *__restrict__ partial,
@@ -1290,6 +1290,7 @@
     const int64_t r0 = (int64_t)blockIdx.x * rows_per_block, r1 = min(rows, r0 + rows_per_block);
     float s = 0.f;
     unsigned mx = 0u;
+    const unsigned seen = htd::mag_seen(amax_out);
     if (c < C)
         for (int64_t r = r0; r < r1; ++r) {
             float v = g[r * C + c];
@@ -1300,7 +1301,7 @@
             mx = max(mx, mag_bits(v));
             s += v;
         }
-    if (amax_out) wave_mag_out(mx, amax_out);
+    if (amax_out) block_mag_out(mx, amax_out, seen);
     if (partial && c < C) partial[(int64_t)blockIdx.x * C + c] = s;
 }
 
@@ -1311,6 +1312,7 @@
 {
     __shared__ float4 red[256];
     unsigned mx = 0u;
+    const unsigned seen = htd::mag_seen(amax_out);
     const int C4 = C >> 2;
     const int cbase = blockIdx.y * 256;
     const int cw = min(256, C4 - cbase);
@@ -1353,7 +1355,7 @@
             s.x += v.x; s.y += v.y; s.z += v.z; s.w += v.w;
         }
     }
-    if (amax_out) wave_mag_out(mx, amax_out);
+    if (amax_out) block_mag_out(mx, amax_out, seen);
     if (!partial) return;
     red[threadIdx.x] = s;
     __syncthreads();
diff --git a/htd_amd/csrc/roi_align.hip b/htd_amd/csrc/roi_align.hip
--- a/htd_amd/csrc/roi_align.hip
+++ b/htd_amd/csrc/roi_align.hip
@@ -57,6 +57,8 @@
     lo = (int)c0;
     hi = min((int)c1 + 1, extent - 1);
 }
+
+__device__ __forceinline__ int wave_index() { return __builtin_amdgcn_readfirstlane((int)(threadIdx.x >> 6)); }
 
 __device__ __forceinline__ float lane_bcast(float v, int src)
 {
@@ -221,62 +223,57 @@
                                                                    float *__restrict__ amax_out)
 {
     const int lane = threadIdx.x & 63;
-    const int64_t task = (int64_t)blockIdx.x * (blockDim.x >> 6) + (threadIdx.x >> 6);
-    if (task >= tasks) return;
-    const unsigned seen = amax_out ? *reinterpret_cast<const volatile unsigned *>(amax_out) : 0u;
-    const int chunk = (int)(task % chunks);
-    const int64_t t2 = task / chunks;
-    const int bin = (int)(t2 % (ph * pw));
-    const int64_t ri = t2 / (ph * pw);
-    const int lv = (int)roi_level[ri];
-    const int ch = chunk * 256 + lane * 4;
-    const bool act = ch < C;
-    const size_t bin_off = ((size_t)ri * ph * pw + bin) * C;
-    float4 acc = make_float4(0.f, 0.f, 0.f, 0.f);
-    RoiGeom g{};
-    g.inv_count = 0.f;
-    if (lv >= 0 && lv < L) {
-        const int H = tab.H[lv], W = tab.W[lv];
-        const float *feat = tab.feat[lv];
-        const int bi = bin / pw, bj = bin % pw;
-        g = roi_geometry(rois + 5 * ri, tab.scale[lv], ph, pw, sampling_ratio, aligned);
-        int r0, r1, c0, c1;
-        axis_span(g.start_h, g.bin_h, bi, g.grid_h, H, r0, r1);
-        axis_span(g.start_w, g.bin_w, bj, g.grid_w, W, c0, c1);
-        if (g.batch < 0 || g.batch >= B) { r0 = 0; r1 = -1; }
-        const size_t img_base = (size_t)g.batch * H * W * C;
-        for (int rb = r0; rb <= r1; rb += 64) {
-            const float wy_l = (rb + lane <= r1) ? axis_weight(g.start_h, g.bin_h, bi, g.grid_h, rb + lane, H) : 0.f;
-            for (int cb = c0; cb <= c1; cb += 64) {
-                const float wx_l = (cb + lane <= c1) ? axis_weight(g.start_w, g.bin_w, bj, g.grid_w, cb + lane, W) : 0.f;
-                const int rn = min(64, r1 - rb + 1), cn = min(64, c1 - cb + 1);
-                for (int r = 0; r < rn; ++r) {
-                    const float wy = lane_bcast(wy_l, r);
-                    const float *row = feat + img_base + ((size_t)(rb + r) * W + cb) * C + ch;
+    const unsigned seen = htd::mag_seen(amax_out);
+    unsigned mx = 0u;
+    for (int64_t task = (int64_t)blockIdx.x * 4 + wave_index(); task < tasks; task += (int64_t)gridDim.x * 4) {
+        const int chunk = (int)(task % chunks);
+        const int64_t t2 = task / chunks;
+        const int bin = (int)(t2 % (ph * pw));
+        const int64_t ri = t2 / (ph * pw);
+        const int lv = (int)roi_level[ri];
+        const int ch = chunk * 256 + lane * 4;
+        const bool act = ch < C;
+        const size_t bin_off = ((size_t)ri * ph * pw + bin) * C;
+        float4 acc = make_float4(0.f, 0.f, 0.f, 0.f);
+        RoiGeom g{};
+        g.inv_count = 0.f;
+        if (lv >= 0 && lv < L) {
+            const int H = tab.H[lv], W = tab.W[lv];
+            const float *feat = tab.feat[lv];
+            const int bi = bin / pw, bj = bin % pw;
+            g = roi_geometry(rois + 5 * ri, tab.scale[lv], ph, pw, sampling_ratio, aligned);
+            int r0, r1, c0, c1;
+            axis_span(g.start_h, g.bin_h, bi, g.grid_h, H, r0, r1);
+            axis_span(g.start_w, g.bin_w, bj, g.grid_w, W, c0, c1);
+            if (g.batch < 0 || g.batch >= B) { r0 = 0; r1 = -1; }
+            const size_t img_base = (size_t)g.batch * H * W * C;
+            for (int rb = r0; rb <= r1; rb += 64) {
+                const float wy_l = (rb + lane <= r1) ? axis_weight(g.start_h, g.bin_h, bi, g.grid_h, rb + lane, H) : 0.f;
+                for (int cb = c0; cb <= c1; cb += 64) {
+                    const float wx_l = (cb + lane <= c1) ? axis_weight(g.start_w, g.bin_w, bj, g.grid_w, cb + lane, W) : 0.f;
+                    const int rn = min(64, r1 - rb + 1), cn = min(64, c1 - cb + 1);
+                    for (int r = 0; r < rn; ++r) {
+                        const float wy = lane_bcast(wy_l, r);
+                        const float *row = feat + img_base + ((size_t)(rb + r) * W + cb) * C + ch;
 #pragma unroll 4
-                    for (int c = 0; c < cn; ++c) {
-                        const float w = wy * lane_bcast(wx_l, c);
-                        if (act) {
-                            const float4 v = *reinterpret_cast<const float4 *>(row + (size_t)c * C);
-                            acc.x += w * v.x; acc.y += w * v.y; acc.z += w * v.z; acc.w += w * v.w;
+                        for (int c = 0; c < cn; ++c) {
+                            const float w = wy * lane_bcast(wx_l, c);
+                            if (act) {
+                                const float4 v = *reinterpret_cast<const float4 *>(row + (size_t)c * C);
+                                acc.x += w * v.x; acc.y += w * v.y; acc.z += w * v.z; acc.w += w * v.w;
+                            }
                         }
                     }
                 }
             }
         }
-    }
-    if (act) {
-        acc.x *= g.inv_count; acc.y *= g.inv_count; acc.z *= g.inv_count; acc.w *= g.inv_count;
-        *reinterpret_cast<float4 *>(out + bin_off + ch) = acc;
-    }
-    if (amax_out) {
-        const bool nan = act && ((acc.x != acc.x) | (acc.y != acc.y) | (acc.z != acc.z) | (acc.w != acc.w));
-        const float m = act ? fmaxf(fmaxf(fabsf(acc.x), fabsf(acc.y)), fmaxf(fabsf(acc.z), fabsf(acc.w))) : 0.f;
-        unsigned bits = nan ? 0x7fc00000u : __float_as_uint(m);
-        for (int o = 32; o > 0; o >>= 1) bits = max(bits, (unsigned)__shfl_xor((int)bits, o));
-        if (lane == 0 && bits > seen)
-            __hip_atomic_fetch_max(reinterpret_cast<unsigned *>(amax_out), bits, __ATOMIC_RELAXED, __HIP_MEMORY_SCOPE_AGENT);
-    }
+        if (act) {
+            acc.x *= g.inv_count; acc.y *= g.inv_count; acc.z *= g.inv_count; acc.w *= g.inv_count;
+            *reinterpret_cast<float4 *>(out + bin_off + ch) = acc;
+            mx = htd::mag_bits4(mx, acc);
+        }
+    }
+    if (amax_out) htd::block_mag_out(mx, amax_out, seen);
 }
 
 struct AllLevelsOut {
@@ -436,7 +433,66 @@
 
 constexpr int GW_TILE = 8;
 
-struct RoiBox { short b, r_lo, r_hi, c_lo, c_hi, pad0, pad1, pad2; };
+struct alignas(16) RoiBox { short b, r_lo, r_hi, c_lo, c_hi, pad; int idx; };
+
+constexpr int LIST_IMAGES = 256;
+constexpr int64_t LIST_MAX_N = 64 * 1024;
+constexpr int LIST_THREADS = 1024;
+
+inline int64_t level_ws_bytes(int64_t n) { return (n > 0 ? n : 1) * 2 * (int64_t)sizeof(RoiBox) + LIST_IMAGES * (int64_t)sizeof(int2); }
+inline RoiBox *ws_box(void *ws, int64_t l, int64_t n) { return (RoiBox *)((char *)ws + l * level_ws_bytes(n)); }
+inline RoiBox *ws_list(void *ws, int64_t l, int64_t n) { return ws_box(ws, l, n) + (n > 0 ? n : 1); }
+inline int2 *ws_tab(void *ws, int64_t l, int64_t n) { return (int2 *)(ws_list(ws, l, n) + (n > 0 ? n : 1)); }
+
+__device__ __forceinline__ void roi_list_build(const RoiBox *__restrict__ box, RoiBox *__restrict__ list, int2 *__restrict__ tab,
+                                               int64_t n, int b)
+{
+    __shared__ int before[LIST_MAX_N / 64];
+    __shared__ int total[2];
+    const int lane = threadIdx.x & 63, wave = threadIdx.x >> 6;
+    const int batches = (int)((n + 63) / 64);
+    if (threadIdx.x < 2) total[threadIdx.x] = 0;
+    __syncthreads();
+    int lower = 0;
+    for (int k = wave; k < batches; k += LIST_THREADS / 64) {
+        const int64_t ri = (int64_t)k * 64 + lane;
+        const short ob = ri < n ? box[ri].b : (short)-1;
+        lower += __popcll(__ballot(ob >= 0 && ob < b));
+        const int here = __popcll(__ballot(ob == b));
+        if (lane == 0) before[k] = here;
+    }
+    if (lane == 0 && lower) atomicAdd(&total[0], lower);
+    __syncthreads();
+    if (wave == 0) {
+        int run = 0;
+        for (int k0 = 0; k0 < batches; k0 += 64) {
+            const int v = k0 + lane < batches ? before[k0 + lane] : 0;
+            int inc = v;
+#pragma unroll
+            for (int o = 1; o < 64; o <<= 1) {
+                const int t = __shfl_up(inc, o, 64);
+                if (lane >= o) inc += t;
+            }
+            if (k0 + lane < batches) before[k0 + lane] = run + inc - v;
+            run += __shfl(inc, 63, 64);
+        }
+        if (lane == 0) total[1] = run;
+    }
+    __syncthreads();
+    const int start = total[0];
+    if (threadIdx.x == 0) tab[b] = make_int2(start, total[1]);
+    for (int k = wave; k < batches; k += LIST_THREADS / 64) {
+        const int64_t ri = (int64_t)k * 64 + lane;
+        RoiBox o{};
+        o.b = -1;
+        if (ri < n) o = box[ri];
+        const unsigned long long m = __ballot(o.b == b);
+        if (o.b == b) {
+            o.idx = (int)ri;
+            list[start + before[k] + __popcll(m & ((1ull << lane) - 1ull))] = o;
+        }
+    }
+}
 
 __global__ __launch_bounds__(256) void roi_bbox_kernel(const float *__restrict__ rois, const int64_t *__restrict__ roi_level,
                                                        int level, RoiBox *__restrict__ box, int64_t n, int B, int H, int W,
@@ -457,7 +513,14 @@
         ok = ok && !(t0 < c_lo || c_hi < t1);
         if (ok) { o.b = (short)g.batch; o.r_lo = (short)r_lo; o.r_hi = (short)r_hi; o.c_lo = (short)c_lo; o.c_hi = (short)c_hi; }
     }
+    o.idx = (int)ri;
     box[ri] = o;
+}
+
+__global__ __launch_bounds__(LIST_THREADS) void roi_list_kernel(const RoiBox *__restrict__ box, RoiBox *__restrict__ list,
+                                                                int2 *__restrict__ tab, int64_t n)
+{
+    roi_list_build(box, list, tab, n, blockIdx.x);
 }
 
 template <int CPL, int ROWS, int RS, bool FOLD>
@@ -465,15 +528,14 @@
                                             const RoiBox *__restrict__ box, float *__restrict__ gfeat, int64_t n, int B, int C,
                                             int H, int W, int ph, int pw, float scale, int sampling_ratio, int aligned,
                                             int accumulate, int chunks, int segs, int hts, int64_t task, bool active,
-                                            const float *__restrict__ tbuf)
+                                            const float *__restrict__ tbuf, const RoiBox *__restrict__ list,
+                                            const int2 *__restrict__ tab)
 {
     static_assert(!FOLD || ROWS == 1, "folded rows: one-row tiles");
     static_assert(ROWS * MAXP <= 64, "one lane per (row, bin) weight");
     static_assert(RS == 1 || ROWS == 1, "the RoI split keeps one-row tiles");
     const int lane = threadIdx.x & 63;
-    const int wave = threadIdx.x >> 6, part = wave % RS;
-    constexpr unsigned long long kEvery = RS == 4 ? 0x1111111111111111ull : (RS == 2 ? 0x5555555555555555ull : ~0ull);
-    const unsigned long long mine = kEvery << part;
+    const int wave = wave_index(), part = wave % RS;
     const int chunk = (int)(task % chunks);
     int64_t t2 = task / chunks;
     const int seg = (int)(t2 % segs);
@@ -493,17 +555,27 @@
             for (int k = 0; k < CPL; ++k) acc[r][i][k] = 0.f;
     bool touched = false;
 
-    for (int64_t base = 0; base < (active ? n : 0); base += 64) {
-        bool hit = false;
-        if (base + lane < n) {
-            const RoiBox o = box[base + lane];
-            hit = o.b == b && o.r_lo <= y1 && y0 <= o.r_hi && o.c_lo <= x1 && o.c_hi >= x0;
-        }
-        unsigned long long mask = __ballot(hit) & mine;
+    const RoiBox *src = box;
+    int64_t cnt = n;
+    if (list) {
+        const int2 sc = tab[b];
+        src = list + sc.x;
+        cnt = sc.y;
+    }
+    if (!active) cnt = 0;
+    RoiBox nxt{};
+    if (lane < cnt) nxt = src[lane];
+    for (int64_t base = 0; base < cnt; base += 64) {
+        const RoiBox o = nxt;
+        const bool have = base + lane < cnt;
+        if (base + 64 + lane < cnt) nxt = src[base + 64 + lane];
+        const bool hit = have && o.b == b && o.r_lo <= y1 && y0 <= o.r_hi && o.c_lo <= x1 && o.c_hi >= x0 &&
+                         (RS == 1 || (o.idx & (RS - 1)) == part);
+        unsigned long long mask = __ballot(hit);
         while (mask) {
-            const int src = __builtin_ctzll(mask);
+            const int src_lane = __builtin_ctzll(mask);
             mask &= mask - 1;
-            const int64_t ri = base + src;
+            const int64_t ri = __builtin_amdgcn_readlane(o.idx, src_lane);
             touched = true;
             const RoiGeom g = roi_geometry(rois + 5 * ri, scale, ph, pw, sampling_ratio, aligned);
             if constexpr (FOLD) {
@@ -633,16 +705,17 @@
 }
 
 template <int CPL, int ROWS, int RS>
-__global__ __launch_bounds__(256, (RS > 1 ? 4 : 1)) void roi_align_bwd_gather_kernel(const float *__restrict__ gout, const float *__restrict__ rois,
+__global__ __launch_bounds__(256, (RS > 1 ? 4 : 5)) void roi_align_bwd_gather_kernel(const float *__restrict__ gout, const float *__restrict__ rois,
                                                                    const RoiBox *__restrict__ box, float *__restrict__ gfeat,
                                                                    int64_t n, int B, int C, int H, int W, int ph, int pw,
                                                                    float scale, int sampling_ratio, int aligned, int accumulate,
-                                                                   int chunks, int segs, int hts, int64_t tasks)
-{
-    const int64_t task = (int64_t)blockIdx.x * (4 / RS) + (threadIdx.x >> 6) / RS;
+                                                                   int chunks, int segs, int hts, int64_t tasks,
+                                                                   const RoiBox *__restrict__ list, const int2 *__restrict__ tab)
+{
+    const int64_t task = (int64_t)blockIdx.x * (4 / RS) + wave_index() / RS;
     if (RS == 1 && task >= tasks) return;
     gather_tile<CPL, ROWS, RS, false>(gout, rois, box, gfeat, n, B, C, H, W, ph, pw, scale, sampling_ratio, aligned, accumulate,
-                                      chunks, segs, hts, task < tasks ? task : 0, task < tasks, nullptr);
+                                      chunks, segs, hts, task < tasks ? task : 0, task < tasks, nullptr, list, tab);
 }
 
 constexpr int GL_MAX = 6;
@@ -652,6 +725,8 @@
     float *tbuf[GL_MAX];
     int64_t ftask0[GL_MAX + 1];
     const RoiBox *box[GL_MAX];
+    const RoiBox *list[GL_MAX];
+    const int2 *tab[GL_MAX];
     int H[GL_MAX], W[GL_MAX], segs[GL_MAX], hts[GL_MAX], accumulate[GL_MAX], level[GL_MAX];
     float scale[GL_MAX];
     int64_t task0[GL_MAX + 1];
@@ -703,12 +778,12 @@
 }
 
 template <int CPL, int ROWS, int RS, bool FOLD>
-__global__ __launch_bounds__(256, (RS > 1 ? 4 : 1)) void roi_align_bwd_gather_levels_kernel(const float *__restrict__ gout,
+__global__ __launch_bounds__(256, (RS > 1 ? 4 : 5)) void roi_align_bwd_gather_levels_kernel(const float *__restrict__ gout,
                                                                           const float *__restrict__ rois, GatherLevels t, int64_t n,
                                                                           int B, int C, int ph, int pw, int sampling_ratio,
                                                                           int aligned, int chunks)
 {
-    int64_t task = (int64_t)blockIdx.x * (4 / RS) + (threadIdx.x >> 6) / RS;
+    int64_t task = (int64_t)blockIdx.x * (4 / RS) + wave_index() / RS;
     const bool active = task < t.task0[t.slots];
     if (RS == 1 && !active) return;
     if (!active) task = 0;
@@ -718,7 +793,7 @@
         if (i < t.slots && task >= t.task0[i]) k = i;
     gather_tile<CPL, ROWS, RS, FOLD>(t.gout[k] ? t.gout[k] : gout, rois, t.box[k], t.gfeat[k], n, B, C, t.H[k], t.W[k], ph, pw,
                                      t.scale[k], sampling_ratio, aligned, t.accumulate[k], chunks, t.segs[k], t.hts[k],
-                                     task - t.task0[k], active, t.tbuf[k]);
+                                     task - t.task0[k], active, t.tbuf[k], t.list[k], t.tab[k]);
 }
 
 __global__ __launch_bounds__(256) void roi_bbox_levels_kernel(const float *__restrict__ rois, const int64_t *__restrict__ roi_level,
@@ -742,7 +817,14 @@
         ok = ok && !(t0 < c_lo || c_hi < t1);
         if (ok) { o.b = (short)g.batch; o.r_lo = (short)r_lo; o.r_hi = (short)r_hi; o.c_lo = (short)c_lo; o.c_hi = (short)c_hi; }
     }
+    o.idx = (int)ri;
     const_cast<RoiBox *>(t.box[k])[ri] = o;
+}
+
+__global__ __launch_bounds__(LIST_THREADS) void roi_list_levels_kernel(GatherLevels t, int64_t n)
+{
+    const int k = blockIdx.y;
+    roi_list_build(t.box[k], const_cast<RoiBox *>(t.list[k]), const_cast<int2 *>(t.tab[k]), n, blockIdx.x);
 }
 
 int gather_split(int64_t n, int64_t tiles_min, bool every_level)
@@ -751,6 +833,28 @@
     if (forced == 1 || forced == 2 || forced == 4) return forced;
     (void)n; (void)tiles_min;
     return every_level ? 2 : 1;
+}
+
+int fwd_resident_blocks()
+{
+    static const int resident = [] {
+        int dev = 0, cus = 0, per_cu = 0;
+        if (hipGetDevice(&dev) != hipSuccess || hipDeviceGetAttribute(&cus, hipDeviceAttributeMultiprocessorCount, dev) != hipSuccess ||
+            hipOccupancyMaxActiveBlocksPerMultiprocessor(&per_cu, roi_align_levels_fwd_kernel, 256, 0) != hipSuccess || cus <= 0 || per_cu <= 0) {
+            (void)hipGetLastError();
+            return 2048;
+        }
+        return cus * per_cu;
+    }();
+    return resident;
+}
+
+int g_roi_lists = -1;
+bool gather_lists(int64_t n, int B)
+{
+    static const int env = getenv("HTD_ROI_BWD_LISTS") ? atoi(getenv("HTD_ROI_BWD_LISTS")) : 1;
+    const int on = g_roi_lists >= 0 ? g_roi_lists : env;
+    return on != 0 && B <= LIST_IMAGES && n <= LIST_MAX_N;
 }
 
 int launch(bool backward, const float *in, const float *rois, const int64_t *roi_level, int level, float *out,
@@ -816,8 +920,12 @@
     }
     const int chunks = (C + 255) / 256;
     const int64_t tasks = n * ph * pw * chunks;
-    const int64_t blocks = htd::ceil_div(tasks, 4);
+    int64_t blocks = htd::ceil_div(tasks, 4);
     HTD_REQUIRE(blocks < (1ll << 31), "roi_align_levels: too many tasks");
+    if (amax_out) {
+        static const int rounds = getenv("HTD_ROI_FWD_ROUNDS") ? std::max(1, atoi(getenv("HTD_ROI_FWD_ROUNDS"))) : 1;
+        blocks = std::min<int64_t>(blocks, (int64_t)rounds * fwd_resident_blocks());
+    }
     hipLaunchKernelGGL(roi_align_levels_fwd_kernel, dim3((unsigned)blocks), dim3(256), 0, (hipStream_t)stream, tab, rois, roi_level, out,
                        n, B, C, L, ph, pw, sampling_ratio, aligned, chunks, tasks, amax_out);
     return htd::check_launch("roi_align_levels");
@@ -868,7 +976,14 @@
     return htd::check_launch("roi_align_all_levels");
 }
 
-extern "C" int64_t htd_roi_align_bwd_gather_workspace_bytes(int64_t n) { return (n > 0 ? n : 1) * (int64_t)sizeof(RoiBox); }
+extern "C" int64_t htd_roi_align_bwd_gather_workspace_bytes(int64_t n) { return level_ws_bytes(n); }
+
+extern "C" int htd_roi_align_bwd_set_lists(int on)
+{
+    HTD_REQUIRE(on >= -1 && on <= 1, "roi_align_bwd_set_lists: %d is not -1, 0 or 1", on);
+    g_roi_lists = on;
+    return HTD_OK;
+}
 
 extern "C" int htd_roi_align_bwd_gather(const float *grad_out, const float *rois, const int64_t *roi_level, int level,
                                         float *grad_feat, int64_t n, int B, int C, int H, int W, int ph, int pw,
@@ -887,9 +1002,17 @@
         }
         return HTD_OK;
     }
-    RoiBox *box = (RoiBox *)workspace;
+    RoiBox *box = ws_box(workspace, 0, n);
     hipLaunchKernelGGL(roi_bbox_kernel, dim3((unsigned)htd::ceil_div(n, 256)), dim3(256), 0, s, rois, roi_level, level, box, n, B,
                        H, W, ph, pw, spatial_scale, sampling_ratio, aligned);
+    const RoiBox *list = nullptr;
+    const int2 *tab = nullptr;
+    if (gather_lists(n, B)) {
+        list = ws_list(workspace, 0, n);
+        tab = ws_tab(workspace, 0, n);
+        hipLaunchKernelGGL(roi_list_kernel, dim3((unsigned)B), dim3(LIST_THREADS), 0, s, box, const_cast<RoiBox *>(list),
+                           const_cast<int2 *>(tab), n);
+    }
     const int segs = (W + GW_TILE - 1) / GW_TILE;
     constexpr int rows = 1;
     const int chunks = (C + 255) / 256;
@@ -900,14 +1023,14 @@
     const int rs = gather_split(n, tasks, roi_level == nullptr);
     if (rs == 4)
         hipLaunchKernelGGL((roi_align_bwd_gather_kernel<4, rows, 4>), dim3((unsigned)tasks), dim3(256), 0, s, grad_out, rois, box,
-                           grad_feat, n, B, C, H, W, ph, pw, spatial_scale, sampling_ratio, aligned, accumulate, chunks, segs, hts, tasks);
+                           grad_feat, n, B, C, H, W, ph, pw, spatial_scale, sampling_ratio, aligned, accumulate, chunks, segs, hts, tasks, list, tab);
     else if (rs == 2)
         hipLaunchKernelGGL((roi_align_bwd_gather_kernel<4, rows, 2>), dim3((unsigned)htd::ceil_div(tasks, 2)), dim3(256), 0, s, grad_out,
                            rois, box, grad_feat, n, B, C, H, W, ph, pw, spatial_scale, sampling_ratio, aligned, accumulate, chunks, segs,
-                           hts, tasks);
+                           hts, tasks, list, tab);
     else
         hipLaunchKernelGGL((roi_align_bwd_gather_kernel<4, rows, 1>), dim3((unsigned)blocks), dim3(256), 0, s, grad_out, rois, box,
-                           grad_feat, n, B, C, H, W, ph, pw, spatial_scale, sampling_ratio, aligned, accumulate, chunks, segs, hts, tasks);
+                           grad_feat, n, B, C, H, W, ph, pw, spatial_scale, sampling_ratio, aligned, accumulate, chunks, segs, hts, tasks, list, tab);
     return htd::check_launch("roi_align_bwd_gather");
 }
 
@@ -925,6 +1048,7 @@
     hipStream_t s = (hipStream_t)stream;
     GatherLevels t{};
     const int chunks = (C + 255) / 256;
+    const bool lists = gather_lists(n, B);
     int64_t tasks = 0, tiles_min = 1ll << 62;
     for (int l = L - 1; l >= 0; --l) {
         if (!grad_feats[l]) continue;
@@ -940,7 +1064,9 @@
         t.gfeat[k] = grad_feats[l];
         t.gout[k] = grad_outs ? grad_outs[l] : nullptr;
         HTD_REQUIRE(!grad_outs || grad_outs[l], "%s: level %d has a gradient map but no grad_out", what, l);
-        t.box[k] = (const RoiBox *)workspace + (int64_t)l * n;
+        t.box[k] = ws_box(workspace, l, n);
+        t.list[k] = lists ? ws_list(workspace, l, n) : nullptr;
+        t.tab[k] = lists ? ws_tab(workspace, l, n) : nullptr;
         t.H[k] = H[l]; t.W[k] = W[l]; t.scale[k] = scales[l]; t.accumulate[k] = accumulate[l]; t.level[k] = l;
         t.segs[k] = (W[l] + GW_TILE - 1) / GW_TILE;
         t.hts[k] = H[l];
@@ -961,6 +1087,7 @@
     t.ftask0[t.slots] = ftasks;
     hipLaunchKernelGGL(roi_bbox_levels_kernel, dim3((unsigned)htd::ceil_div(n, 256), (unsigned)t.slots), dim3(256), 0, s, rois,
                        roi_level, t, n, B, ph, pw, sampling_ratio, aligned);
+    if (lists) hipLaunchKernelGGL(roi_list_levels_kernel, dim3((unsigned)B, (unsigned)t.slots), dim3(LIST_THREADS), 0, s, t, n);
     HTD_REQUIRE(tasks < (1ll << 31), "%s: too many tiles", what);
     const int rs = gather_split(n, tiles_min, roi_level == nullptr);
     if (fold_ws) {
diff --git a/htd_amd/csrc/roi_ops.hip b/htd_amd/csrc/roi_ops.hip
--- a/htd_amd/csrc/roi_ops.hip
+++ b/htd_amd/csrc/roi_ops.hip
@@ -15,6 +15,7 @@
                                                               int C4, int B, float *__restrict__ amax_out)
 {
     unsigned mx = 0u;
+    const unsigned seen = htd::mag_seen(amax_out);
     for (int64_t idx = (int64_t)blockIdx.x * blockDim.x + threadIdx.x; idx < total4;
          idx += (int64_t)gridDim.x * blockDim.x) {
         const int c4 = (int)(idx % C4);
@@ -31,7 +32,7 @@
         st4(out + idx * 4, v);
         mx = htd::mag_bits4(mx, v);
     }
-    if (amax_out) htd::wave_mag_out(mx, amax_out);
+    if (amax_out) htd::block_mag_out(mx, amax_out, seen);
 }
 
 __global__ __launch_bounds__(256) void plain_and_fused_kernel(const float *__restrict__ x, const float *__restrict__ rois,
@@ -39,6 +40,7 @@
                                                               int64_t total4, int P, int C4, int B, float *__restrict__ amax_out)
 {
     unsigned mx = 0u;
+    const unsigned seen = htd::mag_seen(amax_out);
     for (int64_t idx = (int64_t)blockIdx.x * blockDim.x + threadIdx.x; idx < total4; idx += (int64_t)gridDim.x * blockDim.x) {
         const int c4 = (int)(idx % C4);
         const int64_t i = idx / ((int64_t)P * C4);
@@ -52,7 +54,7 @@
         st4(both + (total4 + idx) * 4, v);
         mx = htd::mag_bits4(mx, v);
     }
-    if (amax_out) htd::wave_mag_out(mx, amax_out);
+    if (amax_out) htd::block_mag_out(mx, amax_out, seen);
 }
 
 constexpr int ROIS_PER_BLOCK = 16;
@@ -763,6 +765,8 @@
     }
 }
 
+constexpr int AMAX_GRID_CAP = 2048;
+
 inline unsigned grid_for(int64_t work, int block = 256, int cap = 4096)
 {
     int64_t b = htd::ceil_div(work, block);
@@ -779,7 +783,7 @@
     if (n == 0) return HTD_OK;
     HTD_REQUIRE(roi_feats && rois && global_feat && out, "fuse_global: null pointer");
     const int64_t total4 = n * P * (C / 4);
-    hipLaunchKernelGGL(fuse_global_fwd_kernel, dim3(grid_for(total4)), dim3(256), 0, (hipStream_t)stream, roi_feats,
+    hipLaunchKernelGGL(fuse_global_fwd_kernel, dim3(grid_for(total4, 256, amax_out ? AMAX_GRID_CAP : 4096)), dim3(256), 0, (hipStream_t)stream, roi_feats,
                        rois, global_feat, extra, alpha, out, total4, P, C / 4, B, amax_out);
     return htd::check_launch("fuse_global_fwd");
 }
@@ -805,7 +809,7 @@
     if (n == 0) return HTD_OK;
     HTD_REQUIRE(roi_feats && rois && global_feat && both, "plain_and_fused: null pointer");
     const int64_t total4 = n * P * (C / 4);
-    hipLaunchKernelGGL(plain_and_fused_kernel, dim3(grid_for(total4)), dim3(256), 0, (hipStream_t)stream, roi_feats, rois,
+    hipLaunchKernelGGL(plain_and_fused_kernel, dim3(grid_for(total4, 256, amax_out ? AMAX_GRID_CAP : 4096)), dim3(256), 0, (hipStream_t)stream, roi_feats, rois,
                        global_feat, both, total4, P, C / 4, B, amax_out);
     return htd::check_launch("plain_and_fused_fwd");
 }
@@ -1106,6 +1110,7 @@
 {
     const int64_t total = (int64_t)B * Ho * Wo * C4;
     unsigned mx = 0u;
+    const unsigned seen = htd::mag_seen(amax_out);
     for (int64_t t = (int64_t)blockIdx.x * 256 + threadIdx.x; t < total; t += (int64_t)gridDim.x * 256) {
         const int c4 = (int)(t % C4);
         int64_t r = t / C4;
@@ -1132,7 +1137,7 @@
         if (idx) reinterpret_cast<int4 *>(idx)[t] = am;
         mx = htd::mag_bits4(mx, m);
     }
-    if (amax_out) htd::wave_mag_out(mx, amax_out);
+    if (amax_out) htd::block_mag_out(mx, amax_out, seen);
 }
 
 __global__ __launch_bounds__(256) void max_pool_bwd_kernel(const float *__restrict__ g, const int *__restrict__ idx,
@@ -1259,7 +1264,7 @@
     const int Ho = (H + 2 * pad - k) / stride + 1, Wo = (W + 2 * pad - k) / stride + 1;
     HTD_REQUIRE(Ho > 0 && Wo > 0, "max_pool2d: empty output");
     const int64_t total = (int64_t)B * Ho * Wo * (C / 4);
-    const unsigned blocks = (unsigned)std::min<int64_t>(htd::ceil_div(total, 256), 65536);
+    const unsigned blocks = (unsigned)std::min<int64_t>(htd::ceil_div(total, 256), amax_out ? AMAX_GRID_CAP : 65536);
     hipLaunchKernelGGL(max_pool_fwd_kernel, dim3(blocks), dim3(256), 0, (hipStream_t)stream, x, y, idx, B, H, W, C / 4,
                        Ho, Wo, k, stride, pad, amax_out);
     return htd::check_launch("max_pool2d_fwd");
diff --git a/include/htd_amd.h b/include/htd_amd.h
--- a/include/htd_amd.h
+++ b/include/htd_amd.h
@@ -12,7 +12,7 @@
 #define HTD_ERR_LAUNCH 2
 
 const char *htd_last_error(void);
-#define HTD_ABI_VERSION 5
+#define HTD_ABI_VERSION 6
 int htd_abi_version(void);
 
 int htd_roi_align_fwd(const float *feat, const float *rois, const int64_t *roi_level, int level,
@@ -48,6 +48,7 @@
                                                int L, int64_t n, int B, int C, int ph, int pw, int sampling_ratio,
                                                int aligned, void *workspace, void *fold_ws, void *stream);
 int64_t htd_roi_align_bwd_gather_workspace_bytes(int64_t n);
+int htd_roi_align_bwd_set_lists(int on);
 int htd_roi_align_bwd_gather(const float *grad_out, const float *rois, const int64_t *roi_level, int level,
                              float *grad_feat, int64_t n, int B, int C, int H, int W, int ph, int pw,
                              float spatial_scale, int sampling_ratio, int aligned, int accumulate, void *workspace,
```

Measured after the change: 122.6 images/sec. 0.987x the previous value.
